# iDC-NEU/NeutronStarLite

Hardware: NVIDIA H100
Metric: gcn_aggregated_edges_per_sec (higher is better)
Workload: dtype f32

## Files before the change

### include/nts_b200.h

```cpp
#ifndef NTS_B200_H
#define NTS_B200_H

#include <stddef.h>
#include <stdint.h>

#ifdef __cplusplus
extern "C" {
#endif

typedef uint32_t nts_vid_t;

int nts_version(void);
const char *nts_last_error(void);
int nts_device_count(void);
int nts_set_device(int device);
int nts_device_sm_count(int *sm_count);
int nts_device_synchronize(void);
int nts_device_reset(void);

void *nts_malloc_device(size_t bytes);
int nts_free_device(void *ptr);
void *nts_malloc_pinned(size_t bytes);
int nts_free_pinned(void *ptr);
void *nts_pinned_device_pointer(void *host_ptr);
int nts_memcpy_h2d(void *dst_device, const void *src_host, size_t bytes, void *stream, int sync);
int nts_memcpy_d2h(void *dst_host, const void *src_device, size_t bytes, void *stream, int sync);
int nts_memcpy_d2d(void *dst_device, const void *src_device, size_t bytes, void *stream);
int nts_zero(void *device_ptr, size_t bytes, void *stream);

void *nts_stream_create(int non_blocking);
int nts_stream_destroy(void *stream);
int nts_stream_synchronize(void *stream);
void *nts_event_create(int with_timing);
int nts_event_destroy(void *event);
int nts_event_record(void *event, void *stream);
int nts_stream_wait_event(void *stream, void *event);
int nts_event_elapsed_ms(void *start, void *stop, float *ms);

int nts_segment_gather_sum(const float *input, float *output, const float *weight,
                           const nts_vid_t *indices, const nts_vid_t *offsets, nts_vid_t index_base,
                           nts_vid_t n_rows, uint64_t n_edges, nts_vid_t feature_size, void *stream);

int nts_gather_by_dst_from_src(const float *input, float *output, const float *weight_forward,
                               const nts_vid_t *row_indices, const nts_vid_t *column_offset,
                               nts_vid_t src_start, nts_vid_t src_end, nts_vid_t dst_start,
                               nts_vid_t dst_end, nts_vid_t edges, nts_vid_t batch_size,
                               nts_vid_t feature_size, int with_weight, void *stream);

int nts_gather_by_src_from_dst(const float *input, float *output, const float *weight_backward,
                               const nts_vid_t *row_offset, const nts_vid_t *column_indices,
                               nts_vid_t src_start, nts_vid_t src_end, nts_vid_t dst_start,
                               nts_vid_t dst_end, nts_vid_t edges, nts_vid_t batch_size,
                               nts_vid_t feature_size, int with_weight, void *stream);

int nts_segment_gather_sum_range(const float *input, float *output, const float *weight, const nts_vid_t *indices,
                                 const nts_vid_t *offsets, const nts_vid_t *slot_of, nts_vid_t index_base,
                                 nts_vid_t n_rows, uint64_t edge_begin, uint64_t edge_end, nts_vid_t feature_size,
                                 void *stream);

typedef struct nts_gather_plan nts_gather_plan;
int nts_gather_plan_pick_slabs(nts_vid_t gather_rows, uint64_t n_edges, nts_vid_t n_rows, nts_vid_t feature_size,
                               uint64_t l2_budget_bytes );
nts_gather_plan *nts_gather_plan_create(const nts_vid_t *offsets, const nts_vid_t *indices, const float *weight,
                                        const nts_vid_t *slot_of, nts_vid_t index_base, nts_vid_t n_rows,
                                        uint64_t n_edges, nts_vid_t gather_rows, int n_slabs, void *stream);
nts_gather_plan *nts_gather_plan_create_hybrid(const nts_vid_t *offsets, const nts_vid_t *indices,
                                               const float *weight, const nts_vid_t *slot_of, nts_vid_t index_base,
                                               nts_vid_t n_rows, uint64_t n_edges, nts_vid_t gather_rows, int n_slabs,
                                               int n_hub_cols, int n_hub_rows, void *stream);
nts_gather_plan *nts_gather_plan_create_tuned(const nts_vid_t *offsets, const nts_vid_t *indices, const float *weight,
                                              const nts_vid_t *slot_of, nts_vid_t index_base, nts_vid_t n_rows,
                                              uint64_t n_edges, nts_vid_t gather_rows, nts_vid_t feature_size,
                                              void *stream);
typedef struct nts_plan_part {
  const nts_vid_t *offsets, *indices;
  const float *weight;
  const nts_vid_t *slot_of;
  nts_vid_t index_base, index_add, n_rows, row_add;
  uint64_t n_edges;
} nts_plan_part;
nts_gather_plan *nts_gather_plan_create_parts(const nts_plan_part *parts, int n_parts, nts_vid_t n_rows,
                                              nts_vid_t gather_rows, int n_slabs, nts_vid_t feature_size, void *stream);
float nts_gather_plan_tuned_ms(const nts_gather_plan *plan);
int nts_gather_plan_destroy(nts_gather_plan *plan);
int nts_gather_plan_slabs(const nts_gather_plan *plan);
int nts_gather_plan_hubs(const nts_gather_plan *plan, int *cols, int *rows);
uint64_t nts_gather_plan_bytes(const nts_gather_plan *plan);
int nts_gather_plan_run(nts_gather_plan *plan, const float *input, float *output, nts_vid_t feature_size,
                        void *stream);
int nts_gather_plan_last_launch(const nts_gather_plan *plan, int *launches, int *grid, int *k, int *u, int *outv);
enum { NTS_DTYPE_F32 = 0, NTS_DTYPE_BF16 = 1 };
int nts_gather_plan_run_bf16(nts_gather_plan *plan, const void *input, int input_dtype, float *output,
                             nts_vid_t feature_size, void *stream);
nts_gather_plan *nts_gather_plan_create_tuned_bf16(const nts_vid_t *offsets, const nts_vid_t *indices,
                                                   const float *weight, const nts_vid_t *slot_of, nts_vid_t index_base,
                                                   nts_vid_t n_rows, uint64_t n_edges, nts_vid_t gather_rows,
                                                   nts_vid_t feature_size, void *stream);
int nts_gather_plan_set_tuning(int u, int min_blocks, int edges_per_warp);
int nts_gather_plan_set_variant(int variant);

int nts_segment_gather_sum_slots(const float *input, float *output, const float *weight,
                                 const nts_vid_t *indices, const nts_vid_t *offsets,
                                 const nts_vid_t *slot_of, nts_vid_t n_rows, uint64_t n_edges,
                                 nts_vid_t feature_size, void *stream);

int nts_segment_gather_sum_heads(const float *input, float *output, const float *weight,
                                 const nts_vid_t *indices, const nts_vid_t *offsets, const nts_vid_t *slot_of,
                                 nts_vid_t index_base, nts_vid_t n_rows, uint64_t n_edges,
                                 nts_vid_t feature_size, nts_vid_t heads, void *stream);

int nts_aggregate_set_variant(int variant, int edges_per_warp);
int nts_aggregate_last_launch(int *grid, int *block, int *smem_bytes, int *variant);
uint64_t nts_kernel_launch_count(void);

int nts_scatter_src_mirror_to_msg(float *message, const float *src_mirror_feature,
                                  const nts_vid_t *row_indices, const nts_vid_t *column_offset,
                                  const nts_vid_t *mirror_index, nts_vid_t batch_size,
                                  nts_vid_t feature_size, void *stream);
int nts_gather_msg_to_src_mirror(float *src_mirror_feature, const float *message,
                                 const nts_vid_t *row_indices, const nts_vid_t *column_offset,
                                 const nts_vid_t *mirror_index, nts_vid_t batch_size,
                                 nts_vid_t feature_size, void *stream);
int nts_scatter_dst_to_msg(float *message, const float *dst_feature, const nts_vid_t *row_indices,
                           const nts_vid_t *column_offset, nts_vid_t batch_size,
                           nts_vid_t feature_size, void *stream);
int nts_gather_msg_to_dst(float *dst_feature, const float *message, const nts_vid_t *row_indices,
                          const nts_vid_t *column_offset, nts_vid_t batch_size,
                          nts_vid_t feature_size, void *stream);
int nts_edge_softmax_forward(float *msg_output, const float *msg_input, float *msg_cached,
                             const nts_vid_t *row_indices, const nts_vid_t *column_offset,
                             nts_vid_t batch_size, nts_vid_t feature_size, void *stream);
int nts_edge_softmax_backward(float *msg_input_grad, const float *msg_output_grad,
                              const float *msg_cached, const nts_vid_t *row_indices,
                              const nts_vid_t *column_offset, nts_vid_t batch_size,
                              nts_vid_t feature_size, void *stream);
int nts_scatter_grad_back_to_message(const float *input, float *message_grad,
                                     const nts_vid_t *row_indices, const nts_vid_t *column_offset,
                                     nts_vid_t batch_size, nts_vid_t feature_size, void *stream);

int nts_aggregate_dst_fuse_weight_backward(float *mirror_grad, float *edge_weight_grad,
                                           const float *mirror, const float *edge_weight,
                                           const float *dst_grad, const nts_vid_t *row_indices,
                                           const nts_vid_t *column_offset,
                                           const nts_vid_t *mirror_index, nts_vid_t batch_size,
                                           nts_vid_t feature_size, void *stream);
int nts_aggregate_dst_fuse_weight_backward_heads(float *mirror_grad, float *edge_weight_grad,
                                                 const float *mirror, const float *edge_weight,
                                                 const float *dst_grad, const nts_vid_t *row_indices,
                                                 const nts_vid_t *column_offset,
                                                 const nts_vid_t *mirror_index, nts_vid_t batch_size,
                                                 nts_vid_t feature_size, nts_vid_t heads, void *stream);

int nts_gat_softmax_stats(float *seg_max, float *seg_sum, const float *src_score, const float *dst_score,
                          const nts_vid_t *row_indices, const nts_vid_t *column_offset,
                          const nts_vid_t *mirror_index, nts_vid_t batch_size, nts_vid_t heads,
                          float negative_slope, void *stream);
int nts_gat_fused_aggregate_forward(const float *mirror, float *output, const float *src_score,
                                    const float *dst_score, const float *seg_max, const float *seg_sum,
                                    const nts_vid_t *row_indices, const nts_vid_t *column_offset,
                                    const nts_vid_t *mirror_index, nts_vid_t batch_size, uint64_t n_edges,
                                    nts_vid_t feature_size, nts_vid_t heads, float negative_slope, void *stream);
int nts_gat_fused_aggregate_backward(float *mirror_grad, float *src_score_grad, float *dst_score_grad,
                                     const float *mirror, const float *src_score, const float *dst_score,
                                     const float *seg_max, const float *seg_sum, const float *out_dot_grad,
                                     const float *dst_grad, const nts_vid_t *row_indices,
                                     const nts_vid_t *column_offset, const nts_vid_t *mirror_index,
                                     nts_vid_t batch_size, nts_vid_t feature_size, nts_vid_t heads,
                                     float negative_slope, void *stream);
int nts_gat_fused_aggregate_backward_two_pass(float *mirror_grad, float *src_score_grad, float *dst_score_grad,
                                              float *dst_pack, const float *mirror, const float *src_score,
                                              const float *dst_score, const float *seg_max, const float *seg_sum,
                                              const float *out_dot_grad, const float *dst_grad,
                                              const nts_vid_t *row_indices, const nts_vid_t *column_offset,
                                              const nts_vid_t *mirror_index, const nts_vid_t *slot_row_offset,
                                              const nts_vid_t *slot_column_indices, nts_vid_t batch_size,
                                              nts_vid_t mirror_size, nts_vid_t feature_size, nts_vid_t heads,
                                              float negative_slope, void *stream);
int nts_gat_fused_aggregate_forward_bf16(const void *mirror, float *output, const float *src_score,
                                         const float *dst_score, const float *seg_max, const float *seg_sum,
                                         const nts_vid_t *row_indices, const nts_vid_t *column_offset,
                                         const nts_vid_t *mirror_index, nts_vid_t batch_size, uint64_t n_edges,
                                         nts_vid_t feature_size, nts_vid_t ld, nts_vid_t heads, float negative_slope,
                                         void *stream);
int nts_gat_fused_aggregate_backward_two_pass_bf16(float *mirror_grad, float *src_score_grad, float *dst_score_grad,
                                                   float *dst_pack, const void *mirror, const float *src_score,
                                                   const float *dst_score, const float *seg_max, const float *seg_sum,
                                                   const float *out_dot_grad, const void *dst_grad,
                                                   const nts_vid_t *row_indices, const nts_vid_t *column_offset,
                                                   const nts_vid_t *mirror_index, const nts_vid_t *slot_row_offset,
                                                   const nts_vid_t *slot_column_indices, nts_vid_t batch_size,
                                                   nts_vid_t mirror_size, nts_vid_t feature_size, nts_vid_t ld,
                                                   nts_vid_t heads, float negative_slope, void *stream);
int nts_rows_to_bf16(const void *src, int src_dtype, nts_vid_t lds, void *dst, nts_vid_t n_rows, nts_vid_t feature_size,
                     nts_vid_t ld, void *stream);

int nts_deserialize_records(float *mirror, const float *records, nts_vid_t n_records,
                            nts_vid_t feature_size, nts_vid_t partition_start,
                            nts_vid_t partition_end, void *stream);
int nts_aggregate_records(float *aggregate, const float *records, nts_vid_t n_records,
                          nts_vid_t feature_size, nts_vid_t partition_start,
                          nts_vid_t partition_end, void *stream);

int nts_gather_rows(float *dst, const float *src, const nts_vid_t *rows, nts_vid_t n_rows,
                    nts_vid_t feature_size, void *stream);
int nts_scatter_add_rows(float *dst, const float *src, const nts_vid_t *rows, nts_vid_t n_rows,
                         nts_vid_t feature_size, void *stream);
int nts_scatter_add_rows_atomic(float *dst, const float *src, const nts_vid_t *rows, nts_vid_t n_rows,
                                nts_vid_t feature_size, void *stream);

int nts_adam_update(float *W, float *M, float *V, const float *grad, uint64_t n, float weight_decay, float beta1,
                    float beta2, float alpha, float epsilon, void *stream);

#define NTS_IPC_HANDLE_BYTES 64
int nts_ipc_get_handle(void *device_ptr, unsigned char handle[NTS_IPC_HANDLE_BYTES]);
void *nts_ipc_open_handle(const unsigned char handle[NTS_IPC_HANDLE_BYTES]);
int nts_ipc_close_handle(void *peer_ptr);
int nts_signal_set(uint32_t *flag, uint32_t value, void *stream);
int nts_signal_wait_geq(const uint32_t *flag, uint32_t value, void *stream);

typedef struct nts_exchange nts_exchange;
typedef struct nts_exchange_chunk {
  const nts_vid_t *column_offset;
  const nts_vid_t *slots;
  const float *weight_forward;
  const nts_vid_t *row_offset_compact;
  const nts_vid_t *column_indices;
  const float *weight_backward;
  uint64_t edges;
} nts_exchange_chunk;
typedef struct nts_exchange_desc {
  int partitions, rank;
  nts_vid_t owned_vertices, dst_start;
  const nts_vid_t *local_column_offset, *local_row_indices, *local_row_offset, *local_column_indices;
  const float *local_weight_forward, *local_weight_backward;
  nts_vid_t local_edges;
  const nts_exchange_chunk *chunks;
  const nts_vid_t *need_count;
  const nts_vid_t *send_count;
  const nts_vid_t *send_rows_all;
  const nts_vid_t *fwd_push_offset;
  const nts_vid_t *bwd_push_offset;
  const nts_vid_t *local_need;
  nts_vid_t local_need_count;
} nts_exchange_desc;

nts_exchange *nts_exchange_create(const nts_exchange_desc *desc);
int nts_exchange_destroy(nts_exchange *ex);
uint64_t nts_exchange_required_floats(const nts_exchange *ex, nts_vid_t feature_size);
uint64_t nts_exchange_required_floats_bf16(const nts_exchange *ex, nts_vid_t feature_size);
uint64_t nts_exchange_capacity_floats(const nts_exchange *ex);
int nts_exchange_release_peers(nts_exchange *ex);
int nts_exchange_reserve(nts_exchange *ex, uint64_t floats_per_buffer, int n_buffers);
int nts_exchange_handles(nts_exchange *ex, unsigned char window_handle[64], unsigned char flags_handle[64]);
int nts_exchange_open_peers(nts_exchange *ex, const unsigned char *window_handles, const unsigned char *flag_handles);
int nts_exchange_forward(nts_exchange *ex, const float *x, float *y, nts_vid_t feature_size, void *stream);
int nts_exchange_backward(nts_exchange *ex, const float *g, float *dx, nts_vid_t feature_size, void *stream);
int nts_exchange_forward_bf16(nts_exchange *ex, const void *x, int x_dtype, float *y, nts_vid_t feature_size,
                              void *stream);
int nts_exchange_backward_bf16(nts_exchange *ex, const float *g, float *dx, nts_vid_t feature_size, void *stream);
int nts_exchange_set_trace(nts_exchange *ex, int enable);
int nts_exchange_last_timeline(nts_exchange *ex, float *ms, int capacity);
int nts_exchange_fetch_mirrors(nts_exchange *ex, const float *x, float *mirror, nts_vid_t feature_size, void *stream);
int nts_exchange_return_mirror_grads(nts_exchange *ex, const float *mirror_grad, float *dx, nts_vid_t feature_size,
                                     void *stream);

typedef struct nts_host_chunk {
  const nts_vid_t *column_offset, *row_indices, *row_offset, *column_indices;
  const float *edge_weight_forward, *edge_weight_backward;
  nts_vid_t src_start, src_end, dst_start, dst_end;
  uint64_t edges;
} nts_host_chunk;
typedef struct nts_exchange_plan nts_exchange_plan;
nts_exchange_plan *nts_exchange_plan_create(const nts_host_chunk *chunks, int partitions, int rank);
void nts_exchange_plan_destroy(nts_exchange_plan *plan);
const nts_vid_t *nts_exchange_plan_need(const nts_exchange_plan *plan, int i, nts_vid_t *count);
uint64_t nts_exchange_plan_packed_rows(const nts_exchange_plan *plan);
int nts_exchange_plan_pack_needs(const nts_exchange_plan *plan, nts_vid_t *need_counts, nts_vid_t *need_rows);
int nts_exchange_plan_set_peer_needs(nts_exchange_plan *plan, int j, const nts_vid_t *need_counts,
                                     const nts_vid_t *need_rows);
int nts_exchange_plan_finalize(nts_exchange_plan *plan);
typedef struct nts_exchange_plan_view {
  int partitions, rank;
  nts_vid_t owned_vertices, recv_total, send_total, backward_rows;
  uint64_t remote_edges;
  const nts_vid_t *need_count, *send_count, *peer_bwd_offset;
  const nts_vid_t *fwd_push_offset, *bwd_push_offset;
  const nts_vid_t *remote_column_offset, *remote_slots;
  const float *remote_weight;
  const nts_vid_t *backward_offsets, *backward_indices;
  const float *backward_weight;
  const nts_vid_t *send_rows_all;
} nts_exchange_plan_view;
int nts_exchange_plan_get_view(const nts_exchange_plan *plan, nts_exchange_plan_view *view);
int nts_exchange_plan_chunk(const nts_exchange_plan *plan, int i, const nts_vid_t **slots,
                            const nts_vid_t **row_offset_compact);
typedef struct nts_device_chunk {
  const nts_vid_t *column_offset, *row_indices, *row_offset, *column_indices;
  const float *edge_weight_forward, *edge_weight_backward;
} nts_device_chunk;
nts_exchange *nts_exchange_create_from_plan(nts_exchange_plan *plan, const nts_device_chunk *device_chunks);

int nts_host_degrees(const nts_vid_t *edges_src_dst, uint64_t n_edges, nts_vid_t n_vertices,
                     nts_vid_t *out_degree, nts_vid_t *in_degree);
int nts_host_partition_offsets(const nts_vid_t *edges_src_dst, uint64_t n_edges, nts_vid_t n_vertices,
                               int partitions, nts_vid_t *partition_offset);
int nts_host_chunk_edge_counts(const nts_vid_t *edges_src_dst, uint64_t n_edges,
                               const nts_vid_t *partition_offset, int partitions, int rank,
                               uint64_t *counts);
int nts_host_build_chunk(const nts_vid_t *edges_src_dst, uint64_t n_edges, nts_vid_t n_vertices,
                         const nts_vid_t *partition_offset, int partitions, int rank, int src_partition,
                         const nts_vid_t *out_degree, const nts_vid_t *in_degree,
                         nts_vid_t *column_offset, nts_vid_t *row_indices, float *edge_weight_forward,
                         nts_vid_t *row_offset, nts_vid_t *column_indices, float *edge_weight_backward,
                         unsigned char *source_active);
int nts_host_mirror_index(const nts_vid_t *edges_src_dst, uint64_t n_edges, nts_vid_t n_vertices,
                          const nts_vid_t *partition_offset, int rank, nts_vid_t *mirror_index,
                          nts_vid_t *owned);

int nts_host_read_feature_label_mask(const char *feature_path, const char *label_path, const char *mask_path,
                                     nts_vid_t feature_size, nts_vid_t v_begin, nts_vid_t v_end, float *features,
                                     int64_t *labels, int32_t *masks);
int nts_host_read_feature_binary(const char *path, nts_vid_t feature_size, nts_vid_t v_begin, nts_vid_t v_end,
                                 float *features);

#ifdef __cplusplus
}
#endif
#endif
```

### neutronstarlite_b200/_lib.py

```python
from __future__ import annotations

import ctypes as C
import os
import re

PKG = os.path.dirname(os.path.abspath(__file__))
ROOT = os.path.dirname(PKG)
LIB_PATH = os.path.join(PKG, "lib", "libnts_b200.so")
HEADER = os.path.join(ROOT, "include", "nts_b200.h")

_vp = C.c_void_p
_u32 = C.c_uint32
_u64 = C.c_uint64
_int = C.c_int
_sz = C.c_size_t

SIGNATURES = {
    "nts_version": (_int, []),
    "nts_last_error": (C.c_char_p, []),
    "nts_device_count": (_int, []),
    "nts_set_device": (_int, [_int]),
    "nts_device_sm_count": (_int, [C.POINTER(_int)]),
    "nts_device_synchronize": (_int, []),
    "nts_device_reset": (_int, []),
    "nts_malloc_device": (_vp, [_sz]),
    "nts_free_device": (_int, [_vp]),
    "nts_malloc_pinned": (_vp, [_sz]),
    "nts_free_pinned": (_int, [_vp]),
    "nts_pinned_device_pointer": (_vp, [_vp]),
    "nts_memcpy_h2d": (_int, [_vp, _vp, _sz, _vp, _int]),
    "nts_memcpy_d2h": (_int, [_vp, _vp, _sz, _vp, _int]),
    "nts_memcpy_d2d": (_int, [_vp, _vp, _sz, _vp]),
    "nts_zero": (_int, [_vp, _sz, _vp]),
    "nts_stream_create": (_vp, [_int]),
    "nts_stream_destroy": (_int, [_vp]),
    "nts_stream_synchronize": (_int, [_vp]),
    "nts_event_create": (_vp, [_int]),
    "nts_event_destroy": (_int, [_vp]),
    "nts_event_record": (_int, [_vp, _vp]),
    "nts_stream_wait_event": (_int, [_vp, _vp]),
    "nts_event_elapsed_ms": (_int, [_vp, _vp, C.POINTER(C.c_float)]),
    "nts_segment_gather_sum": (_int, [_vp, _vp, _vp, _vp, _vp, _u32, _u32, _u64, _u32, _vp]),
    "nts_gather_by_dst_from_src": (_int, [_vp, _vp, _vp, _vp, _vp, _u32, _u32, _u32, _u32, _u32, _u32, _u32, _int, _vp]),
    "nts_gather_by_src_from_dst": (_int, [_vp, _vp, _vp, _vp, _vp, _u32, _u32, _u32, _u32, _u32, _u32, _u32, _int, _vp]),
    "nts_segment_gather_sum_range": (_int, [_vp, _vp, _vp, _vp, _vp, _vp, _u32, _u32, _u64, _u64, _u32, _vp]),
    "nts_gather_plan_pick_slabs": (_int, [_u32, _u64, _u32, _u32, _u64]),
    "nts_gather_plan_create": (_vp, [_vp, _vp, _vp, _vp, _u32, _u32, _u64, _u32, _int, _vp]),
    "nts_gather_plan_create_hybrid": (_vp, [_vp, _vp, _vp, _vp, _u32, _u32, _u64, _u32, _int, _int, _int, _vp]),
    "nts_gather_plan_create_tuned": (_vp, [_vp, _vp, _vp, _vp, _u32, _u32, _u64, _u32, _u32, _vp]),
    "nts_gather_plan_create_parts": (_vp, [_vp, _int, _u32, _u32, _int, _u32, _vp]),
    "nts_gather_plan_tuned_ms": (C.c_float, [_vp]),
    "nts_gather_plan_destroy": (_int, [_vp]),
    "nts_gather_plan_slabs": (_int, [_vp]),
    "nts_gather_plan_hubs": (_int, [_vp, C.POINTER(_int), C.POINTER(_int)]),
    "nts_gather_plan_bytes": (_u64, [_vp]),
    "nts_gather_plan_run": (_int, [_vp, _vp, _vp, _u32, _vp]),
    "nts_gather_plan_run_bf16": (_int, [_vp, _vp, _int, _vp, _u32, _vp]),
    "nts_gather_plan_create_tuned_bf16": (_vp, [_vp, _vp, _vp, _vp, _u32, _u32, _u64, _u32, _u32, _vp]),
    "nts_gather_plan_last_launch": (_int, [_vp] + [C.POINTER(_int)] * 5),
    "nts_gather_plan_set_tuning": (_int, [_int, _int, _int]),
    "nts_gather_plan_set_variant": (_int, [_int]),
    "nts_segment_gather_sum_slots": (_int, [_vp, _vp, _vp, _vp, _vp, _vp, _u32, _u64, _u32, _vp]),
    "nts_segment_gather_sum_heads": (_int, [_vp, _vp, _vp, _vp, _vp, _vp, _u32, _u32, _u64, _u32, _u32, _vp]),
    "nts_aggregate_set_variant": (_int, [_int, _int]),
    "nts_aggregate_last_launch": (_int, [C.POINTER(_int)] * 4),
    "nts_kernel_launch_count": (_u64, []),
    "nts_scatter_src_mirror_to_msg": (_int, [_vp, _vp, _vp, _vp, _vp, _u32, _u32, _vp]),
    "nts_gather_msg_to_src_mirror": (_int, [_vp, _vp, _vp, _vp, _vp, _u32, _u32, _vp]),
    "nts_scatter_dst_to_msg": (_int, [_vp, _vp, _vp, _vp, _u32, _u32, _vp]),
    "nts_gather_msg_to_dst": (_int, [_vp, _vp, _vp, _vp, _u32, _u32, _vp]),
    "nts_edge_softmax_forward": (_int, [_vp, _vp, _vp, _vp, _vp, _u32, _u32, _vp]),
    "nts_edge_softmax_backward": (_int, [_vp, _vp, _vp, _vp, _vp, _u32, _u32, _vp]),
    "nts_scatter_grad_back_to_message": (_int, [_vp, _vp, _vp, _vp, _u32, _u32, _vp]),
    "nts_aggregate_dst_fuse_weight_backward": (_int, [_vp, _vp, _vp, _vp, _vp, _vp, _vp, _vp, _u32, _u32, _vp]),
    "nts_aggregate_dst_fuse_weight_backward_heads": (_int, [_vp] * 8 + [_u32, _u32, _u32, _vp]),
    "nts_gat_softmax_stats": (_int, [_vp] * 7 + [_u32, _u32, C.c_float, _vp]),
    "nts_gat_fused_aggregate_forward": (_int, [_vp] * 9 + [_u32, _u64, _u32, _u32, C.c_float, _vp]),
    "nts_gat_fused_aggregate_backward": (_int, [_vp] * 13 + [_u32, _u32, _u32, C.c_float, _vp]),
    "nts_gat_fused_aggregate_backward_two_pass": (_int, [_vp] * 16 + [_u32, _u32, _u32, _u32, C.c_float, _vp]),
    "nts_gat_fused_aggregate_forward_bf16": (_int, [_vp] * 9 + [_u32, _u64, _u32, _u32, _u32, C.c_float, _vp]),
    "nts_gat_fused_aggregate_backward_two_pass_bf16": (_int, [_vp] * 16 + [_u32] * 5 + [C.c_float, _vp]),
    "nts_rows_to_bf16": (_int, [_vp, _int, _u32, _vp, _u32, _u32, _u32, _vp]),
    "nts_deserialize_records": (_int, [_vp, _vp, _u32, _u32, _u32, _u32, _vp]),
    "nts_aggregate_records": (_int, [_vp, _vp, _u32, _u32, _u32, _u32, _vp]),
    "nts_gather_rows": (_int, [_vp, _vp, _vp, _u32, _u32, _vp]),
    "nts_scatter_add_rows": (_int, [_vp, _vp, _vp, _u32, _u32, _vp]),
    "nts_scatter_add_rows_atomic": (_int, [_vp, _vp, _vp, _u32, _u32, _vp]),
    "nts_ipc_get_handle": (_int, [_vp, C.c_char_p]),
    "nts_ipc_open_handle": (_vp, [C.c_char_p]),
    "nts_ipc_close_handle": (_int, [_vp]),
    "nts_adam_update": (_int, [_vp, _vp, _vp, _vp, _u64] + [C.c_float] * 5 + [_vp]),
    "nts_signal_set": (_int, [_vp, _u32, _vp]),
    "nts_signal_wait_geq": (_int, [_vp, _u32, _vp]),
    "nts_host_degrees": (_int, [_vp, _u64, _u32, _vp, _vp]),
    "nts_host_partition_offsets": (_int, [_vp, _u64, _u32, _int, _vp]),
    "nts_host_chunk_edge_counts": (_int, [_vp, _u64, _vp, _int, _int, _vp]),
    "nts_host_build_chunk": (_int, [_vp, _u64, _u32, _vp, _int, _int, _int, _vp, _vp, _vp, _vp, _vp, _vp, _vp, _vp, _vp]),
    "nts_host_mirror_index": (_int, [_vp, _u64, _u32, _vp, _int, _vp, _vp]),
    "nts_host_read_feature_label_mask": (_int, [C.c_char_p, C.c_char_p, C.c_char_p, _u32, _u32, _u32, _vp, _vp, _vp]),
    "nts_host_read_feature_binary": (_int, [C.c_char_p, _u32, _u32, _u32, _vp]),
}



class ExchangeChunk(C.Structure):
    _fields_ = [
        ("column_offset", _vp), ("slots", _vp), ("weight_forward", _vp), ("row_offset_compact", _vp),
        ("column_indices", _vp), ("weight_backward", _vp), ("edges", _u64),
    ]


class ExchangeDesc(C.Structure):
    _fields_ = [
        ("partitions", _int), ("rank", _int), ("owned_vertices", _u32), ("dst_start", _u32),
        ("local_column_offset", _vp), ("local_row_indices", _vp), ("local_row_offset", _vp),
        ("local_column_indices", _vp), ("local_weight_forward", _vp), ("local_weight_backward", _vp),
        ("local_edges", _u32),
        ("chunks", C.POINTER(ExchangeChunk)),
        ("need_count", C.POINTER(_u32)), ("send_count", C.POINTER(_u32)),
        ("send_rows_all", _vp), ("fwd_push_offset", C.POINTER(_u32)), ("bwd_push_offset", C.POINTER(_u32)),
        ("local_need", _vp), ("local_need_count", _u32),
    ]


class DeviceChunk(C.Structure):
    _fields_ = [
        ("column_offset", _vp), ("row_indices", _vp), ("row_offset", _vp), ("column_indices", _vp),
        ("edge_weight_forward", _vp), ("edge_weight_backward", _vp),
    ]


SIGNATURES.update({
    "nts_exchange_create": (_vp, [C.POINTER(ExchangeDesc)]),
    "nts_exchange_destroy": (_int, [_vp]),
    "nts_exchange_required_floats": (_u64, [_vp, _u32]),
    "nts_exchange_capacity_floats": (_u64, [_vp]),
    "nts_exchange_release_peers": (_int, [_vp]),
    "nts_exchange_reserve": (_int, [_vp, _u64, _int]),
    "nts_exchange_handles": (_int, [_vp, C.c_char_p, C.c_char_p]),
    "nts_exchange_open_peers": (_int, [_vp, C.c_char_p, C.c_char_p]),
    "nts_exchange_forward": (_int, [_vp, _vp, _vp, _u32, _vp]),
    "nts_exchange_backward": (_int, [_vp, _vp, _vp, _u32, _vp]),
    "nts_exchange_forward_bf16": (_int, [_vp, _vp, _int, _vp, _u32, _vp]),
    "nts_exchange_backward_bf16": (_int, [_vp, _vp, _vp, _u32, _vp]),
    "nts_exchange_required_floats_bf16": (_u64, [_vp, _u32]),
    "nts_exchange_set_trace": (_int, [_vp, _int]),
    "nts_exchange_last_timeline": (_int, [_vp, C.POINTER(C.c_float), _int]),
    "nts_exchange_fetch_mirrors": (_int, [_vp, _vp, _vp, _u32, _vp]),
    "nts_exchange_return_mirror_grads": (_int, [_vp, _vp, _vp, _u32, _vp]),
})



class HostChunk(C.Structure):
    _fields_ = [
        ("column_offset", _vp), ("row_indices", _vp), ("row_offset", _vp), ("column_indices", _vp),
        ("edge_weight_forward", _vp), ("edge_weight_backward", _vp),
        ("src_start", _u32), ("src_end", _u32), ("dst_start", _u32), ("dst_end", _u32), ("edges", _u64),
    ]


class ExchangePlanView(C.Structure):
    _fields_ = [
        ("partitions", _int), ("rank", _int),
        ("owned_vertices", _u32), ("recv_total", _u32), ("send_total", _u32), ("backward_rows", _u32),
        ("remote_edges", _u64),
        ("need_count", C.POINTER(_u32)), ("send_count", C.POINTER(_u32)), ("peer_bwd_offset", C.POINTER(_u32)),
        ("fwd_push_offset", C.POINTER(_u32)), ("bwd_push_offset", C.POINTER(_u32)),
        ("remote_column_offset", C.POINTER(_u32)), ("remote_slots", C.POINTER(_u32)),
        ("remote_weight", C.POINTER(C.c_float)),
        ("backward_offsets", C.POINTER(_u32)), ("backward_indices", C.POINTER(_u32)),
        ("backward_weight", C.POINTER(C.c_float)),
        ("send_rows_all", C.POINTER(_u32)),
    ]


SIGNATURES.update({
    "nts_exchange_plan_create": (_vp, [C.POINTER(HostChunk), _int, _int]),
    "nts_exchange_plan_destroy": (None, [_vp]),
    "nts_exchange_plan_need": (C.POINTER(_u32), [_vp, _int, C.POINTER(_u32)]),
    "nts_exchange_plan_packed_rows": (_u64, [_vp]),
    "nts_exchange_plan_pack_needs": (_int, [_vp, _vp, _vp]),
    "nts_exchange_plan_set_peer_needs": (_int, [_vp, _int, _vp, _vp]),
    "nts_exchange_plan_finalize": (_int, [_vp]),
    "nts_exchange_plan_get_view": (_int, [_vp, C.POINTER(ExchangePlanView)]),
    "nts_exchange_plan_chunk": (_int, [_vp, _int, C.POINTER(C.POINTER(_u32)), C.POINTER(C.POINTER(_u32))]),
    "nts_exchange_create_from_plan": (_vp, [_vp, C.POINTER(DeviceChunk)]),
})

_lib = None


class NtsError(RuntimeError):
    pass


def header_symbols():
    text = open(HEADER).read()
    text = re.sub(r"/\*.*?\*/", "", text, flags=re.S)
    return sorted(set(re.findall(r"\b(nts_[a-z0-9_]+)\s*\(", text)))


def load():
    global _lib
    if _lib is not None:
        return _lib
    if not os.path.exists(LIB_PATH):
        raise NtsError("libnts_b200.so not found at %s - run `python -m neutronstarlite_b200.build` "
                       "(there is no CPU fallback)" % LIB_PATH)
    lib = C.CDLL(LIB_PATH, mode=C.RTLD_GLOBAL)
    for name, (res, args) in SIGNATURES.items():
        fn = getattr(lib, name)
        fn.restype = res
        fn.argtypes = args
    _lib = lib
    return lib


def check(rc, what=""):
    if rc != 0:
        msg = load().nts_last_error().decode(errors="replace")
        raise NtsError("libnts_b200 %s failed (rc=%d): %s" % (what, rc, msg))


def call(name, *args):
    rc = getattr(load(), name)(*args)
    check(rc, name)
```

### neutronstarlite_b200/csrc/nts_common.cuh

```cuda
#pragma once
#include <cuda_bf16.h>
#include <cuda_runtime.h>
#include <stdint.h>
#include <stdio.h>
#include <stdlib.h>
#include <string.h>

#include "nts_b200.h"

namespace nts {

char *last_error_buffer();
bool abort_on_error();
void count_launch();

inline int fail(int code, const char *what, const char *file, int line) {
  snprintf(last_error_buffer(), 512, "%s (%s:%d)", what, file, line);
  if (abort_on_error()) {
    fprintf(stderr, "libnts_b200: %s\n", last_error_buffer());
    exit(1);
  }
  return code;
}

#define NTS_CUDA_OK(expr)                                                                         \
  do {                                                                                            \
    cudaError_t nts_e_ = (expr);                                                                  \
    if (nts_e_ != cudaSuccess)                                                                    \
      return ::nts::fail((int)nts_e_, cudaGetErrorString(nts_e_), __FILE__, __LINE__);            \
  } while (0)

#define NTS_ARG_CHECK(cond, msg)                                                                  \
  do {                                                                                            \
    if (!(cond))                                                                                  \
      return ::nts::fail(-1, msg, __FILE__, __LINE__);                                            \
  } while (0)

#define NTS_LAUNCH_CHECK()                                                                        \
  do {                                                                                            \
    ::nts::count_launch();                                                                        \
    NTS_CUDA_OK(cudaGetLastError());                                                              \
  } while (0)

inline cudaStream_t as_stream(void *s) { return reinterpret_cast<cudaStream_t>(s); }

inline bool aligned_to(const void *p, size_t a) { return (reinterpret_cast<uintptr_t>(p) & (a - 1)) == 0; }

int sm_count();

int run_plan_bf16(nts_gather_plan *pl, const void *input, int dtype, uint32_t lds, float *output, uint32_t F,
                  cudaStream_t st);
int to_bf16_rows(const void *src, int dtype, uint32_t lds, void *dst, uint32_t n_rows, uint32_t F, uint32_t ld,
                 cudaStream_t st);

int check_gat_bf16_layout(uint32_t F, uint32_t ld, uint32_t heads);

struct __align__(16) float8v {
  float4 lo, hi;
};

template <int VEC> struct Vec;
template <> struct Vec<1> { using type = float; };
template <> struct Vec<2> { using type = float2; };
template <> struct Vec<4> { using type = float4; };
template <> struct Vec<8> { using type = float8v; };

template <class T, int VEC> struct Ld { using type = typename Vec<VEC>::type; };
template <> struct Ld<__nv_bfloat16, 2> { using type = uint32_t; };
template <> struct Ld<__nv_bfloat16, 4> { using type = uint2; };
template <> struct Ld<__nv_bfloat16, 8> { using type = uint4; };
__device__ __forceinline__ float widen(float v) { return v; }
__device__ __forceinline__ float2 widen(float2 v) { return v; }
__device__ __forceinline__ float4 widen(float4 v) { return v; }
__device__ __forceinline__ float2 widen(uint32_t u) {
  return make_float2(__uint_as_float(u << 16), __uint_as_float(u & 0xffff0000u));
}
__device__ __forceinline__ float4 widen(uint2 u) {
  const float2 a = widen(u.x), b = widen(u.y);
  return make_float4(a.x, a.y, b.x, b.y);
}
__device__ __forceinline__ float8v widen(uint4 u) { return {widen(make_uint2(u.x, u.y)), widen(make_uint2(u.z, u.w))}; }

}

extern "C" nts_gather_plan *nts_plan_create_parts_typed(const nts_plan_part *parts, int n_parts, nts_vid_t n_rows,
                                                        nts_vid_t gather_rows, int n_slabs, nts_vid_t feature_size,
                                                        int bf16, void *stream);
```

### neutronstarlite_b200/csrc/nts_plan.cu

```cuda
#include <cub/cub.cuh>
#include <cuda_bf16.h>

#include <algorithm>
#include <type_traits>
#include <vector>

#include "nts_common.cuh"

struct nts_gather_plan {
  uint32_t n_rows = 0;
  uint64_t n_edges = 0;
  uint32_t gather_rows = 0;
  int slabs = 1;
  uint32_t slab_rows = 0;
  uint2 *pairs = nullptr;
  uint32_t *voff = nullptr;
  std::vector<uint64_t> slab_edge;
  float *workspace = nullptr;
  size_t workspace_floats = 0;
  __nv_bfloat16 *workspace_bf16 = nullptr;
  size_t workspace_bf16_elems = 0;
  int hub_cols = 0, hub_rows = 0;
  uint32_t *hub_col_ids = nullptr;
  uint32_t *hub_row_ids = nullptr;
  uint32_t lda_c = 0, lda_r = 0;
  float *dense = nullptr;
  size_t dense_floats = 0;
  int last_grid = 0, last_launches = 0, last_k = 0, last_u = 0, last_outv = 0;
  float tuned_ms = 0.f;
};

namespace nts {

static int g_plan_u = 0, g_plan_minb = 0, g_plan_q = 0, g_plan_variant = 0;

__device__ __forceinline__ uint32_t plan_find_row(const uint32_t *__restrict__ off, uint32_t n_rows, uint32_t e) {
  uint32_t lo = 0, hi = n_rows;
  while (hi - lo > 1) {
    uint32_t mid = lo + ((hi - lo) >> 1);
    if (__ldg(off + mid) <= e)
      lo = mid;
    else
      hi = mid;
  }
  return lo;
}

__global__ void plan_keys_kernel(const uint32_t *__restrict__ off, const uint32_t *__restrict__ idx,
                                 const uint32_t *__restrict__ slot_of, uint32_t base, uint32_t n_rows, uint32_t n_edges,
                                 uint32_t slab_rows, uint32_t slabs, uint32_t *__restrict__ key,
                                 uint32_t *__restrict__ val) {
  for (uint64_t e = (uint64_t)blockIdx.x * blockDim.x + threadIdx.x; e < n_edges; e += (uint64_t)gridDim.x * blockDim.x) {
    const uint32_t r = plan_find_row(off, n_rows, (uint32_t)e);
    const uint32_t id = __ldg(idx + e);
    const uint32_t g = slot_of ? __ldg(slot_of + id) : id - base;
    uint32_t s = g / slab_rows;
    if (s >= slabs)
      s = slabs - 1;
    key[e] = s * n_rows + r;
    val[e] = (uint32_t)e;
  }
}

__global__ void plan_pairs_kernel(const uint32_t *__restrict__ perm, const uint32_t *__restrict__ idx,
                                  const float *__restrict__ w, const uint32_t *__restrict__ slot_of, uint32_t base,
                                  uint32_t n_edges, uint2 *__restrict__ pairs) {
  for (uint64_t i = (uint64_t)blockIdx.x * blockDim.x + threadIdx.x; i < n_edges; i += (uint64_t)gridDim.x * blockDim.x) {
    const uint32_t e = perm ? __ldg(perm + i) : (uint32_t)i;
    const uint32_t id = __ldg(idx + e);
    const uint32_t g = slot_of ? __ldg(slot_of + id) : id - base;
    const float wt = w ? __ldg(w + e) : 1.f;
    pairs[i] = make_uint2(g, __float_as_uint(wt));
  }
}

__global__ void plan_part_keys_kernel(const uint32_t *__restrict__ off, const uint32_t *__restrict__ idx,
                                      const uint32_t *__restrict__ slot_of, const float *__restrict__ w, uint32_t base,
                                      uint32_t index_add, uint32_t n_rows_part, uint32_t row_add, uint32_t n_edges,
                                      uint32_t e_off, uint32_t n_rows_total, uint32_t slab_rows, uint32_t slabs,
                                      uint32_t *__restrict__ key, uint32_t *__restrict__ val,
                                      uint2 *__restrict__ unsorted) {
  for (uint64_t e = (uint64_t)blockIdx.x * blockDim.x + threadIdx.x; e < n_edges; e += (uint64_t)gridDim.x * blockDim.x) {
    const uint32_t r = plan_find_row(off, n_rows_part, (uint32_t)e) + row_add;
    const uint32_t id = __ldg(idx + e);
    const uint32_t g = (slot_of ? __ldg(slot_of + id) : id - base) + index_add;
    uint32_t s = g / slab_rows;
    if (s >= slabs)
      s = slabs - 1;
    key[e_off + e] = s * n_rows_total + r;
    val[e_off + e] = e_off + (uint32_t)e;
    unsorted[e_off + e] = make_uint2(g, __float_as_uint(w ? __ldg(w + e) : 1.f));
  }
}
__global__ void plan_permute_pairs_kernel(const uint32_t *__restrict__ perm, const uint2 *__restrict__ unsorted,
                                          uint32_t n_edges, uint2 *__restrict__ pairs) {
  for (uint64_t i = (uint64_t)blockIdx.x * blockDim.x + threadIdx.x; i < n_edges; i += (uint64_t)gridDim.x * blockDim.x)
    pairs[i] = unsorted[__ldg(perm + i)];
}

template <class KeyT>
__global__ void plan_offsets_kernel(const KeyT *__restrict__ sorted_key, uint32_t n_edges, uint32_t n_keys,
                                    uint32_t *__restrict__ voff) {
  for (uint64_t k = (uint64_t)blockIdx.x * blockDim.x + threadIdx.x; k <= n_keys; k += (uint64_t)gridDim.x * blockDim.x) {
    uint32_t lo = 0, hi = n_edges;
    while (lo < hi) {
      uint32_t mid = lo + ((hi - lo) >> 1);
      if (__ldg(sorted_key + mid) < (KeyT)k)
        lo = mid + 1;
      else
        hi = mid;
    }
    voff[k] = lo;
  }
}

constexpr uint32_t kNoHub = 0xffffffffu;

__global__ void plan_ref_count_kernel(const uint32_t *__restrict__ idx, const uint32_t *__restrict__ slot_of,
                                      uint32_t base, uint32_t n_edges, uint32_t *__restrict__ cnt) {
  for (uint64_t e = (uint64_t)blockIdx.x * blockDim.x + threadIdx.x; e < n_edges; e += (uint64_t)gridDim.x * blockDim.x) {
    const uint32_t id = __ldg(idx + e);
    atomicAdd(cnt + (slot_of ? __ldg(slot_of + id) : id - base), 1u);
  }
}

__global__ void plan_hybrid_keys_kernel(const uint32_t *__restrict__ off, const uint32_t *__restrict__ idx,
                                        const uint32_t *__restrict__ slot_of, uint32_t base, uint32_t n_rows,
                                        uint32_t n_edges, uint32_t slab_rows, uint32_t slabs,
                                        const uint32_t *__restrict__ col_slot, const uint32_t *__restrict__ row_slot,
                                        uint32_t lda_c, uint64_t dc_cells, uint32_t lda_r, uint64_t *__restrict__ key,
                                        uint32_t *__restrict__ val) {
  const uint64_t n_keys = (uint64_t)slabs * n_rows;
  for (uint64_t e = (uint64_t)blockIdx.x * blockDim.x + threadIdx.x; e < n_edges; e += (uint64_t)gridDim.x * blockDim.x) {
    const uint32_t r = plan_find_row(off, n_rows, (uint32_t)e);
    const uint32_t id = __ldg(idx + e);
    const uint32_t g = slot_of ? __ldg(slot_of + id) : id - base;
    const uint32_t cs = __ldg(col_slot + g), rs = __ldg(row_slot + r);
    uint64_t k;
    if (cs != kNoHub) {
      k = n_keys + (uint64_t)cs * lda_c + r;
    } else if (rs != kNoHub) {
      k = n_keys + dc_cells + (uint64_t)g * lda_r + rs;
    } else {
      uint32_t s = g / slab_rows;
      if (s >= slabs)
        s = slabs - 1;
      k = (uint64_t)s * n_rows + r;
    }
    key[e] = k;
    val[e] = (uint32_t)e;
  }
}

__global__ void plan_cell_sum_kernel(const uint64_t *__restrict__ cell_key, const uint32_t *__restrict__ run_start,
                                     const uint32_t *__restrict__ run_len, uint32_t n_runs,
                                     const uint32_t *__restrict__ perm, const float *__restrict__ w, uint64_t n_keys,
                                     float *__restrict__ dense) {
  const uint32_t lane = threadIdx.x & 31;
  for (uint64_t run = ((uint64_t)blockIdx.x * blockDim.x + threadIdx.x) >> 5; run < n_runs;
       run += ((uint64_t)gridDim.x * blockDim.x) >> 5) {
    const uint32_t b = __ldg(run_start + run), n = __ldg(run_len + run);
    float s = 0.f;
    for (uint32_t j = lane; j < n; j += 32)
      s += w ? __ldg(w + __ldg(perm + b + j)) : 1.f;
#pragma unroll
    for (int o = 16; o > 0; o >>= 1)
      s += __shfl_xor_sync(0xffffffffu, s, o);
    if (lane == 0)
      dense[__ldg(cell_key + run) - n_keys] = s;
  }
}

__global__ void pad_rows_kernel(const float *__restrict__ src, float *__restrict__ dst, uint32_t n_rows, uint32_t F,
                                uint32_t ld) {
  const uint64_t total = (uint64_t)n_rows * ld;
  for (uint64_t i = (uint64_t)blockIdx.x * blockDim.x + threadIdx.x; i < total; i += (uint64_t)gridDim.x * blockDim.x) {
    const uint64_t r = i / ld;
    const uint32_t c = (uint32_t)(i - r * ld);
    dst[i] = c < F ? __ldg(src + r * F + c) : 0.f;
  }
}

template <class S>
__global__ void bf16_rows_kernel(const S *__restrict__ src, uint32_t lds, uint4 *__restrict__ dst, uint32_t n_rows,
                                 uint32_t F, uint32_t ld) {
  const uint32_t ld8 = ld / 8;
  const uint64_t total = (uint64_t)n_rows * ld8;
  for (uint64_t i = (uint64_t)blockIdx.x * blockDim.x + threadIdx.x; i < total; i += (uint64_t)gridDim.x * blockDim.x) {
    const uint64_t r = i / ld8;
    const uint32_t c = (uint32_t)(i - r * ld8) * 8;
    const S *s = src + r * lds;
    uint32_t w[4];
#pragma unroll
    for (int j = 0; j < 4; j++) {
      const uint32_t c0 = c + 2 * j, c1 = c0 + 1;
      if constexpr (std::is_same<S, float>::value) {
        const __nv_bfloat162 h = __floats2bfloat162_rn(c0 < F ? __ldg(s + c0) : 0.f, c1 < F ? __ldg(s + c1) : 0.f);
        w[j] = *reinterpret_cast<const uint32_t *>(&h);
      } else {
        const uint16_t *u = reinterpret_cast<const uint16_t *>(s);
        w[j] = (c0 < F ? (uint32_t)__ldg(u + c0) : 0u) | ((c1 < F ? (uint32_t)__ldg(u + c1) : 0u) << 16);
      }
    }
    dst[i] = make_uint4(w[0], w[1], w[2], w[3]);
  }
}

__device__ __forceinline__ uint32_t p_smem_u32(const void *p) { return (uint32_t)__cvta_generic_to_shared(p); }
__device__ __forceinline__ void p_mbar_init(uint64_t *bar, uint32_t count) {
  asm volatile("mbarrier.init.shared::cta.b64 [%0], %1;" ::"r"(p_smem_u32(bar)), "r"(count));
}
__device__ __forceinline__ void p_mbar_expect_tx(uint64_t *bar, uint32_t bytes) {
  asm volatile("mbarrier.arrive.expect_tx.shared::cta.b64 _, [%0], %1;" ::"r"(p_smem_u32(bar)), "r"(bytes) : "memory");
}
__device__ __forceinline__ void p_mbar_wait(uint64_t *bar, uint32_t parity) {
  asm volatile("{\n\t"
               ".reg .pred p;\n\t"
               "WAIT_%=:\n\t"
               "mbarrier.try_wait.parity.shared::cta.b64 p, [%0], %1;\n\t"
               "@p bra DONE_%=;\n\t"
               "bra WAIT_%=;\n\t"
               "DONE_%=:\n\t"
               "}" ::"r"(p_smem_u32(bar)),
               "r"(parity)
               : "memory");
}
__device__ __forceinline__ void p_bulk_g2s(void *smem_dst, const void *gmem_src, uint32_t bytes, uint64_t *bar) {
  asm volatile("cp.async.bulk.shared::cluster.global.mbarrier::complete_tx::bytes [%0], [%1], %2, [%3];" ::"r"(
                   p_smem_u32(smem_dst)),
               "l"(gmem_src), "r"(bytes), "r"(p_smem_u32(bar))
               : "memory");
}

constexpr int kPlanWarps = 8;

template <int OUTV, bool ATOMIC>
__device__ __forceinline__ void flush_chunk(float *__restrict__ orow, uint32_t col, uint32_t F, float4 a) {
  if constexpr (OUTV == 4) {
    float4 *p = reinterpret_cast<float4 *>(orow + col);
    if constexpr (ATOMIC) {
      asm volatile("red.global.add.v4.f32 [%0], {%1, %2, %3, %4};" ::"l"(p), "f"(a.x), "f"(a.y), "f"(a.z), "f"(a.w)
                   : "memory");
    } else {
      float4 o = *p;
      o.x += a.x, o.y += a.y, o.z += a.z, o.w += a.w;
      *p = o;
    }
  } else if constexpr (OUTV == 2) {
    float2 *p = reinterpret_cast<float2 *>(orow + col);
    if constexpr (ATOMIC) {
      asm volatile("red.global.add.v2.f32 [%0], {%1, %2};" ::"l"(p), "f"(a.x), "f"(a.y) : "memory");
      if (col + 2 < F)
        asm volatile("red.global.add.v2.f32 [%0], {%1, %2};" ::"l"(p + 1), "f"(a.z), "f"(a.w) : "memory");
    } else {
      float2 o = p[0];
      o.x += a.x, o.y += a.y;
      p[0] = o;
      if (col + 2 < F) {
        float2 o1 = p[1];
        o1.x += a.z, o1.y += a.w;
        p[1] = o1;
      }
    }
  } else {
    const float v[4] = {a.x, a.y, a.z, a.w};
#pragma unroll
    for (int i = 0; i < 4; i++)
      if (col + i < F) {
        if constexpr (ATOMIC)
          atomicAdd(orow + col + i, v[i]);
        else
          orow[col + i] += v[i];
      }
  }
}

template <class T> struct GatherT;
template <> struct GatherT<float> {
  using chunk = float4;
  static constexpr int V = 4;
  __device__ static __forceinline__ void widen(const float4 &c, float (&v)[4]) {
    v[0] = c.x, v[1] = c.y, v[2] = c.z, v[3] = c.w;
  }
};
template <> struct GatherT<__nv_bfloat16> {
  using chunk = uint4;
  static constexpr int V = 8;
  __device__ static __forceinline__ void widen(const uint4 &c, float (&v)[8]) {
    const uint32_t u[4] = {c.x, c.y, c.z, c.w};
#pragma unroll
    for (int i = 0; i < 4; i++) {
      v[2 * i] = __uint_as_float(u[i] << 16);
      v[2 * i + 1] = __uint_as_float(u[i] & 0xffff0000u);
    }
  }
};

template <class T, int K, int U, int OUTV, int MINB, int G = 1>
__global__ void __launch_bounds__(kPlanWarps * 32, MINB)
    planned_gather_sum_kernel(const typename GatherT<T>::chunk *__restrict__ in, uint32_t ldc, float *__restrict__ out,
                              uint32_t F, const uint2 *__restrict__ pairs, const uint32_t *__restrict__ off,
                              uint32_t n_rows, uint32_t e_begin, uint32_t e_end, uint32_t Q, uint32_t tiles,
                              uint32_t tile_vecs) {
  static_assert(G == 1 || K == 1, "virtual warps are for rows narrower than a warp");
  using Chunk = typename GatherT<T>::chunk;
  constexpr int V = GatherT<T>::V;
  constexpr uint32_t GS = 32 / G;
  const uint32_t lane = threadIdx.x & (GS - 1);
  const uint32_t vwarp_in_block = threadIdx.x / GS;
  const uint64_t gwarp = (uint64_t)blockIdx.x * (kPlanWarps * G) + vwarp_in_block;
  const uint32_t tile = (uint32_t)(gwarp % tiles);
  const uint64_t q = gwarp / tiles;
  const uint64_t e0_64 = e_begin + q * (uint64_t)Q;

  extern __shared__ __align__(16) unsigned char smem_raw[];
  uint64_t *bar = reinterpret_cast<uint64_t *>(smem_raw);
  uint2 *s_pair = reinterpret_cast<uint2 *>(smem_raw + 16);
  uint32_t cta_e_base = 0, bulk_bytes = 0;
  {
    const uint64_t cta_w0 = (uint64_t)blockIdx.x * (kPlanWarps * G);
    const uint64_t first_q = cta_w0 / tiles;
    const uint64_t last_q = (cta_w0 + kPlanWarps * G - 1) / tiles;
    uint64_t ce0 = e_begin + first_q * (uint64_t)Q;
    uint64_t ce1 = e_begin + (last_q + 1) * (uint64_t)Q;
    if (ce1 > e_end)
      ce1 = e_end;
    if (ce0 < ce1) {
      cta_e_base = (uint32_t)(ce0 & ~1ull);
      const uint32_t n_el = (uint32_t)(ce1 - cta_e_base);
      bulk_bytes = (n_el * 8u) & ~15u;
      if (threadIdx.x == 0) {
        p_mbar_init(bar, 1);
        asm volatile("fence.mbarrier_init.release.cluster;" ::: "memory");
        if (n_el & 1u)
          s_pair[n_el - 1] = __ldg(pairs + cta_e_base + n_el - 1);
      }
      __syncthreads();
      if (threadIdx.x == 0 && bulk_bytes) {
        p_mbar_expect_tx(bar, bulk_bytes);
        p_bulk_g2s(s_pair, pairs + cta_e_base, bulk_bytes, bar);
      }
    }
  }
  if (e0_64 >= e_end)
    return;
  const uint32_t e0 = (uint32_t)e0_64;
  const uint32_t e1 = (e0_64 + Q < e_end) ? e0 + Q : e_end;

  const uint32_t c0 = tile * tile_vecs + lane;
  bool act[K];
#pragma unroll
  for (int k = 0; k < K; k++)
    act[k] = (k * GS + lane) < tile_vecs && (c0 + k * GS) < ldc;

  uint32_t row = plan_find_row(off, n_rows, e0);
  uint32_t row_end = __ldg(off + row + 1);
  bool row_started_inside = __ldg(off + row) >= e0;

  float acc[K][V];
#pragma unroll
  for (int k = 0; k < K; k++)
#pragma unroll
    for (int j = 0; j < V; j++)
      acc[k][j] = 0.f;

  auto flush = [&](bool whole) {
    float *orow = out + (size_t)row * F;
#pragma unroll
    for (int k = 0; k < K; k++) {
#pragma unroll
      for (int h = 0; h < V; h += 4) {
        const uint32_t col = (c0 + k * GS) * V + h;
        const float4 a = make_float4(acc[k][h], acc[k][h + 1], acc[k][h + 2], acc[k][h + 3]);
        if (act[k] && col < F) {
          if (whole)
            flush_chunk<OUTV, false>(orow, col, F, a);
          else
            flush_chunk<OUTV, true>(orow, col, F, a);
        }
      }
#pragma unroll
      for (int j = 0; j < V; j++)
        acc[k][j] = 0.f;
    }
  };
  auto advance = [&](uint32_t ee) {
    flush(row_started_inside);
    do {
      row++;
      row_end = __ldg(off + row + 1);
    } while (ee >= row_end);
    row_started_inside = true;
  };

  if (bulk_bytes)
    p_mbar_wait(bar, 0);

  const uint2 *sp = s_pair - cta_e_base;
  uint32_t e = e0;
  auto fma_chunk = [&](int k, float w, const Chunk &c) {
    float x[V];
    GatherT<T>::widen(c, x);
#pragma unroll
    for (int j = 0; j < V; j++)
      acc[k][j] = fmaf(w, x[j], acc[k][j]);
  };
  for (; e + U <= e1; e += U) {
    Chunk v[U][K];
    float wu[U];
#pragma unroll
    for (int u = 0; u < U; u++) {
      const uint2 pr = sp[e + u];
      wu[u] = __uint_as_float(pr.y);
      const Chunk *p = in + (size_t)pr.x * ldc + c0;
#pragma unroll
      for (int k = 0; k < K; k++)
        if (act[k])
          v[u][k] = __ldg(p + k * GS);
    }
#pragma unroll
    for (int u = 0; u < U; u++) {
      if (e + u >= row_end)
        advance(e + u);
#pragma unroll
      for (int k = 0; k < K; k++)
        if (act[k])
          fma_chunk(k, wu[u], v[u][k]);
    }
  }
  for (; e < e1; e++) {
    const uint2 pr = sp[e];
    const float wj = __uint_as_float(pr.y);
    const Chunk *p = in + (size_t)pr.x * ldc + c0;
    Chunk v1[K];
#pragma unroll
    for (int k = 0; k < K; k++)
      if (act[k])
        v1[k] = __ldg(p + k * GS);
    if (e >= row_end)
      advance(e);
#pragma unroll
    for (int k = 0; k < K; k++)
      if (act[k])
        fma_chunk(k, wj, v1[k]);
  }
  flush(row_started_inside && row_end <= e1);
}

struct PlanShape;
template <int K, int STAGES, int OUTV, int MINB>
__global__ void __launch_bounds__(kPlanWarps * 32, MINB)
    planned_gather_sum_tma_kernel(const float4 *__restrict__ in, uint32_t ld4, float *__restrict__ out, uint32_t F,
                                  const uint2 *__restrict__ pairs, const uint32_t *__restrict__ off, uint32_t n_rows,
                                  uint32_t e_begin, uint32_t e_end, uint32_t Q, uint32_t tiles, uint32_t tile_vecs,
                                  uint32_t pair_bytes) {
  const uint32_t lane = threadIdx.x & 31;
  const uint32_t warp_in_block = threadIdx.x >> 5;
  const uint64_t gwarp = (uint64_t)blockIdx.x * kPlanWarps + warp_in_block;
  const uint32_t tile = (uint32_t)(gwarp % tiles);
  const uint64_t q = gwarp / tiles;
  const uint64_t e0_64 = e_begin + q * (uint64_t)Q;

  extern __shared__ __align__(16) unsigned char smem_raw[];
  uint64_t *bar = reinterpret_cast<uint64_t *>(smem_raw);
  uint2 *s_pair = reinterpret_cast<uint2 *>(smem_raw + 16);
  const uint32_t ring_bytes = 8u * STAGES + 8u * (STAGES & 1) + STAGES * tile_vecs * 16u;
  unsigned char *ring = smem_raw + 16 + pair_bytes + (size_t)warp_in_block * ring_bytes;
  uint64_t *sbar = reinterpret_cast<uint64_t *>(ring);
  float4 *sbuf = reinterpret_cast<float4 *>(ring + 8u * STAGES + 8u * (STAGES & 1));
  uint32_t cta_e_base = 0, bulk_bytes = 0;
  {
    const uint64_t cta_w0 = (uint64_t)blockIdx.x * kPlanWarps;
    const uint64_t first_q = cta_w0 / tiles;
    const uint64_t last_q = (cta_w0 + kPlanWarps - 1) / tiles;
    uint64_t ce0 = e_begin + first_q * (uint64_t)Q;
    uint64_t ce1 = e_begin + (last_q + 1) * (uint64_t)Q;
    if (ce1 > e_end)
      ce1 = e_end;
    if (lane == 0)
      for (int s = 0; s < STAGES; s++)
        p_mbar_init(sbar + s, 1);
    if (ce0 < ce1) {
      cta_e_base = (uint32_t)(ce0 & ~1ull);
      const uint32_t n_el = (uint32_t)(ce1 - cta_e_base);
      bulk_bytes = (n_el * 8u) & ~15u;
      if (threadIdx.x == 0) {
        p_mbar_init(bar, 1);
        if (n_el & 1u)
          s_pair[n_el - 1] = __ldg(pairs + cta_e_base + n_el - 1);
      }
    }
    asm volatile("fence.mbarrier_init.release.cluster;" ::: "memory");
    __syncthreads();
    if (threadIdx.x == 0 && bulk_bytes) {
      p_mbar_expect_tx(bar, bulk_bytes);
      p_bulk_g2s(s_pair, pairs + cta_e_base, bulk_bytes, bar);
    }
  }
  if (e0_64 >= e_end)
    return;
  const uint32_t e0 = (uint32_t)e0_64;
  const uint32_t e1 = (e0_64 + Q < e_end) ? e0 + Q : e_end;
  const uint32_t c0 = tile * tile_vecs + lane;
  const uint32_t my_vecs = min(tile_vecs, ld4 - tile * tile_vecs);
  const uint32_t row_bytes = my_vecs * 16u;
  bool act[K];
#pragma unroll
  for (int k = 0; k < K; k++)
    act[k] = (k * 32 + lane) < my_vecs;

  uint32_t row = plan_find_row(off, n_rows, e0);
  uint32_t row_end = __ldg(off + row + 1);
  bool row_started_inside = __ldg(off + row) >= e0;
  float4 acc[K];
#pragma unroll
  for (int k = 0; k < K; k++)
    acc[k] = make_float4(0.f, 0.f, 0.f, 0.f);
  auto flush = [&](bool whole) {
    float *orow = out + (size_t)row * F;
#pragma unroll
    for (int k = 0; k < K; k++) {
      const uint32_t col = (c0 + k * 32) * 4;
      if (act[k] && col < F) {
        if (whole)
          flush_chunk<OUTV, false>(orow, col, F, acc[k]);
        else
          flush_chunk<OUTV, true>(orow, col, F, acc[k]);
      }
      acc[k] = make_float4(0.f, 0.f, 0.f, 0.f);
    }
  };
  auto advance = [&](uint32_t ee) {
    flush(row_started_inside);
    do {
      row++;
      row_end = __ldg(off + row + 1);
    } while (ee >= row_end);
    row_started_inside = true;
  };
  if (bulk_bytes)
    p_mbar_wait(bar, 0);
  const uint2 *sp = s_pair - cta_e_base;
  auto issue = [&](uint32_t e, uint32_t stage) {
    const uint32_t src_row = sp[e].x;
    p_mbar_expect_tx(sbar + stage, row_bytes);
    p_bulk_g2s(sbuf + (size_t)stage * tile_vecs, in + (size_t)src_row * ld4 + tile * tile_vecs, row_bytes, sbar + stage);
  };
  if (lane == 0)
    for (uint32_t s = 0; s < STAGES && e0 + s < e1; s++)
      issue(e0 + s, s);
  uint32_t stage = 0, parity = 0;
  for (uint32_t e = e0; e < e1; e++) {
    const float w = __uint_as_float(sp[e].y);
    p_mbar_wait(sbar + stage, parity);
    const float4 *b = sbuf + (size_t)stage * tile_vecs + lane;
    float4 v[K];
#pragma unroll
    for (int k = 0; k < K; k++)
      if (act[k])
        v[k] = b[k * 32];
    if (e >= row_end)
      advance(e);
#pragma unroll
    for (int k = 0; k < K; k++)
      if (act[k]) {
        acc[k].x = fmaf(w, v[k].x, acc[k].x);
        acc[k].y = fmaf(w, v[k].y, acc[k].y);
        acc[k].z = fmaf(w, v[k].z, acc[k].z);
        acc[k].w = fmaf(w, v[k].w, acc[k].w);
      }
    __syncwarp();
    if (lane == 0 && e + STAGES < e1)
      issue(e + STAGES, stage);
    if (++stage == STAGES) {
      stage = 0;
      parity ^= 1u;
    }
  }
  flush(row_started_inside && row_end <= e1);
}

template <int K, int STAGES, int OUTV, int MINB>
static int launch_planned_tma(nts_gather_plan *pl, const PlanShape &sh, const float4 *in, uint32_t ld4, float *out,
                              uint32_t F, uint32_t Q, cudaStream_t st);

struct PlanShape {
  int k, u, outv, minb, g;
  uint32_t tiles, tile_vecs;
};

template <class T, int K, int U, int OUTV, int MINB, int G = 1>
static int launch_planned(nts_gather_plan *pl, const PlanShape &sh, const T *in_rows, uint32_t ldc, float *out,
                          uint32_t F, uint32_t Q, cudaStream_t st) {
  auto kern = planned_gather_sum_kernel<T, K, U, OUTV, MINB, G>;
  const auto *in = reinterpret_cast<const typename GatherT<T>::chunk *>(in_rows);
  const size_t smem = 16 + ((size_t)kPlanWarps * G * Q + 4) * 8;
  NTS_CUDA_OK(cudaFuncSetAttribute(kern, cudaFuncAttributeMaxDynamicSharedMemorySize, (int)smem));
  pl->last_launches = 0;
  for (int s = 0; s < pl->slabs; s++) {
    const uint64_t eb = pl->slab_edge[s], ee = pl->slab_edge[s + 1];
    if (ee <= eb)
      continue;
    const uint64_t quanta = (ee - eb + Q - 1) / Q;
    const uint64_t blocks = (quanta * sh.tiles + kPlanWarps * G - 1) / (kPlanWarps * G);
    NTS_ARG_CHECK(blocks <= 0x7fffffffull, "aggregation grid too large");
    kern<<<(unsigned)blocks, kPlanWarps * 32, smem, st>>>(in, ldc, out, F, pl->pairs, pl->voff + (size_t)s * pl->n_rows,
                                                          pl->n_rows, (uint32_t)eb, (uint32_t)ee, Q, sh.tiles,
                                                          sh.tile_vecs);
    NTS_LAUNCH_CHECK();
    pl->last_grid = (int)blocks;
    pl->last_launches++;
  }
  return 0;
}

template <int K, int STAGES, int OUTV, int MINB>
static int launch_planned_tma(nts_gather_plan *pl, const PlanShape &sh, const float4 *in, uint32_t ld4, float *out,
                              uint32_t F, uint32_t Q, cudaStream_t st) {
  auto kern = planned_gather_sum_tma_kernel<K, STAGES, OUTV, MINB>;
  const uint32_t pair_bytes = (kPlanWarps * Q + 4) * 8;
  const uint32_t ring_bytes = 8u * STAGES + 8u * (STAGES & 1) + STAGES * sh.tile_vecs * 16u;
  const size_t smem = 16 + pair_bytes + (size_t)kPlanWarps * ring_bytes;
  NTS_ARG_CHECK(smem <= 227 * 1024, "row-staging ring does not fit shared memory");
  NTS_CUDA_OK(cudaFuncSetAttribute(kern, cudaFuncAttributeMaxDynamicSharedMemorySize, (int)smem));
  pl->last_launches = 0;
  for (int s = 0; s < pl->slabs; s++) {
    const uint64_t eb = pl->slab_edge[s], ee = pl->slab_edge[s + 1];
    if (ee <= eb)
      continue;
    const uint64_t quanta = (ee - eb + Q - 1) / Q;
    const uint64_t blocks = (quanta * sh.tiles + kPlanWarps - 1) / kPlanWarps;
    NTS_ARG_CHECK(blocks <= 0x7fffffffull, "aggregation grid too large");
    kern<<<(unsigned)blocks, kPlanWarps * 32, smem, st>>>(in, ld4, out, F, pl->pairs, pl->voff + (size_t)s * pl->n_rows,
                                                          pl->n_rows, (uint32_t)eb, (uint32_t)ee, Q, sh.tiles,
                                                          sh.tile_vecs, pair_bytes);
    NTS_LAUNCH_CHECK();
    pl->last_grid = (int)blocks;
    pl->last_launches++;
  }
  return 0;
}

#define NTS_PLAN_TMA_CASE(K_, S_, B_)                                                                               \
  if (sh.k == K_ && stages == S_ && sh.minb == B_) {                                                                \
    if (sh.outv == 4)                                                                                               \
      return launch_planned_tma<K_, S_, 4, B_>(pl, sh, in4, ld4, out, F, Q, st);                                    \
    if (sh.outv == 2)                                                                                               \
      return launch_planned_tma<K_, S_, 2, B_>(pl, sh, in4, ld4, out, F, Q, st);                                    \
    return launch_planned_tma<K_, S_, 1, B_>(pl, sh, in4, ld4, out, F, Q, st);                                      \
  }

#define NTS_PLAN_CASE_G(U_, B_, G_)                                                                                 \
  if (sh.k == 1 && sh.u == U_ && sh.minb == B_ && sh.g == G_) {                                                     \
    if (sh.outv == 4)                                                                                               \
      return launch_planned<T, 1, U_, 4, B_, G_>(pl, sh, in, ldc, out, F, Q, st);                                   \
    if (sh.outv == 2)                                                                                               \
      return launch_planned<T, 1, U_, 2, B_, G_>(pl, sh, in, ldc, out, F, Q, st);                                   \
    return launch_planned<T, 1, U_, 1, B_, G_>(pl, sh, in, ldc, out, F, Q, st);                                     \
  }

#define NTS_PLAN_CASE(K_, U_, B_)                                                                                   \
  if (sh.k == K_ && sh.u == U_ && sh.minb == B_) {                                                                  \
    if (sh.outv == 4)                                                                                               \
      return launch_planned<T, K_, U_, 4, B_>(pl, sh, in, ldc, out, F, Q, st);                                       \
    if (sh.outv == 2)                                                                                               \
      return launch_planned<T, K_, U_, 2, B_>(pl, sh, in, ldc, out, F, Q, st);                                       \
    return launch_planned<T, K_, U_, 1, B_>(pl, sh, in, ldc, out, F, Q, st);                                         \
  }

constexpr int kHubBM = 128, kHubBN = 128, kHubBK = 16, kHubThreads = 256;

__device__ __forceinline__ void p_cp_async16(void *smem_dst, const void *gmem_src, bool full) {
  asm volatile("cp.async.cg.shared.global [%0], [%1], 16, %2;" ::"r"(p_smem_u32(smem_dst)), "l"(gmem_src),
               "r"(full ? 16 : 0)
               : "memory");
}

template <class TB, int OUTV, bool SPLIT>
__global__ void __launch_bounds__(kHubThreads, 2)
    hub_block_gemm_kernel(const float *__restrict__ At, uint32_t lda, uint32_t M, uint32_t K, uint32_t k_split,
                          const TB *__restrict__ B, uint32_t ldb, const uint32_t *__restrict__ colmap,
                          float *__restrict__ out, uint32_t F, const uint32_t *__restrict__ rowmap, uint32_t m_tiles,
                          uint32_t n_tiles) {
  constexpr bool kBf16 = std::is_same<TB, __nv_bfloat16>::value;
  constexpr uint32_t kBV = 16 / sizeof(TB);
  __shared__ __align__(16) float As[2][kHubBK][kHubBM];
  __shared__ __align__(16) TB Bs[2][kHubBK][kHubBN];
  const uint32_t t = threadIdx.x;
  const uint32_t n_tile = blockIdx.x % n_tiles, rest = blockIdx.x / n_tiles;
  const uint32_t m0 = (rest % m_tiles) * kHubBM, n0 = n_tile * kHubBN;
  const uint32_t k_begin = (rest / m_tiles) * k_split;
  const uint32_t k_end = min(K, k_begin + k_split);
  if (k_begin >= k_end)
    return;
  const uint32_t n_kt = (k_end - k_begin + kHubBK - 1) / kHubBK;

  auto load = [&](uint32_t kt, int buf) {
#pragma unroll
    for (int i = 0; i < 2; i++) {
      const uint32_t c = t + i * kHubThreads, kk = c >> 5, c4 = (c & 31) * 4;
      const uint32_t k = k_begin + kt * kHubBK + kk;
      const bool a_ok = k < k_end && m0 + c4 < lda;
      p_cp_async16(&As[buf][kk][c4], a_ok ? At + (size_t)k * lda + m0 + c4 : At, a_ok);
    }
#pragma unroll
    for (int i = 0; i < (int)(kHubBK * kHubBN / kBV / kHubThreads); i++) {
      constexpr uint32_t kRowChunks = kHubBN / kBV;
      const uint32_t c = t + i * kHubThreads, kk = c / kRowChunks, cv = (c % kRowChunks) * kBV;
      const uint32_t k = k_begin + kt * kHubBK + kk;
      const bool b_ok = k < k_end && n0 + cv < ldb;
      const uint32_t brow = b_ok ? (colmap ? __ldg(colmap + k) : k) : 0;
      p_cp_async16(&Bs[buf][kk][cv], B + (size_t)brow * ldb + (b_ok ? n0 + cv : 0), b_ok);
    }
    asm volatile("cp.async.commit_group;" ::: "memory");
  };
  auto read_b4 = [&](int buf, int kk, uint32_t n) -> float4 {
    if constexpr (kBf16) {
      const uint2 u = *reinterpret_cast<const uint2 *>(&Bs[buf][kk][n]);
      return make_float4(__uint_as_float(u.x << 16), __uint_as_float(u.x & 0xffff0000u), __uint_as_float(u.y << 16),
                         __uint_as_float(u.y & 0xffff0000u));
    } else {
      return *reinterpret_cast<const float4 *>(&Bs[buf][kk][n]);
    }
  };

  const uint32_t tx = t & 15, ty = t >> 4;
  float acc[8][8];
#pragma unroll
  for (int i = 0; i < 8; i++)
#pragma unroll
    for (int j = 0; j < 8; j++)
      acc[i][j] = 0.f;

  load(0, 0);
  for (uint32_t kt = 0; kt < n_kt; kt++) {
    const int buf = kt & 1;
    if (kt + 1 < n_kt) {
      load(kt + 1, buf ^ 1);
      asm volatile("cp.async.wait_group 1;" ::: "memory");
    } else {
      asm volatile("cp.async.wait_group 0;" ::: "memory");
    }
    __syncthreads();
#pragma unroll
    for (int kk = 0; kk < kHubBK; kk++) {
      const float4 a0 = *reinterpret_cast<const float4 *>(&As[buf][kk][ty * 4]);
      const float4 a1 = *reinterpret_cast<const float4 *>(&As[buf][kk][64 + ty * 4]);
      const float4 b0 = read_b4(buf, kk, tx * 4);
      const float4 b1 = read_b4(buf, kk, 64 + tx * 4);
      const float a[8] = {a0.x, a0.y, a0.z, a0.w, a1.x, a1.y, a1.z, a1.w};
      const float b[8] = {b0.x, b0.y, b0.z, b0.w, b1.x, b1.y, b1.z, b1.w};
#pragma unroll
      for (int i = 0; i < 8; i++)
#pragma unroll
        for (int j = 0; j < 8; j++)
          acc[i][j] = fmaf(a[i], b[j], acc[i][j]);
    }
    __syncthreads();
  }

#pragma unroll
  for (int i = 0; i < 8; i++) {
    const uint32_t m = m0 + (i >> 2) * 64 + ty * 4 + (i & 3);
    if (m >= M)
      continue;
    float *orow = out + (size_t)(rowmap ? __ldg(rowmap + m) : m) * F;
#pragma unroll
    for (int j = 0; j < 2; j++) {
      const uint32_t col = n0 + j * 64 + tx * 4;
      if (col < F)
        flush_chunk<OUTV, SPLIT>(orow, col, F,
                                 make_float4(acc[i][j * 4], acc[i][j * 4 + 1], acc[i][j * 4 + 2], acc[i][j * 4 + 3]));
    }
  }
}

template <class TB, int OUTV>
static int launch_hub_blocks(nts_gather_plan *pl, const TB *in, uint32_t ldb, float *out, uint32_t F,
                             cudaStream_t st) {
  const uint32_t n_tiles = (F + kHubBN - 1) / kHubBN;
  if (pl->hub_cols) {
    const uint32_t m_tiles = (pl->n_rows + kHubBM - 1) / kHubBM;
    const uint64_t blocks = (uint64_t)m_tiles * n_tiles;
    NTS_ARG_CHECK(blocks <= 0x7fffffffull, "hub column block grid too large");
    hub_block_gemm_kernel<TB, OUTV, false><<<(unsigned)blocks, kHubThreads, 0, st>>>(
        pl->dense, pl->lda_c, pl->n_rows, (uint32_t)pl->hub_cols, (uint32_t)pl->hub_cols, in, ldb, pl->hub_col_ids, out,
        F, nullptr, m_tiles, n_tiles);
    NTS_LAUNCH_CHECK();
  }
  if (pl->hub_rows) {
    const uint32_t m_tiles = (pl->hub_rows + kHubBM - 1) / kHubBM;
    const uint32_t K = pl->gather_rows;
    const uint64_t want = (uint64_t)sm_count() * 2 * 4;
    uint64_t splits = (want + (uint64_t)m_tiles * n_tiles - 1) / ((uint64_t)m_tiles * n_tiles);
    uint32_t k_split = (uint32_t)((K + splits - 1) / splits);
    k_split = std::max<uint32_t>((k_split + kHubBK - 1) / kHubBK * kHubBK, 16 * kHubBK);
    splits = (K + k_split - 1) / k_split;
    hub_block_gemm_kernel<TB, OUTV, true><<<(unsigned)(splits * m_tiles * n_tiles), kHubThreads, 0, st>>>(
        pl->dense + (size_t)pl->hub_cols * pl->lda_c, pl->lda_r, (uint32_t)pl->hub_rows, K, k_split, in, ldb, nullptr,
        out, F, pl->hub_row_ids, m_tiles, n_tiles);
    NTS_LAUNCH_CHECK();
  }
  return 0;
}

template <class T>
static int run_gather(nts_gather_plan *pl, const T *in, uint32_t ld, float *output, uint32_t F, cudaStream_t st) {
  constexpr bool kBf16 = std::is_same<T, __nv_bfloat16>::value;
  PlanShape sh;
  const uint32_t ldc = ld / GatherT<T>::V;
  const uint32_t chunks = (ldc + 31) / 32;
  const uint32_t kmax = 5;
  sh.tiles = (chunks + kmax - 1) / kmax;
  sh.tile_vecs = (ldc + sh.tiles - 1) / sh.tiles;
  sh.k = (int)((sh.tile_vecs + 31) / 32);
  sh.tiles = (ldc + sh.tile_vecs - 1) / sh.tile_vecs;
  sh.outv = (F % 4 == 0 && aligned_to(output, 16)) ? 4 : ((F % 2 == 0 && aligned_to(output, 8)) ? 2 : 1);
  if (pl->hub_cols || pl->hub_rows) {
    const int rc = sh.outv == 4   ? launch_hub_blocks<T, 4>(pl, in, ld, output, F, st)
                   : sh.outv == 2 ? launch_hub_blocks<T, 2>(pl, in, ld, output, F, st)
                                  : launch_hub_blocks<T, 1>(pl, in, ld, output, F, st);
    if (rc)
      return rc;
  }
  sh.g = ldc <= 8 ? 4 : (ldc <= 16 ? 2 : 1);
  if (g_plan_variant == 1 || getenv("NTS_PLAN_NO_SUBWARP"))
    sh.g = 1;
  sh.minb = sh.k >= 3 ? 2 : (sh.k == 2 ? 3 : 4);
  sh.u = sh.k == 4 ? 2 : 4;
  if constexpr (kBf16) {
    sh.minb = sh.k >= 4 ? 2 : (sh.k >= 2 ? 3 : 4);
    sh.u = sh.k == 1 ? 4 : 2;
  }
  {
    static int env_read = 0;
    if (!env_read) {
      env_read = 1;
      if (const char *t = getenv("NTS_PLAN_TUNE"))
        sscanf(t, "%d,%d,%d", &g_plan_u, &g_plan_minb, &g_plan_q);
    }
    if (g_plan_u > 0)
      sh.u = g_plan_u;
    if (g_plan_minb > 0)
      sh.minb = g_plan_minb;
  }
  uint32_t Q = g_plan_q > 0 ? (uint32_t)g_plan_q : 512u / sh.g;
  if (g_plan_q <= 0) {
    const uint64_t per_slab = pl->slab_edge[pl->slabs] / (uint64_t)pl->slabs + 1;
    const uint64_t want_warps = (uint64_t)sm_count() * 64 * sh.g;
    while (Q > 32 && ((per_slab + Q - 1) / Q) * sh.tiles < want_warps)
      Q >>= 1;
  }
  Q = (Q + 31u) & ~31u;
  if (Q * sh.g > 1024)
    Q = (1024 / sh.g) & ~31u;
  pl->last_k = sh.k, pl->last_u = sh.u, pl->last_outv = sh.outv;
  float *out = output;
  if constexpr (kBf16) {
    NTS_PLAN_CASE_G(4, 4, 2)
    NTS_PLAN_CASE_G(4, 4, 4)
    NTS_PLAN_CASE_G(8, 2, 2)
    NTS_PLAN_CASE_G(8, 2, 4)
    if (sh.g != 1)
      return fail(-1, "no BF16 virtual-warp instantiation for this (U, occupancy) point", __FILE__, __LINE__);
    NTS_PLAN_CASE(1, 4, 4)
    NTS_PLAN_CASE(1, 8, 2)
    NTS_PLAN_CASE(2, 2, 3)
    NTS_PLAN_CASE(2, 4, 2)
    NTS_PLAN_CASE(3, 4, 2)
    NTS_PLAN_CASE(3, 2, 3)
    NTS_PLAN_CASE(3, 6, 1)
    NTS_PLAN_CASE(4, 2, 2)
    NTS_PLAN_CASE(4, 4, 2)
    NTS_PLAN_CASE(5, 2, 2)
    return fail(-1, "no BF16 planned-aggregation instantiation for this (chunks, U, occupancy) point", __FILE__,
                __LINE__);
  } else {
  const float4 *in4 = reinterpret_cast<const float4 *>(in);
  const uint32_t ld4 = ldc;
  if (g_plan_variant == 1) {
    const int stages = sh.u >= 8 ? 8 : (sh.u >= 4 ? 4 : 2);
    sh.minb = g_plan_minb > 0 ? g_plan_minb : (sh.k >= 4 ? 2 : 4);
    NTS_PLAN_TMA_CASE(1, 8, 4)
    NTS_PLAN_TMA_CASE(1, 4, 4)
    NTS_PLAN_TMA_CASE(1, 8, 3)
    NTS_PLAN_TMA_CASE(2, 4, 3)
    NTS_PLAN_TMA_CASE(2, 4, 2)
    NTS_PLAN_TMA_CASE(3, 4, 2)
    NTS_PLAN_TMA_CASE(4, 4, 2)
    NTS_PLAN_TMA_CASE(4, 2, 2)
    NTS_PLAN_TMA_CASE(5, 4, 2)
    NTS_PLAN_TMA_CASE(5, 2, 2)
    NTS_PLAN_TMA_CASE(5, 4, 1)
    NTS_PLAN_TMA_CASE(5, 8, 1)
    return fail(-1, "no TMA row-staging instantiation for this (chunks, stages, occupancy) point", __FILE__, __LINE__);
  }
  NTS_PLAN_CASE_G(4, 4, 2)
  NTS_PLAN_CASE_G(4, 4, 4)
  NTS_PLAN_CASE_G(8, 3, 2)
  NTS_PLAN_CASE_G(8, 3, 4)
  if (sh.g != 1)
    return fail(-1, "no virtual-warp instantiation for this (U, occupancy) point", __FILE__, __LINE__);
  NTS_PLAN_CASE(1, 8, 4)
  NTS_PLAN_CASE(1, 4, 4)
  NTS_PLAN_CASE(1, 8, 3)
  NTS_PLAN_CASE(1, 16, 2)
  NTS_PLAN_CASE(2, 4, 3)
  NTS_PLAN_CASE(2, 8, 2)
  NTS_PLAN_CASE(3, 4, 3)
  NTS_PLAN_CASE(3, 4, 2)
  NTS_PLAN_CASE(4, 2, 2)
  NTS_PLAN_CASE(4, 4, 2)
  NTS_PLAN_CASE(5, 2, 2)
  NTS_PLAN_CASE(5, 1, 3)
  NTS_PLAN_CASE(5, 2, 3)
  NTS_PLAN_CASE(5, 4, 1)
  NTS_PLAN_CASE(5, 4, 2)
  return fail(-1, "no planned-aggregation instantiation for this (chunks, U, occupancy) point", __FILE__, __LINE__);
  }
}

template <class E> static int ensure_workspace(E *&ws, size_t &have, size_t elems) {
  if (elems <= have)
    return 0;
  if (ws)
    NTS_CUDA_OK(cudaFree(ws));
  ws = nullptr;
  have = 0;
  NTS_CUDA_OK(cudaMalloc(reinterpret_cast<void **>(&ws), elems * sizeof(E)));
  have = elems;
  return 0;
}

static int run_plan(nts_gather_plan *pl, const float *input, float *output, uint32_t F, cudaStream_t st) {
  if (pl->n_rows == 0 || pl->n_edges == 0 || F == 0)
    return 0;
  NTS_ARG_CHECK(input && output, "null feature pointer");
  const uint32_t ld = (F + 3u) & ~3u;
  const float *in = input;
  if (ld != F || !aligned_to(input, 16)) {
    if (const int rc = ensure_workspace(pl->workspace, pl->workspace_floats, (size_t)pl->gather_rows * ld))
      return rc;
    const uint64_t total = (uint64_t)pl->gather_rows * ld;
    const unsigned blocks = (unsigned)std::min<uint64_t>((total + 255) / 256, (uint64_t)sm_count() * 32);
    pad_rows_kernel<<<blocks, 256, 0, st>>>(input, pl->workspace, pl->gather_rows, F, ld);
    NTS_LAUNCH_CHECK();
    in = pl->workspace;
  }
  return run_gather<float>(pl, in, ld, output, F, st);
}

int to_bf16_rows(const void *src, int dtype, uint32_t lds, void *dst, uint32_t n_rows, uint32_t F, uint32_t ld,
                 cudaStream_t st) {
  NTS_ARG_CHECK(dtype == NTS_DTYPE_F32 || dtype == NTS_DTYPE_BF16, "input dtype must be NTS_DTYPE_F32 or NTS_DTYPE_BF16");
  NTS_ARG_CHECK(ld % 8 == 0 && ld >= F && lds >= F && aligned_to(dst, 16), "bad BF16 row layout");
  if (!n_rows || !F)
    return 0;
  const uint64_t total = (uint64_t)n_rows * (ld / 8);
  const unsigned blocks = (unsigned)std::min<uint64_t>((total + 255) / 256, (uint64_t)sm_count() * 32);
  uint4 *d = static_cast<uint4 *>(dst);
  if (dtype == NTS_DTYPE_F32)
    bf16_rows_kernel<float><<<blocks, 256, 0, st>>>(static_cast<const float *>(src), lds, d, n_rows, F, ld);
  else
    bf16_rows_kernel<__nv_bfloat16><<<blocks, 256, 0, st>>>(static_cast<const __nv_bfloat16 *>(src), lds, d, n_rows,
                                                            F, ld);
  NTS_LAUNCH_CHECK();
  return 0;
}

int run_plan_bf16(nts_gather_plan *pl, const void *input, int dtype, uint32_t lds, float *output, uint32_t F,
                  cudaStream_t st) {
  NTS_ARG_CHECK(dtype == NTS_DTYPE_F32 || dtype == NTS_DTYPE_BF16, "input dtype must be NTS_DTYPE_F32 or NTS_DTYPE_BF16");
  NTS_ARG_CHECK(g_plan_variant == 0, "the TMA row-staging variant (nts_gather_plan_set_variant(1)) gathers FP32 rows only");
  if (pl->n_rows == 0 || pl->n_edges == 0 || F == 0)
    return 0;
  NTS_ARG_CHECK(input && output, "null feature pointer");
  NTS_ARG_CHECK(lds >= F, "row stride below the feature width");
  if (dtype == NTS_DTYPE_BF16 && lds % 8 == 0 && aligned_to(input, 16))
    return run_gather<__nv_bfloat16>(pl, static_cast<const __nv_bfloat16 *>(input), lds, output, F, st);
  const uint32_t ld = (F + 7u) & ~7u;
  if (const int rc = ensure_workspace(pl->workspace_bf16, pl->workspace_bf16_elems, (size_t)pl->gather_rows * ld))
    return rc;
  if (const int rc = to_bf16_rows(input, dtype, lds, pl->workspace_bf16, pl->gather_rows, F, ld, st))
    return rc;
  return run_gather<__nv_bfloat16>(pl, pl->workspace_bf16, ld, output, F, st);
}

}

using namespace nts;

extern "C" {

static int pick_slabs_for_rows(nts_vid_t gather_rows, uint64_t n_edges, nts_vid_t n_rows, uint64_t row_bytes,
                               uint64_t l2_budget_bytes) {
  if (!l2_budget_bytes)
    l2_budget_bytes = 16ull << 20;
  const uint64_t bytes = (uint64_t)gather_rows * row_bytes;
  uint64_t s = (bytes + l2_budget_bytes - 1) / l2_budget_bytes;
  const uint64_t by_degree = n_rows ? n_edges / ((uint64_t)n_rows * 16ull) : 1;
  if (s > by_degree)
    s = by_degree;
  if (s > 64)
    s = 64;
  return s < 1 ? 1 : (int)s;
}

int nts_gather_plan_pick_slabs(nts_vid_t gather_rows, uint64_t n_edges, nts_vid_t n_rows, nts_vid_t feature_size,
                               uint64_t l2_budget_bytes) {
  return pick_slabs_for_rows(gather_rows, n_edges, n_rows, ((feature_size + 3ull) & ~3ull) * 4ull, l2_budget_bytes);
}

static bool hub_counts(const nts_vid_t *offsets, const nts_vid_t *indices, const nts_vid_t *slot_of, nts_vid_t base,
                       uint32_t n_rows, uint32_t E, uint32_t gather_rows, std::vector<uint32_t> &col_cnt,
                       std::vector<uint32_t> &seg, cudaStream_t st) {
  uint32_t *cnt = nullptr;
  std::vector<uint32_t> off(n_rows + 1);
  col_cnt.assign(gather_rows, 0);
  const unsigned blocks = (unsigned)std::min<uint64_t>(((uint64_t)E + 255) / 256, (uint64_t)sm_count() * 32);
  bool ok = cudaMalloc(reinterpret_cast<void **>(&cnt), (size_t)gather_rows * 4) == cudaSuccess &&
            cudaMemsetAsync(cnt, 0, (size_t)gather_rows * 4, st) == cudaSuccess;
  if (ok && E) {
    plan_ref_count_kernel<<<blocks, 256, 0, st>>>(indices, slot_of, base, E, cnt);
    count_launch();
  }
  ok = ok && cudaMemcpyAsync(col_cnt.data(), cnt, (size_t)gather_rows * 4, cudaMemcpyDeviceToHost, st) == cudaSuccess &&
       cudaMemcpyAsync(off.data(), offsets, ((size_t)n_rows + 1) * 4, cudaMemcpyDeviceToHost, st) == cudaSuccess &&
       cudaStreamSynchronize(st) == cudaSuccess;
  cudaFree(cnt);
  seg.resize(n_rows);
  for (uint32_t r = 0; r < n_rows; r++)
    seg[r] = off[r + 1] - off[r];
  return ok;
}

static std::vector<uint32_t> top_ids(const std::vector<uint32_t> &cnt, size_t h) {
  std::vector<uint32_t> ids(cnt.size());
  for (size_t i = 0; i < ids.size(); i++)
    ids[i] = (uint32_t)i;
  h = std::min(h, ids.size());
  std::partial_sort(ids.begin(), ids.begin() + h, ids.end(),
                    [&](uint32_t a, uint32_t b) { return cnt[a] != cnt[b] ? cnt[a] > cnt[b] : a < b; });
  ids.resize(h);
  return ids;
}

static bool build_hybrid(nts_gather_plan *pl, const nts_vid_t *offsets, const nts_vid_t *indices, const float *weight,
                         const nts_vid_t *slot_of, nts_vid_t index_base, int n_hub_cols, int n_hub_rows,
                         cudaStream_t st) {
  const uint32_t E = (uint32_t)pl->n_edges, n_rows = pl->n_rows, G = pl->gather_rows;
  std::vector<uint32_t> col_cnt, seg;
  if (!hub_counts(offsets, indices, slot_of, index_base, n_rows, E, G, col_cnt, seg, st))
    return false;
  const std::vector<uint32_t> cols = top_ids(col_cnt, (size_t)n_hub_cols), rows = top_ids(seg, (size_t)n_hub_rows);
  pl->hub_cols = (int)cols.size();
  pl->hub_rows = (int)rows.size();
  pl->lda_c = (n_rows + 3u) & ~3u;
  pl->lda_r = ((uint32_t)pl->hub_rows + 3u) & ~3u;
  const uint64_t dc_cells = (uint64_t)pl->hub_cols * pl->lda_c;
  pl->dense_floats = dc_cells + (pl->hub_rows ? (uint64_t)G * pl->lda_r : 0);
  std::vector<uint32_t> col_slot(G, kNoHub), row_slot(n_rows, kNoHub);
  for (size_t i = 0; i < cols.size(); i++)
    col_slot[cols[i]] = (uint32_t)i;
  for (size_t i = 0; i < rows.size(); i++)
    row_slot[rows[i]] = (uint32_t)i;

  const uint64_t n_keys = (uint64_t)pl->slabs * n_rows;
  int bits = 1;
  while (bits < 64 && (1ull << bits) < n_keys + pl->dense_floats)
    bits++;
  uint64_t *key_in = nullptr, *key_out = nullptr;
  uint32_t *val_in = nullptr, *val_out = nullptr, *d_col_slot = nullptr, *d_row_slot = nullptr, *d_runs = nullptr;
  void *tmp = nullptr;
  size_t tmp_bytes = 0;
  bool ok =
      cudaMalloc(reinterpret_cast<void **>(&pl->pairs), (size_t)E * sizeof(uint2)) == cudaSuccess &&
      cudaMalloc(reinterpret_cast<void **>(&pl->voff), ((size_t)n_keys + 1) * 4) == cudaSuccess &&
      cudaMalloc(reinterpret_cast<void **>(&pl->dense), pl->dense_floats * 4) == cudaSuccess &&
      cudaMalloc(reinterpret_cast<void **>(&pl->hub_col_ids), cols.size() * 4 + 4) == cudaSuccess &&
      cudaMalloc(reinterpret_cast<void **>(&pl->hub_row_ids), rows.size() * 4 + 4) == cudaSuccess &&
      cudaMalloc(reinterpret_cast<void **>(&d_col_slot), (size_t)G * 4 + 4) == cudaSuccess &&
      cudaMalloc(reinterpret_cast<void **>(&d_row_slot), (size_t)n_rows * 4 + 4) == cudaSuccess &&
      cudaMalloc(reinterpret_cast<void **>(&key_in), (size_t)E * 8) == cudaSuccess &&
      cudaMalloc(reinterpret_cast<void **>(&key_out), (size_t)E * 8) == cudaSuccess &&
      cudaMalloc(reinterpret_cast<void **>(&val_in), (size_t)E * 4) == cudaSuccess &&
      cudaMalloc(reinterpret_cast<void **>(&val_out), (size_t)E * 4) == cudaSuccess &&
      cudaMalloc(reinterpret_cast<void **>(&d_runs), 4) == cudaSuccess &&
      cub::DeviceRadixSort::SortPairs(nullptr, tmp_bytes, key_in, key_out, val_in, val_out, (int64_t)E, 0, bits, st) ==
          cudaSuccess &&
      cudaMalloc(&tmp, tmp_bytes ? tmp_bytes : 16) == cudaSuccess &&
      cudaMemcpyAsync(pl->hub_col_ids, cols.data(), cols.size() * 4, cudaMemcpyHostToDevice, st) == cudaSuccess &&
      cudaMemcpyAsync(pl->hub_row_ids, rows.data(), rows.size() * 4, cudaMemcpyHostToDevice, st) == cudaSuccess &&
      cudaMemcpyAsync(d_col_slot, col_slot.data(), (size_t)G * 4, cudaMemcpyHostToDevice, st) == cudaSuccess &&
      cudaMemcpyAsync(d_row_slot, row_slot.data(), (size_t)n_rows * 4, cudaMemcpyHostToDevice, st) == cudaSuccess &&
      cudaMemsetAsync(pl->dense, 0, pl->dense_floats * 4, st) == cudaSuccess;
  const unsigned blocks = (unsigned)std::min<uint64_t>(((uint64_t)E + 255) / 256, (uint64_t)sm_count() * 32);
  if (ok) {
    plan_hybrid_keys_kernel<<<blocks, 256, 0, st>>>(offsets, indices, slot_of, index_base, n_rows, E, pl->slab_rows,
                                                    (uint32_t)pl->slabs, d_col_slot, d_row_slot, pl->lda_c, dc_cells,
                                                    pl->lda_r, key_in, val_in);
    count_launch();
    ok = cub::DeviceRadixSort::SortPairs(tmp, tmp_bytes, key_in, key_out, val_in, val_out, (int64_t)E, 0, bits, st) ==
         cudaSuccess;
  }
  if (ok) {
    const unsigned kb = (unsigned)std::min<uint64_t>((n_keys + 256) / 256, (uint64_t)sm_count() * 32);
    plan_offsets_kernel<uint64_t><<<kb, 256, 0, st>>>(key_out, E, (uint32_t)n_keys, pl->voff);
    count_launch();
    std::vector<uint32_t> h(pl->slabs + 1);
    ok = cudaStreamSynchronize(st) == cudaSuccess;
    for (int s = 0; s <= pl->slabs && ok; s++)
      ok = cudaMemcpy(&h[s], pl->voff + (size_t)s * n_rows, 4, cudaMemcpyDeviceToHost) == cudaSuccess;
    for (int s = 0; s <= pl->slabs; s++)
      pl->slab_edge[s] = h[s];
  }
  const uint32_t n_res = (uint32_t)pl->slab_edge[pl->slabs], n_dense = E - n_res;
  if (ok && n_res) {
    plan_pairs_kernel<<<blocks, 256, 0, st>>>(val_out, indices, weight, slot_of, index_base, n_res, pl->pairs);
    count_launch();
  }
  if (ok && n_dense) {
    uint32_t n_runs = 0;
    size_t b1 = 0, b2 = 0;
    ok = cub::DeviceRunLengthEncode::Encode(nullptr, b1, key_out + n_res, key_in, val_in, d_runs, (int64_t)n_dense,
                                            st) == cudaSuccess &&
         cub::DeviceScan::ExclusiveSum(nullptr, b2, val_in, d_col_slot, (int64_t)n_dense, st) == cudaSuccess;
    if (ok && std::max(b1, b2) > tmp_bytes) {
      cudaFree(tmp);
      tmp_bytes = std::max(b1, b2);
      ok = cudaMalloc(&tmp, tmp_bytes) == cudaSuccess;
    }
    uint32_t *run_start = nullptr;
    ok = ok && cudaMalloc(reinterpret_cast<void **>(&run_start), (size_t)n_dense * 4) == cudaSuccess &&
         cub::DeviceRunLengthEncode::Encode(tmp, b1, key_out + n_res, key_in, val_in, d_runs, (int64_t)n_dense, st) ==
             cudaSuccess &&
         cudaMemcpyAsync(&n_runs, d_runs, 4, cudaMemcpyDeviceToHost, st) == cudaSuccess &&
         cudaStreamSynchronize(st) == cudaSuccess &&
         cub::DeviceScan::ExclusiveSum(tmp, b2, val_in, run_start, (int64_t)n_runs, st) == cudaSuccess;
    if (ok) {
      const unsigned rb = (unsigned)std::min<uint64_t>(((uint64_t)n_runs * 32 + 255) / 256, (uint64_t)sm_count() * 32);
      plan_cell_sum_kernel<<<rb, 256, 0, st>>>(key_in, run_start, val_in, n_runs, val_out + n_res, weight, n_keys,
                                               pl->dense);
      count_launch();
      ok = cudaStreamSynchronize(st) == cudaSuccess;
    }
    cudaFree(run_start);
  }
  cudaFree(key_in), cudaFree(key_out), cudaFree(val_in), cudaFree(val_out), cudaFree(tmp);
  cudaFree(d_col_slot), cudaFree(d_row_slot), cudaFree(d_runs);
  return ok;
}

nts_gather_plan *nts_gather_plan_create(const nts_vid_t *offsets, const nts_vid_t *indices, const float *weight,
                                        const nts_vid_t *slot_of, nts_vid_t index_base, nts_vid_t n_rows,
                                        uint64_t n_edges, nts_vid_t gather_rows, int n_slabs, void *stream) {
  return nts_gather_plan_create_hybrid(offsets, indices, weight, slot_of, index_base, n_rows, n_edges, gather_rows,
                                       n_slabs, 0, 0, stream);
}

nts_gather_plan *nts_gather_plan_create_hybrid(const nts_vid_t *offsets, const nts_vid_t *indices,
                                               const float *weight, const nts_vid_t *slot_of, nts_vid_t index_base,
                                               nts_vid_t n_rows, uint64_t n_edges, nts_vid_t gather_rows, int n_slabs,
                                               int n_hub_cols, int n_hub_rows, void *stream) {
  auto bad = [](const char *m) -> nts_gather_plan * {
    fail(-1, m, __FILE__, __LINE__);
    return nullptr;
  };
  if (n_edges >= 0xffffffffull)
    return bad("chunk edge count must fit uint32 offsets");
  if (n_rows && n_edges && !(offsets && indices))
    return bad("null graph array");
  if (n_hub_cols < 0 || n_hub_rows < 0)
    return bad("negative hub count");
  if (n_slabs < 1)
    n_slabs = 1;
  if (gather_rows == 0)
    n_slabs = 1;
  if ((uint64_t)n_slabs * n_rows >= 0xffffffffull)
    return bad("slabs * rows must fit 32-bit segment keys");
  cudaStream_t st = as_stream(stream);
  nts_gather_plan *pl = new nts_gather_plan();
  pl->n_rows = n_rows;
  pl->n_edges = n_edges;
  pl->gather_rows = gather_rows;
  pl->slabs = n_slabs;
  pl->slab_rows = gather_rows ? (gather_rows + n_slabs - 1) / n_slabs : 1;
  pl->slab_edge.assign(n_slabs + 1, 0);
  if (n_rows == 0 || n_edges == 0)
    return pl;
  const uint32_t E = (uint32_t)n_edges;
  const uint32_t n_keys = (uint32_t)n_slabs * n_rows;
  uint32_t *key_in = nullptr, *key_out = nullptr, *val_in = nullptr, *val_out = nullptr;
  void *tmp = nullptr;
  const bool hubs = gather_rows > 0 && (n_hub_cols > 0 || n_hub_rows > 0);
  bool ok = hubs || (cudaMalloc(reinterpret_cast<void **>(&pl->pairs), (size_t)E * sizeof(uint2)) == cudaSuccess &&
                     cudaMalloc(reinterpret_cast<void **>(&pl->voff), ((size_t)n_keys + 1) * sizeof(uint32_t)) ==
                         cudaSuccess);
  const unsigned blocks = (unsigned)std::min<uint64_t>(((uint64_t)E + 255) / 256, (uint64_t)sm_count() * 32);
  if (hubs) {
    ok = build_hybrid(pl, offsets, indices, weight, slot_of, index_base, n_hub_cols, n_hub_rows, st);
  } else if (ok && n_slabs == 1) {
    plan_pairs_kernel<<<blocks, 256, 0, st>>>(nullptr, indices, weight, slot_of, index_base, E, pl->pairs);
    count_launch();
    ok = cudaMemcpyAsync(pl->voff, offsets, ((size_t)n_rows + 1) * sizeof(uint32_t), cudaMemcpyDeviceToDevice, st) ==
         cudaSuccess;
    pl->slab_edge[0] = 0;
    pl->slab_edge[1] = n_edges;
  } else if (ok) {
    size_t tmp_bytes = 0;
    int bits = 1;
    while (bits < 32 && (1ull << bits) < (uint64_t)n_keys)
      bits++;
    ok = cudaMalloc(reinterpret_cast<void **>(&key_in), (size_t)E * 4) == cudaSuccess &&
         cudaMalloc(reinterpret_cast<void **>(&key_out), (size_t)E * 4) == cudaSuccess &&
         cudaMalloc(reinterpret_cast<void **>(&val_in), (size_t)E * 4) == cudaSuccess &&
         cudaMalloc(reinterpret_cast<void **>(&val_out), (size_t)E * 4) == cudaSuccess &&
         cub::DeviceRadixSort::SortPairs(nullptr, tmp_bytes, key_in, key_out, val_in, val_out, (int64_t)E, 0, bits, st) ==
             cudaSuccess &&
         cudaMalloc(&tmp, tmp_bytes ? tmp_bytes : 16) == cudaSuccess;
    if (ok) {
      plan_keys_kernel<<<blocks, 256, 0, st>>>(offsets, indices, slot_of, index_base, n_rows, E, pl->slab_rows,
                                               (uint32_t)n_slabs, key_in, val_in);
      count_launch();
      ok = cub::DeviceRadixSort::SortPairs(tmp, tmp_bytes, key_in, key_out, val_in, val_out, (int64_t)E, 0, bits, st) ==
           cudaSuccess;
    }
    if (ok) {
      plan_pairs_kernel<<<blocks, 256, 0, st>>>(val_out, indices, weight, slot_of, index_base, E, pl->pairs);
      count_launch();
      const unsigned kb = (unsigned)std::min<uint64_t>(((uint64_t)n_keys + 256) / 256, (uint64_t)sm_count() * 32);
      plan_offsets_kernel<uint32_t><<<kb, 256, 0, st>>>(key_out, E, n_keys, pl->voff);
      count_launch();
      std::vector<uint32_t> h(n_slabs + 1);
      ok = cudaStreamSynchronize(st) == cudaSuccess;
      for (int s = 0; s <= n_slabs && ok; s++)
        ok = cudaMemcpy(&h[s], pl->voff + (size_t)s * n_rows, 4, cudaMemcpyDeviceToHost) == cudaSuccess;
      for (int s = 0; s <= n_slabs; s++)
        pl->slab_edge[s] = h[s];
    }
  }
  if (ok)
    ok = cudaStreamSynchronize(st) == cudaSuccess && cudaGetLastError() == cudaSuccess;
  cudaFree(key_in), cudaFree(key_out), cudaFree(val_in), cudaFree(val_out), cudaFree(tmp);
  if (!ok) {
    nts_gather_plan_destroy(pl);
    fail(-1, "nts_gather_plan_create: device allocation or preprocessing failed", __FILE__, __LINE__);
    return nullptr;
  }
  return pl;
}

static nts_gather_plan *build_plan_parts(const nts_plan_part *parts, int n_parts, nts_vid_t n_rows, nts_vid_t gather_rows,
                                         int n_slabs, cudaStream_t st) {
  auto bad = [](const char *m) -> nts_gather_plan * {
    fail(-1, m, __FILE__, __LINE__);
    return nullptr;
  };
  uint64_t total = 0;
  for (int k = 0; k < n_parts; k++) {
    if (parts[k].n_edges && !(parts[k].offsets && parts[k].indices))
      return bad("null graph array in a plan part");
    if ((uint64_t)parts[k].row_add + parts[k].n_rows > n_rows)
      return bad("plan part rows exceed the output rows");
    total += parts[k].n_edges;
  }
  if (total >= 0xffffffffull)
    return bad("merged edge count must fit uint32 offsets");
  if (n_slabs < 1 || gather_rows == 0)
    n_slabs = 1;
  if ((uint64_t)n_slabs * n_rows >= 0xffffffffull)
    return bad("slabs * rows must fit 32-bit segment keys");
  nts_gather_plan *pl = new nts_gather_plan();
  pl->n_rows = n_rows;
  pl->n_edges = total;
  pl->gather_rows = gather_rows;
  pl->slabs = n_slabs;
  pl->slab_rows = gather_rows ? (gather_rows + n_slabs - 1) / n_slabs : 1;
  pl->slab_edge.assign(n_slabs + 1, 0);
  if (n_rows == 0 || total == 0)
    return pl;
  const uint32_t E = (uint32_t)total, n_keys = (uint32_t)n_slabs * n_rows;
  uint32_t *key_in = nullptr, *key_out = nullptr, *val_in = nullptr, *val_out = nullptr;
  uint2 *unsorted = nullptr;
  void *tmp = nullptr;
  size_t tmp_bytes = 0;
  int bits = 1;
  while (bits < 32 && (1ull << bits) < (uint64_t)n_keys)
    bits++;
  bool ok = cudaMalloc(reinterpret_cast<void **>(&pl->pairs), (size_t)E * sizeof(uint2)) == cudaSuccess &&
            cudaMalloc(reinterpret_cast<void **>(&pl->voff), ((size_t)n_keys + 1) * sizeof(uint32_t)) == cudaSuccess &&
            cudaMalloc(reinterpret_cast<void **>(&unsorted), (size_t)E * sizeof(uint2)) == cudaSuccess &&
            cudaMalloc(reinterpret_cast<void **>(&key_in), (size_t)E * 4) == cudaSuccess &&
            cudaMalloc(reinterpret_cast<void **>(&key_out), (size_t)E * 4) == cudaSuccess &&
            cudaMalloc(reinterpret_cast<void **>(&val_in), (size_t)E * 4) == cudaSuccess &&
            cudaMalloc(reinterpret_cast<void **>(&val_out), (size_t)E * 4) == cudaSuccess &&
            cub::DeviceRadixSort::SortPairs(nullptr, tmp_bytes, key_in, key_out, val_in, val_out, (int64_t)E, 0, bits, st) ==
                cudaSuccess &&
            cudaMalloc(&tmp, tmp_bytes ? tmp_bytes : 16) == cudaSuccess;
  uint32_t e_off = 0;
  for (int k = 0; k < n_parts && ok; k++) {
    const nts_plan_part &pt = parts[k];
    if (!pt.n_edges)
      continue;
    const unsigned blocks = (unsigned)std::min<uint64_t>((pt.n_edges + 255) / 256, (uint64_t)sm_count() * 32);
    plan_part_keys_kernel<<<blocks, 256, 0, st>>>(pt.offsets, pt.indices, pt.slot_of, pt.weight, pt.index_base,
                                                  pt.index_add, pt.n_rows, pt.row_add, (uint32_t)pt.n_edges, e_off, n_rows,
                                                  pl->slab_rows, (uint32_t)n_slabs, key_in, val_in, unsorted);
    count_launch();
    e_off += (uint32_t)pt.n_edges;
  }
  if (ok)
    ok = cub::DeviceRadixSort::SortPairs(tmp, tmp_bytes, key_in, key_out, val_in, val_out, (int64_t)E, 0, bits, st) ==
         cudaSuccess;
  if (ok) {
    const unsigned blocks = (unsigned)std::min<uint64_t>(((uint64_t)E + 255) / 256, (uint64_t)sm_count() * 32);
    plan_permute_pairs_kernel<<<blocks, 256, 0, st>>>(val_out, unsorted, E, pl->pairs);
    count_launch();
    const unsigned kb = (unsigned)std::min<uint64_t>(((uint64_t)n_keys + 256) / 256, (uint64_t)sm_count() * 32);
    plan_offsets_kernel<uint32_t><<<kb, 256, 0, st>>>(key_out, E, n_keys, pl->voff);
    count_launch();
    std::vector<uint32_t> h(n_slabs + 1);
    ok = cudaStreamSynchronize(st) == cudaSuccess;
    for (int s = 0; s <= n_slabs && ok; s++)
      ok = cudaMemcpy(&h[s], pl->voff + (size_t)s * n_rows, 4, cudaMemcpyDeviceToHost) == cudaSuccess;
    for (int s = 0; s <= n_slabs; s++)
      pl->slab_edge[s] = h[s];
  }
  if (ok)
    ok = cudaStreamSynchronize(st) == cudaSuccess && cudaGetLastError() == cudaSuccess;
  cudaFree(key_in), cudaFree(key_out), cudaFree(val_in), cudaFree(val_out), cudaFree(tmp), cudaFree(unsorted);
  if (!ok) {
    fail(-1, "nts_gather_plan_create_parts: device allocation or preprocessing failed", __FILE__, __LINE__);
    cudaFree(pl->pairs), cudaFree(pl->voff);
    delete pl;
    return nullptr;
  }
  return pl;
}

nts_gather_plan *nts_plan_create_parts_typed(const nts_plan_part *parts, int n_parts, nts_vid_t n_rows,
                                             nts_vid_t gather_rows, int n_slabs, nts_vid_t feature_size, int bf16,
                                             void *stream) {
  if (!parts || n_parts < 1) {
    fail(-1, "no plan parts", __FILE__, __LINE__);
    return nullptr;
  }
  cudaStream_t st = as_stream(stream);
  if (n_slabs >= 1)
    return build_plan_parts(parts, n_parts, n_rows, gather_rows, n_slabs, st);
  uint64_t total = 0;
  for (int k = 0; k < n_parts; k++)
    total += parts[k].n_edges;
  const uint64_t row_bytes = bf16 ? ((feature_size + 7ull) & ~7ull) * 2ull : ((feature_size + 3ull) & ~3ull) * 4ull;
  const int s_max = pick_slabs_for_rows(gather_rows, total, n_rows, row_bytes, 16ull << 20);
  nts_gather_plan *best = build_plan_parts(parts, n_parts, n_rows, gather_rows, 1, st);
  if (!best || s_max <= 1 || total == 0 || feature_size == 0)
    return best;
  float *x = nullptr, *y = nullptr;
  cudaEvent_t e0 = nullptr, e1 = nullptr;
  const size_t xb = (size_t)gather_rows * feature_size * (bf16 ? 2 : sizeof(float)),
               yb = (size_t)n_rows * feature_size * sizeof(float);
  bool ok = cudaMalloc(reinterpret_cast<void **>(&x), xb) == cudaSuccess &&
            cudaMalloc(reinterpret_cast<void **>(&y), yb) == cudaSuccess &&
            cudaMemsetAsync(x, 0, xb, st) == cudaSuccess && cudaMemsetAsync(y, 0, yb, st) == cudaSuccess &&
            cudaEventCreate(&e0) == cudaSuccess && cudaEventCreate(&e1) == cudaSuccess;
  auto time_plan = [&](nts_gather_plan *pl, float *ms) -> bool {
    *ms = 1e30f;
    for (int it = 0; it < 3; it++) {
      float t = 0.f;
      if (cudaEventRecord(e0, st) != cudaSuccess ||
          (bf16 ? run_plan_bf16(pl, x, NTS_DTYPE_BF16, feature_size, y, feature_size, st)
                : run_plan(pl, x, y, feature_size, st)) != 0 ||
          cudaEventRecord(e1, st) != cudaSuccess || cudaEventSynchronize(e1) != cudaSuccess ||
          cudaEventElapsedTime(&t, e0, e1) != cudaSuccess)
        return false;
      if (it > 0 && t < *ms)
        *ms = t;
    }
    return true;
  };
  float best_ms = 0.f;
  ok = ok && time_plan(best, &best_ms);
  for (int s = 2; ok; s *= 2) {
    const int cand = s > s_max ? s_max : s;
    nts_gather_plan *pl = build_plan_parts(parts, n_parts, n_rows, gather_rows, cand, st);
    float ms = 0.f;
    if (!pl || !time_plan(pl, &ms)) {
      nts_gather_plan_destroy(pl);
      break;
    }
    if (ms < best_ms) {
      nts_gather_plan_destroy(best);
      best = pl;
      best_ms = ms;
    } else {
      nts_gather_plan_destroy(pl);
      if (ms > 1.1f * best_ms)
        break;
    }
    if (cand == s_max)
      break;
  }
  cudaFree(x), cudaFree(y);
  if (e0)
    cudaEventDestroy(e0);
  if (e1)
    cudaEventDestroy(e1);
  best->tuned_ms = best_ms;
  return best;
}

nts_gather_plan *nts_gather_plan_create_parts(const nts_plan_part *parts, int n_parts, nts_vid_t n_rows,
                                              nts_vid_t gather_rows, int n_slabs, nts_vid_t feature_size, void *stream) {
  return nts_plan_create_parts_typed(parts, n_parts, n_rows, gather_rows, n_slabs, feature_size, 0, stream);
}

float nts_gather_plan_tuned_ms(const nts_gather_plan *pl) { return pl ? pl->tuned_ms : 0.f; }

static constexpr double kHubFloor = 0.05;
static constexpr int kHubMax = 512;

static nts_gather_plan *create_tuned(const nts_vid_t *offsets, const nts_vid_t *indices, const float *weight,
                                     const nts_vid_t *slot_of, nts_vid_t index_base, nts_vid_t n_rows, uint64_t n_edges,
                                     nts_vid_t gather_rows, nts_vid_t feature_size, bool bf16, void *stream) {
  cudaStream_t st = as_stream(stream);
  const uint64_t row_bytes = bf16 ? ((feature_size + 7ull) & ~7ull) * 2ull : ((feature_size + 3ull) & ~3ull) * 4ull;
  const int s_max = pick_slabs_for_rows(gather_rows, n_edges, n_rows, row_bytes, 16ull << 20);
  const char *hub_env = getenv("NTS_PLAN_HUBS");
  const bool try_hubs = !(hub_env && strcmp(hub_env, "0") == 0) && n_rows > 0 && gather_rows > 0;
  nts_gather_plan *best = nts_gather_plan_create(offsets, indices, weight, slot_of, index_base, n_rows, n_edges,
                                                 gather_rows, 1, stream);
  if (!best || (s_max <= 1 && !try_hubs) || n_edges == 0 || feature_size == 0)
    return best;
  float *x = nullptr, *y = nullptr;
  cudaEvent_t e0 = nullptr, e1 = nullptr;
  const size_t xb = (size_t)gather_rows * feature_size * (bf16 ? 2 : sizeof(float)),
               yb = (size_t)n_rows * feature_size * sizeof(float);
  bool ok = cudaMalloc(reinterpret_cast<void **>(&x), xb) == cudaSuccess &&
            cudaMalloc(reinterpret_cast<void **>(&y), yb) == cudaSuccess &&
            cudaMemsetAsync(x, 0, xb, st) == cudaSuccess && cudaMemsetAsync(y, 0, yb, st) == cudaSuccess &&
            cudaEventCreate(&e0) == cudaSuccess && cudaEventCreate(&e1) == cudaSuccess;
  auto run_one = [&](nts_gather_plan *pl) {
    return bf16 ? run_plan_bf16(pl, x, NTS_DTYPE_BF16, feature_size, y, feature_size, st)
                : run_plan(pl, x, y, feature_size, st);
  };
  auto time_plan = [&](nts_gather_plan *pl, float *ms) -> bool {
    *ms = 1e30f;
    for (int it = 0; it < 3; it++) {
      float t = 0.f;
      if (cudaEventRecord(e0, st) != cudaSuccess || run_one(pl) != 0 ||
          cudaEventRecord(e1, st) != cudaSuccess || cudaEventSynchronize(e1) != cudaSuccess ||
          cudaEventElapsedTime(&t, e0, e1) != cudaSuccess)
        return false;
      if (it > 0 && t < *ms)
        *ms = t;
    }
    return true;
  };
  float best_ms = 0.f;
  ok = ok && time_plan(best, &best_ms);
  auto consider = [&](int s, int hc, int hr, float *ms) -> int {
    nts_gather_plan *pl = nts_gather_plan_create_hybrid(offsets, indices, weight, slot_of, index_base, n_rows, n_edges,
                                                        gather_rows, s, hc, hr, stream);
    if (!pl || !time_plan(pl, ms)) {
      nts_gather_plan_destroy(pl);
      return -1;
    }
    if (*ms < best_ms) {
      nts_gather_plan_destroy(best);
      best = pl;
      best_ms = *ms;
      return 1;
    }
    nts_gather_plan_destroy(pl);
    return 0;
  };
  for (int s = 2; ok && s_max > 1; s *= 2) {
    const int cand = s > s_max ? s_max : s;
    float ms = 0.f;
    const int r = consider(cand, 0, 0, &ms);
    if (r < 0 || (r == 0 && ms > 1.1f * best_ms))
      break;
    if (cand == s_max)
      break;
  }
  if (ok && try_hubs) {
    std::vector<uint32_t> col_cnt, seg;
    ok = hub_counts(offsets, indices, slot_of, index_base, n_rows, (uint32_t)n_edges, gather_rows, col_cnt, seg, st);
    int n_c = 0, n_r = 0;
    for (uint32_t c : col_cnt)
      n_c += c > kHubFloor * n_rows;
    for (uint32_t s : seg)
      n_r += s > kHubFloor * gather_rows;
    const int plain_slabs = best->slabs;
    float ms = 0.f;
    for (int c = 32; ok && c <= std::min(n_c, kHubMax); c *= 2)
      if (consider(best->slabs, c, 0, &ms) != 1)
        break;
    for (int r = 32; ok && r <= std::min(n_r, kHubMax); r *= 2)
      if (consider(best->slabs, best->hub_cols, r, &ms) != 1)
        break;
    if (best->hub_cols || best->hub_rows) {
      const int hc = best->hub_cols, hr = best->hub_rows;
      for (int s : {plain_slabs / 2, std::min(plain_slabs * 2, s_max)})
        if (s >= 1 && s != plain_slabs && s != best->slabs)
          consider(s, hc, hr, &ms);
    }
  }
  cudaFree(x), cudaFree(y);
  if (e0)
    cudaEventDestroy(e0);
  if (e1)
    cudaEventDestroy(e1);
  best->tuned_ms = best_ms;
  return best;
}

nts_gather_plan *nts_gather_plan_create_tuned(const nts_vid_t *offsets, const nts_vid_t *indices, const float *weight,
                                              const nts_vid_t *slot_of, nts_vid_t index_base, nts_vid_t n_rows,
                                              uint64_t n_edges, nts_vid_t gather_rows, nts_vid_t feature_size,
                                              void *stream) {
  return create_tuned(offsets, indices, weight, slot_of, index_base, n_rows, n_edges, gather_rows, feature_size, false,
                      stream);
}

nts_gather_plan *nts_gather_plan_create_tuned_bf16(const nts_vid_t *offsets, const nts_vid_t *indices,
                                                   const float *weight, const nts_vid_t *slot_of, nts_vid_t index_base,
                                                   nts_vid_t n_rows, uint64_t n_edges, nts_vid_t gather_rows,
                                                   nts_vid_t feature_size, void *stream) {
  return create_tuned(offsets, indices, weight, slot_of, index_base, n_rows, n_edges, gather_rows, feature_size, true,
                      stream);
}

int nts_gather_plan_destroy(nts_gather_plan *pl) {
  if (!pl)
    return 0;
  cudaFree(pl->pairs);
  cudaFree(pl->voff);
  cudaFree(pl->workspace);
  cudaFree(pl->workspace_bf16);
  cudaFree(pl->dense);
  cudaFree(pl->hub_col_ids);
  cudaFree(pl->hub_row_ids);
  delete pl;
  return 0;
}

int nts_gather_plan_slabs(const nts_gather_plan *pl) { return pl ? pl->slabs : 0; }

int nts_gather_plan_hubs(const nts_gather_plan *pl, int *cols, int *rows) {
  NTS_ARG_CHECK(pl != nullptr, "null plan");
  if (cols)
    *cols = pl->hub_cols;
  if (rows)
    *rows = pl->hub_rows;
  return 0;
}

uint64_t nts_gather_plan_bytes(const nts_gather_plan *pl) {
  if (!pl)
    return 0;
  return pl->n_edges * 8ull + ((uint64_t)pl->slabs * pl->n_rows + 1) * 4ull + pl->workspace_floats * 4ull +
         pl->workspace_bf16_elems * 2ull + pl->dense_floats * 4ull + ((uint64_t)pl->hub_cols + pl->hub_rows) * 4ull;
}

int nts_gather_plan_last_launch(const nts_gather_plan *pl, int *launches, int *grid, int *k, int *u, int *outv) {
  NTS_ARG_CHECK(pl != nullptr, "null plan");
  if (launches)
    *launches = pl->last_launches;
  if (grid)
    *grid = pl->last_grid;
  if (k)
    *k = pl->last_k;
  if (u)
    *u = pl->last_u;
  if (outv)
    *outv = pl->last_outv;
  return 0;
}

int nts_gather_plan_run(nts_gather_plan *pl, const float *input, float *output, nts_vid_t feature_size, void *stream) {
  NTS_ARG_CHECK(pl != nullptr, "null plan");
  return run_plan(pl, input, output, feature_size, as_stream(stream));
}

int nts_gather_plan_run_bf16(nts_gather_plan *pl, const void *input, int input_dtype, float *output,
                             nts_vid_t feature_size, void *stream) {
  NTS_ARG_CHECK(pl != nullptr, "null plan");
  return run_plan_bf16(pl, input, input_dtype, feature_size, output, feature_size, as_stream(stream));
}

int nts_rows_to_bf16(const void *src, int src_dtype, nts_vid_t lds, void *dst, nts_vid_t n_rows, nts_vid_t feature_size,
                     nts_vid_t ld, void *stream) {
  NTS_ARG_CHECK((src && dst) || n_rows == 0 || feature_size == 0, "null pointer passed to nts_rows_to_bf16");
  return to_bf16_rows(src, src_dtype, lds, dst, n_rows, feature_size, ld, as_stream(stream));
}

int nts_gather_plan_set_variant(int variant) {
  NTS_ARG_CHECK(variant == 0 || variant == 1, "variant must be 0 (register staging) or 1 (TMA row staging)");
  g_plan_variant = variant;
  return 0;
}

int nts_gather_plan_set_tuning(int u, int min_blocks, int edges_per_warp) {
  NTS_ARG_CHECK(u >= 0 && min_blocks >= 0 && edges_per_warp >= 0 && edges_per_warp <= 4096, "bad tuning point");
  g_plan_u = u;
  g_plan_minb = min_blocks;
  g_plan_q = edges_per_warp;
  return 0;
}

}
```

### neutronstarlite_b200/exchange.py

```python
from __future__ import annotations

import numpy as np
import torch
import torch.distributed as dist

from . import _lib
from . import ops


def _ptr(t):
    return 0 if t is None else t.data_ptr()


class ExchangePlan:

    def __init__(self, pg, group=None, merged=True):
        self.pg = pg
        self.P = pg.partitions
        self.p = pg.partition_id
        self.group = group
        P, p = self.P, self.p
        chunks = pg.graph_chunks
        dev = chunks[0].column_offset_gpu.device if chunks[0].column_offset_gpu is not None else torch.device("cpu")
        self.device = dev
        self.need = [None] * P
        self.csc_slots = [None] * P
        self.csr_offsets_compact = [None] * P
        for i in range(P):
            c = chunks[i]
            ro = self._arr(c, "row_offset").to(torch.int64)
            deg = ro[1:] - ro[:-1]
            active = torch.nonzero(deg > 0).view(-1)
            self.need[i] = active.to(torch.int32)
            if i != p:
                slot_of = torch.zeros(c.batch_size_backward, dtype=torch.int32, device=dev)
                slot_of[active] = torch.arange(active.numel(), dtype=torch.int32, device=dev)
                ri = self._arr(c, "row_indices").to(torch.int64) - c.src_range[0]
                self.csc_slots[i] = slot_of[ri] if ri.numel() else torch.zeros(0, dtype=torch.int32, device=dev)
                self.csr_offsets_compact[i] = torch.cat([ro[active], ro[-1:]]).to(torch.int32)
        self.need_count = [int(n.numel()) for n in self.need]
        self.send_rows = [None] * P
        counts_in = torch.tensor([self.need_count[i] if i != p else 0 for i in range(P)], dtype=torch.int64)
        counts_out = torch.zeros(P, dtype=torch.int64)
        if P > 1:
            cdev = dev if dist.get_backend(group) == "nccl" else torch.device("cpu")
            ci, co = counts_in.to(cdev), counts_out.to(cdev)
            dist.all_to_all_single(co, ci, group=group)
            counts_out = co.cpu()
            send = torch.cat([self.need[i] if i != p else self.need[i][:0] for i in range(P)]).to(cdev)
            recv = torch.zeros(int(counts_out.sum()), dtype=torch.int32, device=cdev)
            dist.all_to_all_single(recv, send, output_split_sizes=counts_out.tolist(),
                                   input_split_sizes=counts_in.tolist(), group=group)
            pos = 0
            for j in range(P):
                n = int(counts_out[j])
                self.send_rows[j] = recv[pos:pos + n].to(dev)
                pos += n
        self.send_count = [0 if r is None else int(r.numel()) for r in self.send_rows]
        if P == 1:
            self.send_rows = [None]
        self.recv_total = sum(self.need_count[i] for i in range(P) if i != p)
        self.send_total = sum(self.send_count[j] for j in range(P) if j != p)
        rows = [self.send_rows[j] for j in range(P) if j != p and self.send_rows[j] is not None]
        self.send_rows_all = torch.cat(rows).contiguous() if rows else torch.zeros(0, dtype=torch.int32, device=dev)
        self.remote_edges = sum(int(chunks[i].edge_size) for i in range(P) if i != p)
        self.remote_col_offset = self.remote_slots = self.remote_w = None
        self.bwd_offsets = self.bwd_indices = self.bwd_w = None
        self.recv_offs = np.concatenate([[0], np.cumsum([self.need_count[i] if i != p else 0 for i in range(P)])])
        if merged:
            self._merge_remote()

    def _merge_remote(self):
        P, p, dev = self.P, self.p, self.device
        chunks = self.pg.graph_chunks
        self.recv_offs = np.concatenate([[0], np.cumsum([self.need_count[i] if i != p else 0 for i in range(P)])])
        self.remote_edges = 0
        self.remote_col_offset = self.remote_slots = self.remote_w = None
        self.bwd_offsets = self.bwd_indices = self.bwd_w = None
        self.send_rows_all = None
        if P == 1:
            return
        Vp = self.pg.owned_vertices
        dsts, slots, ws, b_off, b_idx, b_w = [], [], [], [], [], []
        edge_base = 0
        for i in range(P):
            if i == p:
                continue
            c = chunks[i]
            if c.edge_size:
                co = self._arr(c, "column_offset").to(torch.int64)
                dsts.append(torch.repeat_interleave(torch.arange(Vp, device=dev), co[1:] - co[:-1]))
                slots.append(self.csc_slots[i].to(torch.int64) + int(self.recv_offs[i]))
                ws.append(self._farr(c, "edge_weight_forward"))
                b_idx.append(self._arr(c, "column_indices"))
                b_w.append(self._farr(c, "edge_weight_backward"))
            b_off.append(self.csr_offsets_compact[i][:-1].to(torch.int64) + edge_base)
            edge_base += c.edge_size
        self.remote_edges = edge_base
        if edge_base:
            dst = torch.cat(dsts)
            order = torch.argsort(dst, stable=True)
            self.remote_slots = torch.cat(slots)[order].to(torch.int32)
            self.remote_w = torch.cat(ws)[order].contiguous()
            col = torch.zeros(Vp + 1, dtype=torch.int64, device=dev)
            col[1:] = torch.cumsum(torch.bincount(dst, minlength=Vp), 0)
            self.remote_col_offset = col.to(torch.int32)
            self.bwd_indices = torch.cat(b_idx).contiguous()
            self.bwd_w = torch.cat(b_w).contiguous()
        self.bwd_offsets = torch.cat(b_off + [torch.tensor([edge_base], dtype=torch.int64, device=dev)]).to(torch.int32)
        rows = [self.send_rows[j] for j in range(P) if j != p and self.send_rows[j] is not None]
        self.send_rows_all = torch.cat(rows).contiguous() if rows else torch.zeros(0, dtype=torch.int32, device=dev)

    @staticmethod
    def _farr(c, name):
        g = getattr(c, name + "_gpu")
        if g is not None:
            return g
        return torch.from_numpy(getattr(c, name))

    @staticmethod
    def _arr(c, name):
        g = getattr(c, name + "_gpu")
        if g is not None:
            return g
        return torch.from_numpy(getattr(c, name).view(np.int32))

    def push_offsets(self):
        P, p = self.P, self.p
        if P == 1:
            return [0], [0]
        mine = [self.need_count[i] if i != p else 0 for i in range(P)]
        allc = [None] * P
        dist.all_gather_object(allc, mine, group=self.group)
        fwd = [int(sum(allc[j][i] for i in range(p) if i != j)) if j != p else 0 for j in range(P)]
        bwd = [int(sum(allc[j][i] for j in range(p) if j != i)) if i != p else 0 for i in range(P)]
        return fwd, bwd

    def ring(self):
        return [(self.p + s) % self.P for s in range(1, self.P)]


class GpuExchange:

    def __init__(self, pg, transport="nccl", group=None, n_buffers=None):
        if not torch.cuda.is_available():
            raise _lib.NtsError("GpuExchange needs a CUDA device (libnts_b200 has no CPU fallback)")
        self.pg = pg
        self.P, self.p = pg.partitions, pg.partition_id
        self.group = group
        self.plan = ExchangePlan(pg, group, merged=(transport != "p2p"))
        self.transport = transport
        self.device = self.plan.device
        self.comm_stream = torch.cuda.Stream(device=self.device)
        self._staging = {}
        self._p2p = None
        if transport == "p2p" and self.P > 1:
            import os
            nb = n_buffers if n_buffers else int(os.environ.get("NTS_EXCHANGE_BUFFERS", "2"))
            self._p2p = _PeerWindows(self, n_buffers=nb)
        elif transport not in ("nccl", "p2p"):
            raise ValueError("transport must be 'nccl' or 'p2p'")

    def close(self):
        if self._p2p is not None:
            self._p2p.close()
            self._p2p = None

    def _buf(self, key, rows, F, dtype=torch.float32):
        t = self._staging.get((key, F))
        if t is None or t.shape[0] < rows:
            t = torch.empty((max(rows, 1), F), dtype=dtype, device=self.device)
            self._staging[(key, F)] = t
        return t[:rows]

    def _merged_plan(self, direction, F):
        plans = self.__dict__.setdefault("_bf16_merged", {})
        pl = plans.get((direction, F))
        if pl is None:
            plan, Vp = self.plan, self.pg.owned_vertices
            if direction == "fwd":
                pl = ops.GatherPlan(plan.remote_col_offset, plan.remote_slots, plan.remote_w, 0, Vp,
                                    plan.remote_edges, plan.recv_total, 0, tune_for=F, gather_dtype=torch.bfloat16)
            else:
                pl = ops.GatherPlan(plan.bwd_offsets, plan.bwd_indices, plan.bwd_w,
                                    self.pg.graph_chunks[self.p].dst_range[0], plan.recv_total, plan.remote_edges,
                                    Vp, 0, tune_for=F, gather_dtype=torch.bfloat16)
            plans[(direction, F)] = pl
        return pl

    def forward(self, x, gather_dtype=None):
        pg, plan, P, p = self.pg, self.plan, self.P, self.p
        bf16 = ops._check_gather_dtype(gather_dtype) is not None
        F = x.shape[1]
        y = torch.zeros((pg.owned_vertices, F), dtype=torch.float32, device=x.device)
        cur = torch.cuda.current_stream()
        if P == 1:
            return ops.gather_by_dst_from_src(pg.graph_chunks[0], y, x, gather_dtype=gather_dtype)
        if self._p2p is not None:
            return self._forward_p2p(x, y, bf16)
        if bf16:
            return self._forward_nccl_bf16(x, y)
        send = self._buf("fsend", plan.send_total, F)
        recv = self._buf("frecv", plan.recv_total, F)
        if plan.send_total:
            _lib.call("nts_gather_rows", _ptr(send), _ptr(x), _ptr(plan.send_rows_all), plan.send_total, F,
                      cur.cuda_stream)
        self.comm_stream.wait_stream(cur)
        with torch.cuda.stream(self.comm_stream):
            in_split = [plan.send_count[j] if j != p else 0 for j in range(P)]
            out_split = [plan.need_count[i] if i != p else 0 for i in range(P)]
            dist.all_to_all_single(recv, send, output_split_sizes=out_split, input_split_sizes=in_split,
                                   group=self.group)
        ops.gather_by_dst_from_src(pg.graph_chunks[p], y, x)
        cur.wait_stream(self.comm_stream)
        recv.record_stream(cur)
        self._aggregate_remote(y, recv)
        return y

    def _forward_nccl_bf16(self, x, y):
        pg, plan, P, p = self.pg, self.plan, self.P, self.p
        F = x.shape[1]
        cur = torch.cuda.current_stream()
        xb = x if x.dtype == torch.bfloat16 else x.to(torch.bfloat16)
        send = self._buf("fsend16", plan.send_total, F, torch.bfloat16)
        recv = self._buf("frecv16", plan.recv_total, F, torch.bfloat16)
        if plan.send_total:
            torch.index_select(xb, 0, plan.send_rows_all, out=send)
        self.comm_stream.wait_stream(cur)
        with torch.cuda.stream(self.comm_stream):
            in_split = [plan.send_count[j] if j != p else 0 for j in range(P)]
            out_split = [plan.need_count[i] if i != p else 0 for i in range(P)]
            dist.all_to_all_single(recv, send, output_split_sizes=out_split, input_split_sizes=in_split,
                                   group=self.group)
        ops.gather_by_dst_from_src(pg.graph_chunks[p], y, xb, gather_dtype=torch.bfloat16)
        cur.wait_stream(self.comm_stream)
        recv.record_stream(cur)
        if plan.remote_edges:
            self._merged_plan("fwd", F).run(recv, y, torch.bfloat16)
        return y

    def _backward_nccl_bf16(self, g, dx):
        pg, plan, P, p = self.pg, self.plan, self.P, self.p
        F = g.shape[1]
        cur = torch.cuda.current_stream()
        gb = g.to(torch.bfloat16)
        send = self._buf("bsend", plan.recv_total, F)
        recv = self._buf("brecv", plan.send_total, F)
        send.zero_()
        if plan.remote_edges:
            self._merged_plan("bwd", F).run(gb, send, torch.bfloat16)
        self.comm_stream.wait_stream(cur)
        with torch.cuda.stream(self.comm_stream):
            in_split = [plan.need_count[i] if i != p else 0 for i in range(P)]
            out_split = [plan.send_count[j] if j != p else 0 for j in range(P)]
            dist.all_to_all_single(recv, send, output_split_sizes=out_split, input_split_sizes=in_split,
                                   group=self.group)
        ops.gather_by_src_from_dst(pg.graph_chunks[p], dx, gb, gather_dtype=torch.bfloat16)
        cur.wait_stream(self.comm_stream)
        recv.record_stream(cur)
        if plan.send_total:
            _lib.call("nts_scatter_add_rows_atomic", _ptr(dx), _ptr(recv), _ptr(plan.send_rows_all), plan.send_total, F,
                      cur.cuda_stream)
        return dx

    def _aggregate_remote(self, y, staged):
        plan = self.plan
        if not plan.remote_edges:
            return
        ev = ops._timer.bracket("fwd", staged.shape[1], plan.remote_edges, self.pg.owned_vertices) if ops._timer else None
        if ev:
            ev[0].record()
        _lib.call("nts_segment_gather_sum", _ptr(staged), _ptr(y), _ptr(plan.remote_w), _ptr(plan.remote_slots),
                  _ptr(plan.remote_col_offset), 0, self.pg.owned_vertices, plan.remote_edges, staged.shape[1],
                  torch.cuda.current_stream().cuda_stream)
        if ev:
            ev[1].record()

    def _partial_remote(self, out_rows, g):
        plan = self.plan
        if not plan.remote_edges:
            return
        ev = ops._timer.bracket("bwd", g.shape[1], plan.remote_edges, out_rows.shape[0]) if ops._timer else None
        if ev:
            ev[0].record()
        _lib.call("nts_segment_gather_sum", _ptr(g), _ptr(out_rows), _ptr(plan.bwd_w), _ptr(plan.bwd_indices),
                  _ptr(plan.bwd_offsets), self.pg.graph_chunks[self.p].dst_range[0], out_rows.shape[0],
                  plan.remote_edges, g.shape[1], torch.cuda.current_stream().cuda_stream)
        if ev:
            ev[1].record()

    def fetch_mirrors(self, x):
        plan, P, p = self.plan, self.P, self.p
        F = x.shape[1]
        cur = torch.cuda.current_stream()
        M = sum(plan.need_count)
        mirror = torch.zeros((M, F), dtype=torch.float32, device=x.device)
        if self._p2p is not None:
            self._p2p.reserve(F)
            _lib.call("nts_exchange_fetch_mirrors", self._p2p.handle, _ptr(x), _ptr(mirror), F, cur.cuda_stream)
            return mirror
        if P == 1:
            if M:
                _lib.call("nts_gather_rows", _ptr(mirror), _ptr(x), _ptr(plan.need[0]), M, F, cur.cuda_stream)
            return mirror
        rows_out = [plan.send_rows[j] if j != p else plan.need[p] for j in range(P)]
        n_out = [int(r.numel()) for r in rows_out]
        send = self._buf("msend", sum(n_out), F)
        pos = 0
        for j in range(P):
            if n_out[j]:
                _lib.call("nts_gather_rows", _ptr(send[pos:pos + n_out[j]]), _ptr(x), _ptr(rows_out[j]), n_out[j], F,
                          cur.cuda_stream)
            pos += n_out[j]
        dist.all_to_all_single(mirror, send, output_split_sizes=list(plan.need_count), input_split_sizes=n_out,
                               group=self.group)
        return mirror

    def return_mirror_grads(self, gm):
        pg, plan, P, p = self.pg, self.plan, self.P, self.p
        F = gm.shape[1]
        cur = torch.cuda.current_stream()
        dx = torch.zeros((pg.owned_vertices, F), dtype=torch.float32, device=gm.device)
        if self._p2p is not None:
            self._p2p.reserve(F)
            _lib.call("nts_exchange_return_mirror_grads", self._p2p.handle, _ptr(gm.contiguous()), _ptr(dx), F,
                      cur.cuda_stream)
            return dx
        if P == 1:
            if gm.shape[0]:
                _lib.call("nts_scatter_add_rows", _ptr(dx), _ptr(gm), _ptr(plan.need[0]), gm.shape[0], F,
                          cur.cuda_stream)
            return dx
        rows_in = [plan.send_rows[j] if j != p else plan.need[p] for j in range(P)]
        n_in = [int(r.numel()) for r in rows_in]
        recv = self._buf("mrecv", sum(n_in), F)
        dist.all_to_all_single(recv, gm.contiguous(), output_split_sizes=n_in,
                               input_split_sizes=list(plan.need_count), group=self.group)
        pos = 0
        for j in range(P):
            if n_in[j]:
                _lib.call("nts_scatter_add_rows", _ptr(dx), _ptr(recv[pos:pos + n_in[j]]), _ptr(rows_in[j]), n_in[j],
                          F, cur.cuda_stream)
            pos += n_in[j]
        return dx

    def backward(self, g, gather_dtype=None):
        pg, plan, P, p = self.pg, self.plan, self.P, self.p
        bf16 = ops._check_gather_dtype(gather_dtype) is not None
        F = g.shape[1]
        dx = torch.zeros((pg.owned_vertices, F), dtype=torch.float32, device=g.device)
        cur = torch.cuda.current_stream()
        if P == 1:
            return ops.gather_by_src_from_dst(pg.graph_chunks[0], dx, g, gather_dtype=gather_dtype)
        if self._p2p is not None:
            return self._backward_p2p(g, dx, bf16)
        if bf16:
            return self._backward_nccl_bf16(g, dx)
        send = self._buf("bsend", plan.recv_total, F)
        recv = self._buf("brecv", plan.send_total, F)
        send.zero_()
        self._partial_remote(send, g)
        self.comm_stream.wait_stream(cur)
        with torch.cuda.stream(self.comm_stream):
            in_split = [plan.need_count[i] if i != p else 0 for i in range(P)]
            out_split = [plan.send_count[j] if j != p else 0 for j in range(P)]
            dist.all_to_all_single(recv, send, output_split_sizes=out_split, input_split_sizes=in_split,
                                   group=self.group)
        ops.gather_by_src_from_dst(pg.graph_chunks[p], dx, g)
        cur.wait_stream(self.comm_stream)
        recv.record_stream(cur)
        if plan.send_total:
            _lib.call("nts_scatter_add_rows_atomic", _ptr(dx), _ptr(recv), _ptr(plan.send_rows_all), plan.send_total, F,
                      cur.cuda_stream)
        return dx

    def _forward_p2p(self, x, y, bf16=False):
        self._p2p.reserve(x.shape[1], bf16)
        ev = ops._timer.bracket("fwd", x.shape[1], self.pg.owned_edges, self.pg.owned_vertices) if ops._timer else None
        if ev:
            ev[0].record()
        if bf16:
            _lib.call("nts_exchange_forward_bf16", self._p2p.handle, _ptr(x), ops._DTYPE_CODE[x.dtype], _ptr(y),
                      x.shape[1], torch.cuda.current_stream().cuda_stream)
        else:
            _lib.call("nts_exchange_forward", self._p2p.handle, _ptr(x), _ptr(y), x.shape[1],
                      torch.cuda.current_stream().cuda_stream)
        if ev:
            ev[1].record()
        return y

    def _backward_p2p(self, g, dx, bf16=False):
        self._p2p.reserve(g.shape[1], bf16)
        ev = ops._timer.bracket("bwd", g.shape[1], self.pg.owned_edges, self.pg.owned_vertices) if ops._timer else None
        if ev:
            ev[0].record()
        _lib.call("nts_exchange_backward_bf16" if bf16 else "nts_exchange_backward", self._p2p.handle, _ptr(g),
                  _ptr(dx), g.shape[1], torch.cuda.current_stream().cuda_stream)
        if ev:
            ev[1].record()
        return dx


class _PeerWindows:

    def __init__(self, ex, n_buffers=2):
        import ctypes as C
        self.ex = ex
        P, p = ex.P, ex.p
        pg, plan = ex.pg, ex.plan
        L = _lib.load()
        self.n_buffers = int(n_buffers)
        fwd_off, bwd_off = plan.push_offsets()
        c = pg.graph_chunks[p]
        u32 = C.c_uint32 * P
        chunks = (_lib.ExchangeChunk * P)()
        for i in range(P):
            if i == p:
                continue
            ci = pg.graph_chunks[i]
            h = chunks[i]
            h.column_offset, h.slots = _ptr(ci.column_offset_gpu), _ptr(plan.csc_slots[i])
            h.weight_forward, h.weight_backward = _ptr(ci.edge_weight_forward_gpu), _ptr(ci.edge_weight_backward_gpu)
            h.row_offset_compact, h.column_indices = _ptr(plan.csr_offsets_compact[i]), _ptr(ci.column_indices_gpu)
            h.edges = int(ci.edge_size)
        self._keep = {
            "need_count": u32(*[plan.need_count[i] if i != p else 0 for i in range(P)]),
            "send_count": u32(*[plan.send_count[j] if j != p else 0 for j in range(P)]),
            "fwd_off": u32(*fwd_off), "bwd_off": u32(*bwd_off), "chunks": chunks,
        }
        d = _lib.ExchangeDesc()
        d.partitions, d.rank = P, p
        d.owned_vertices, d.dst_start = pg.owned_vertices, c.dst_range[0]
        d.local_column_offset, d.local_row_indices = _ptr(c.column_offset_gpu), _ptr(c.row_indices_gpu)
        d.local_row_offset, d.local_column_indices = _ptr(c.row_offset_gpu), _ptr(c.column_indices_gpu)
        d.local_weight_forward, d.local_weight_backward = _ptr(c.edge_weight_forward_gpu), _ptr(c.edge_weight_backward_gpu)
        d.local_edges = c.edge_size
        d.chunks = chunks
        d.need_count = self._keep["need_count"]
        d.send_count = self._keep["send_count"]
        d.send_rows_all = _ptr(plan.send_rows_all)
        d.fwd_push_offset = self._keep["fwd_off"]
        d.bwd_push_offset = self._keep["bwd_off"]
        d.local_need, d.local_need_count = _ptr(plan.need[p]), plan.need_count[p]
        self.handle = L.nts_exchange_create(C.byref(d))
        if not self.handle:
            raise _lib.NtsError("nts_exchange_create failed: " + L.nts_last_error().decode())

    def _cpu_collective(self):
        return dist.get_backend(self.ex.group) != "nccl"

    def reserve(self, F, bf16=False):
        import ctypes as C
        L = _lib.load()
        ex = self.ex
        required = L.nts_exchange_required_floats_bf16 if bf16 else L.nts_exchange_required_floats
        seen = "_max_F16" if bf16 else "_max_F"
        if required(self.handle, F) <= L.nts_exchange_capacity_floats(self.handle) and F <= getattr(self, seen, 0):
            return
        cdev = torch.device("cpu") if self._cpu_collective() else ex.device
        need = torch.tensor([required(self.handle, F)], dtype=torch.int64, device=cdev)
        dist.all_reduce(need, op=dist.ReduceOp.MAX, group=ex.group)
        setattr(self, seen, max(F, getattr(self, seen, 0)))
        if int(need.item()) <= L.nts_exchange_capacity_floats(self.handle):
            return
        _lib.call("nts_exchange_release_peers", self.handle)
        dist.barrier(group=ex.group)
        _lib.call("nts_exchange_reserve", self.handle, int(need.item()), self.n_buffers)
        wh, fh = C.create_string_buffer(64), C.create_string_buffer(64)
        _lib.call("nts_exchange_handles", self.handle, wh, fh)
        handles = [None] * ex.P
        dist.all_gather_object(handles, (bytes(wh.raw), bytes(fh.raw)), group=ex.group)
        _lib.call("nts_exchange_open_peers", self.handle, b"".join(h[0] for h in handles),
                  b"".join(h[1] for h in handles))
        dist.barrier(group=ex.group)

    def close(self):
        if getattr(self, "handle", None):
            _lib.load().nts_exchange_destroy(self.handle)
            self.handle = None

    def __del__(self):
        try:
            self.close()
        except Exception:
            pass


def default_exchange(pg):
    ex = pg.__dict__.get("_default_exchange")
    if ex is None:
        ex = GpuExchange(pg, transport="nccl")
        pg.__dict__["_default_exchange"] = ex
    return ex
```

### neutronstarlite_b200/ops.py

```python
from __future__ import annotations

import ctypes as C
import time as _time

import torch

from . import _lib


def _stream():
    return torch.cuda.current_stream().cuda_stream


def _check_input(t, name="input"):
    if not t.is_cuda:
        raise _lib.NtsError("%s must be a CUDA tensor (libnts_b200 has no CPU fallback)" % name)
    if t.dtype != torch.float32 or t.dim() != 2:
        raise _lib.NtsError("%s must be a 2-D float32 tensor" % name)
    if not t.is_contiguous():
        raise _lib.NtsError("%s must be contiguous" % name)
    return t


def _check_gather_dtype(gather_dtype):
    if gather_dtype is not None and gather_dtype != torch.bfloat16:
        raise _lib.NtsError("gather_dtype must be None or torch.bfloat16, not %s" % (gather_dtype,))
    return gather_dtype


def _check_gathered(t, name, gather_dtype):
    if gather_dtype is None or (t.is_cuda and t.dtype == torch.float32):
        return _check_input(t, name)
    if not t.is_cuda:
        raise _lib.NtsError("%s must be a CUDA tensor (libnts_b200 has no CPU fallback)" % name)
    if t.dtype != torch.bfloat16 or t.dim() != 2:
        raise _lib.NtsError("%s must be a 2-D float32 or bfloat16 tensor" % name)
    if not t.is_contiguous():
        raise _lib.NtsError("%s must be contiguous" % name)
    return t


_DTYPE_CODE = {torch.float32: 0, torch.bfloat16: 1}


def _ptr(t):
    return 0 if t is None else t.data_ptr()


class KernelTimer:

    def __init__(self):
        self.records = []

    def bracket(self, tag, F, edges, rows):
        start = torch.cuda.Event(enable_timing=True)
        stop = torch.cuda.Event(enable_timing=True)
        self.records.append((tag, int(F), int(edges), int(rows), start, stop))
        return start, stop

    def summary(self):
        torch.cuda.synchronize()
        out = {}
        for tag, F, edges, rows, a, b in self.records:
            d = out.setdefault((tag, F), {"calls": 0, "ms": 0.0, "edges": 0, "rows": 0})
            d["calls"] += 1
            d["ms"] += a.elapsed_time(b)
            d["edges"] += edges
            d["rows"] += rows
        return out


_timer = None


def set_kernel_timer(timer):
    global _timer
    _timer = timer


class _timed:

    def __init__(self, tag, F, edges, rows):
        self.ev = _timer.bracket(tag, F, edges, rows) if _timer else None

    def __enter__(self):
        if self.ev:
            self.ev[0].record()

    def __exit__(self, *exc):
        if self.ev:
            self.ev[1].record()
        return False


def segment_gather_sum(out, x, weight, indices, offsets, index_base, n_rows, n_edges):
    _lib.call("nts_segment_gather_sum", _ptr(x), _ptr(out), _ptr(weight), _ptr(indices), _ptr(offsets),
              int(index_base), int(n_rows), int(n_edges), int(x.shape[1]), _stream())
    return out


class GatherPlan:

    def __init__(self, offsets, indices, weight, index_base, n_rows, n_edges, gather_rows, slabs, slot_of=None,
                 tune_for=0, hubs=(0, 0), gather_dtype=None):
        L = _lib.load()
        _check_gather_dtype(gather_dtype)
        t0 = _time.perf_counter()
        if slabs > 0:
            self.handle = L.nts_gather_plan_create_hybrid(_ptr(offsets), _ptr(indices), _ptr(weight), _ptr(slot_of),
                                                          int(index_base), int(n_rows), int(n_edges),
                                                          int(gather_rows), int(slabs), int(hubs[0]), int(hubs[1]),
                                                          _stream())
        else:
            create = L.nts_gather_plan_create_tuned_bf16 if gather_dtype is not None else L.nts_gather_plan_create_tuned
            self.handle = create(_ptr(offsets), _ptr(indices), _ptr(weight), _ptr(slot_of), int(index_base),
                                 int(n_rows), int(n_edges), int(gather_rows), int(tune_for), _stream())
        self.build_s = _time.perf_counter() - t0
        if not self.handle:
            raise _lib.NtsError("nts_gather_plan_create failed: " + L.nts_last_error().decode(errors="replace"))
        self.slabs = int(L.nts_gather_plan_slabs(self.handle))
        hc, hr = C.c_int(0), C.c_int(0)
        _lib.call("nts_gather_plan_hubs", self.handle, C.byref(hc), C.byref(hr))
        self.hub_cols, self.hub_rows = hc.value, hr.value
        self.n_rows, self.n_edges = int(n_rows), int(n_edges)

    def key(self):
        return (self.slabs,) + ((self.hub_cols, self.hub_rows) if self.hub_cols or self.hub_rows else ())

    def run(self, x, out, gather_dtype=None):
        if _check_gather_dtype(gather_dtype) is not None:
            if x.dtype not in _DTYPE_CODE:
                raise _lib.NtsError("BF16 gathers take a float32 or bfloat16 input, not %s" % x.dtype)
            _lib.call("nts_gather_plan_run_bf16", self.handle, _ptr(x), _DTYPE_CODE[x.dtype], _ptr(out),
                      int(x.shape[1]), _stream())
            return out
        if x.dtype == torch.bfloat16:
            raise _lib.NtsError("a bfloat16 input needs gather_dtype=torch.bfloat16")
        _lib.call("nts_gather_plan_run", self.handle, _ptr(x), _ptr(out), int(x.shape[1]), _stream())
        return out

    def bytes(self):
        return int(_lib.load().nts_gather_plan_bytes(self.handle))

    def __del__(self):
        try:
            if getattr(self, "handle", None):
                _lib.load().nts_gather_plan_destroy(self.handle)
                self.handle = None
        except Exception:
            pass


import os as _os

PLAN_MIN_EDGES = 1 << 20
_plan_mode = {"0": "off", "1": "on"}.get(_os.environ.get("NTS_PLAN", ""), "auto")
_plan_slabs = int(_os.environ.get("NTS_PLAN_SLABS", "0"))


def set_plan_mode(mode, slabs=0):
    global _plan_mode, _plan_slabs
    if mode not in ("auto", "on", "off"):
        raise ValueError("plan mode must be auto, on or off")
    _plan_mode, _plan_slabs = mode, int(slabs)


def _chunk_plan(chunk, direction, F, gather_dtype=None):
    if gather_dtype is None and (_plan_mode == "off" or (_plan_mode == "auto" and chunk.edge_size < PLAN_MIN_EDGES)):
        return None
    if direction == "fwd":
        n_rows, gather_rows = chunk.batch_size_forward, chunk.batch_size_backward
    else:
        n_rows, gather_rows = chunk.batch_size_backward, chunk.batch_size_forward
    plans = chunk.__dict__.setdefault("_gather_plans", {})
    tuned = chunk.__dict__.setdefault("_gather_plan_for", {})
    key = (direction, _plan_slabs) if _plan_slabs else (direction, "F", int(F))
    if gather_dtype is not None and not _plan_slabs:
        key += ("bf16",)
    plan = plans.get(key) if _plan_slabs else tuned.get(key)
    if plan is None:
        if direction == "fwd":
            plan = GatherPlan(chunk.column_offset_gpu, chunk.row_indices_gpu, chunk.edge_weight_forward_gpu,
                              chunk.src_range[0], n_rows, chunk.edge_size, gather_rows, _plan_slabs, tune_for=int(F),
                              gather_dtype=gather_dtype)
        else:
            plan = GatherPlan(chunk.row_offset_gpu, chunk.column_indices_gpu, chunk.edge_weight_backward_gpu,
                              chunk.dst_range[0], n_rows, chunk.edge_size, gather_rows, _plan_slabs, tune_for=int(F),
                              gather_dtype=gather_dtype)
        share = (direction,) + plan.key()
        if share in plans:
            plan = plans[share]
        plans[share] = plan
        if not _plan_slabs:
            tuned[key] = plan
    return plan


def _bf16_plan(chunk, direction, F, with_weight, gather_dtype):
    if _check_gather_dtype(gather_dtype) is None:
        return _chunk_plan(chunk, direction, F) if with_weight else None
    if not with_weight:
        raise _lib.NtsError("BF16 gathers always apply the edge weights (with_weight=True)")
    return _chunk_plan(chunk, direction, F, gather_dtype)


def gather_by_dst_from_src(chunk, out, x, with_weight=True, gather_dtype=None):
    plan = _bf16_plan(chunk, "fwd", x.shape[1], with_weight, gather_dtype)
    ev = _timer.bracket("fwd", x.shape[1], chunk.edge_size, chunk.batch_size_forward) if _timer else None
    if ev:
        ev[0].record()
    if plan is not None:
        plan.run(x, out, gather_dtype)
    else:
        _lib.call("nts_gather_by_dst_from_src", _ptr(x), _ptr(out), _ptr(chunk.edge_weight_forward_gpu),
                  _ptr(chunk.row_indices_gpu), _ptr(chunk.column_offset_gpu), chunk.src_range[0], chunk.src_range[1],
                  chunk.dst_range[0], chunk.dst_range[1], chunk.edge_size, chunk.batch_size_forward,
                  int(x.shape[1]), 1 if with_weight else 0, _stream())
    if ev:
        ev[1].record()
    return out


def gather_by_src_from_dst(chunk, out, grad, with_weight=True, gather_dtype=None):
    plan = _bf16_plan(chunk, "bwd", grad.shape[1], with_weight, gather_dtype)
    ev = _timer.bracket("bwd", grad.shape[1], chunk.edge_size, chunk.batch_size_backward) if _timer else None
    if ev:
        ev[0].record()
    if plan is not None:
        plan.run(grad, out, gather_dtype)
    else:
        _lib.call("nts_gather_by_src_from_dst", _ptr(grad), _ptr(out), _ptr(chunk.edge_weight_backward_gpu),
                  _ptr(chunk.row_offset_gpu), _ptr(chunk.column_indices_gpu), chunk.src_range[0], chunk.src_range[1],
                  chunk.dst_range[0], chunk.dst_range[1], chunk.edge_size, chunk.batch_size_backward,
                  int(grad.shape[1]), 1 if with_weight else 0, _stream())
    if ev:
        ev[1].record()
    return out


class ntsGraphOp:

    def __init__(self, partitioned_graph, active=None):
        self.partitioned_graph_ = partitioned_graph
        self.active_ = active

    def forward(self, f_input, f_input1=None):
        raise NotImplementedError

    def backward(self, output_grad):
        raise NotImplementedError

    def get_additional_grad(self):
        raise NotImplementedError("get_additional_grad is not implemented")


class ForwardSingleGPUfuseOp(ntsGraphOp):

    def __init__(self, partitioned_graph, active=None, gather_dtype=None):
        super().__init__(partitioned_graph, active)
        self.gather_dtype = _check_gather_dtype(gather_dtype)

    def forward(self, f_input, f_input1=None):
        x = _check_gathered(f_input, "input", self.gather_dtype)
        c = self.partitioned_graph_.graph_chunks[0]
        y = torch.zeros((c.batch_size_forward, x.shape[1]), dtype=torch.float32, device=x.device)
        return gather_by_dst_from_src(c, y, x, gather_dtype=self.gather_dtype)

    def backward(self, f_output_grad):
        g = _check_input(f_output_grad, "output_grad")
        c = self.partitioned_graph_.graph_chunks[0]
        dx = torch.zeros((c.batch_size_backward, g.shape[1]), dtype=torch.float32, device=g.device)
        return gather_by_src_from_dst(c, dx, g, gather_dtype=self.gather_dtype)


class ForwardGPUfuseOp(ntsGraphOp):

    def __init__(self, partitioned_graph, active=None, exchange=None, gather_dtype=None):
        super().__init__(partitioned_graph, active)
        self.gather_dtype = _check_gather_dtype(gather_dtype)
        if exchange is None:
            from .exchange import default_exchange
            exchange = default_exchange(partitioned_graph)
        self.exchange = exchange

    def forward(self, f_input, f_input1=None):
        x = _check_gathered(f_input, "input", self.gather_dtype)
        if self.gather_dtype is None:
            return self.exchange.forward(x)
        return self.exchange.forward(x, gather_dtype=self.gather_dtype)

    def backward(self, f_output_grad):
        g = _check_input(f_output_grad, "output_grad")
        if self.gather_dtype is None:
            return self.exchange.backward(g)
        return self.exchange.backward(g, gather_dtype=self.gather_dtype)


class _EdgeOp(ntsGraphOp):
    def _topo(self):
        pg = self.partitioned_graph_
        if pg.column_offset_gpu is None or pg.row_indices_gpu is None:
            raise _lib.NtsError("whole-partition CSC missing: call PartitionedGraph.generate_all(dist=True, device=...)")
        return pg


class DistGPUGetDepNbrOp(ntsGraphOp):

    def __init__(self, partitioned_graph, active=None, exchange=None):
        super().__init__(partitioned_graph, active)
        if exchange is None:
            from .exchange import default_exchange
            exchange = default_exchange(partitioned_graph)
        self.exchange = exchange

    def forward(self, f_input, f_input1=None):
        return self.exchange.fetch_mirrors(_check_input(f_input))

    def backward(self, f_output_grad):
        return self.exchange.return_mirror_grads(_check_input(f_output_grad, "output_grad"))


class DistGPUScatterSrc(_EdgeOp):

    def forward(self, f_input, f_input1=None):
        pg = self._topo()
        x = _check_input(f_input)
        msg = torch.zeros((pg.owned_edges, x.shape[1]), dtype=torch.float32, device=x.device)
        _lib.call("nts_scatter_src_mirror_to_msg", _ptr(msg), _ptr(x), _ptr(pg.row_indices_gpu),
                  _ptr(pg.column_offset_gpu), _ptr(pg.mirror_index_gpu), pg.owned_vertices, x.shape[1], _stream())
        return msg

    def backward(self, f_output_grad):
        pg = self._topo()
        g = _check_input(f_output_grad, "output_grad")
        out = torch.zeros((pg.owned_mirrors, g.shape[1]), dtype=torch.float32, device=g.device)
        _lib.call("nts_gather_msg_to_src_mirror", _ptr(out), _ptr(g), _ptr(pg.row_indices_gpu),
                  _ptr(pg.column_offset_gpu), _ptr(pg.mirror_index_gpu), pg.owned_vertices, g.shape[1], _stream())
        return out


class DistGPUScatterDst(_EdgeOp):

    def forward(self, f_input, f_input1=None):
        pg = self._topo()
        x = _check_input(f_input)
        msg = torch.zeros((pg.owned_edges, x.shape[1]), dtype=torch.float32, device=x.device)
        _lib.call("nts_scatter_dst_to_msg", _ptr(msg), _ptr(x), _ptr(pg.row_indices_gpu),
                  _ptr(pg.column_offset_gpu), pg.owned_vertices, x.shape[1], _stream())
        return msg

    def backward(self, f_output_grad):
        pg = self._topo()
        g = _check_input(f_output_grad, "output_grad")
        out = torch.zeros((pg.owned_vertices, g.shape[1]), dtype=torch.float32, device=g.device)
        _lib.call("nts_gather_msg_to_dst", _ptr(out), _ptr(g), _ptr(pg.row_indices_gpu),
                  _ptr(pg.column_offset_gpu), pg.owned_vertices, g.shape[1], _stream())
        return out


class DistGPUAggregateDst(_EdgeOp):

    def forward(self, f_input, f_input1=None):
        pg = self._topo()
        m = _check_input(f_input)
        out = torch.zeros((pg.owned_vertices, m.shape[1]), dtype=torch.float32, device=m.device)
        _lib.call("nts_gather_msg_to_dst", _ptr(out), _ptr(m), _ptr(pg.row_indices_gpu),
                  _ptr(pg.column_offset_gpu), pg.owned_vertices, m.shape[1], _stream())
        return out

    def backward(self, f_output_grad):
        pg = self._topo()
        g = _check_input(f_output_grad, "output_grad")
        msg = torch.zeros((pg.owned_edges, g.shape[1]), dtype=torch.float32, device=g.device)
        _lib.call("nts_scatter_dst_to_msg", _ptr(msg), _ptr(g), _ptr(pg.row_indices_gpu),
                  _ptr(pg.column_offset_gpu), pg.owned_vertices, g.shape[1], _stream())
        return msg


class DistGPUEdgeSoftMax(_EdgeOp):

    def __init__(self, partitioned_graph, active=None):
        super().__init__(partitioned_graph, active)
        self.IntermediateResult = None

    def forward(self, f_input, f_input1=None):
        pg = self._topo()
        m = _check_input(f_input)
        out = torch.zeros_like(m)
        self.IntermediateResult = torch.zeros_like(m)
        _lib.call("nts_edge_softmax_forward", _ptr(out), _ptr(m), _ptr(self.IntermediateResult),
                  _ptr(pg.row_indices_gpu), _ptr(pg.column_offset_gpu), pg.owned_vertices, m.shape[1], _stream())
        return out

    def backward(self, f_output_grad):
        pg = self._topo()
        g = _check_input(f_output_grad, "output_grad")
        out = torch.zeros_like(g)
        _lib.call("nts_edge_softmax_backward", _ptr(out), _ptr(g), _ptr(self.IntermediateResult),
                  _ptr(pg.row_indices_gpu), _ptr(pg.column_offset_gpu), pg.owned_vertices, g.shape[1], _stream())
        return out


class DistGPUAggregateDstFuseWeight(_EdgeOp):

    def __init__(self, partitioned_graph, active=None):
        super().__init__(partitioned_graph, active)
        self._mirror = None
        self._a = None
        self.e_weight_grad = None

    def forward(self, f_input, e_weight=None):
        pg = self._topo()
        x = _check_input(f_input)
        a = _check_input(e_weight, "edge weight")
        self._mirror, self._a = x, a
        heads = int(a.shape[1])
        out = torch.zeros((pg.owned_vertices, x.shape[1]), dtype=torch.float32, device=x.device)
        _lib.call("nts_segment_gather_sum_heads", _ptr(x), _ptr(out), _ptr(a), _ptr(pg.row_indices_gpu),
                  _ptr(pg.column_offset_gpu), _ptr(pg.mirror_index_gpu), 0, pg.owned_vertices, pg.owned_edges,
                  x.shape[1], heads, _stream())
        return out

    def backward(self, f_output_grad):
        pg = self._topo()
        g = _check_input(f_output_grad, "output_grad")
        dm = torch.zeros((pg.owned_mirrors, g.shape[1]), dtype=torch.float32, device=g.device)
        self.e_weight_grad = torch.zeros_like(self._a)
        _lib.call("nts_aggregate_dst_fuse_weight_backward_heads", _ptr(dm), _ptr(self.e_weight_grad),
                  _ptr(self._mirror), _ptr(self._a), _ptr(g), _ptr(pg.row_indices_gpu), _ptr(pg.column_offset_gpu),
                  _ptr(pg.mirror_index_gpu), pg.owned_vertices, g.shape[1], int(self._a.shape[1]), _stream())
        return dm

    def get_additional_grad(self):
        return self.e_weight_grad


class DistGPUFusedGATOp(_EdgeOp):

    def __init__(self, partitioned_graph, active=None, negative_slope=0.2, two_pass_backward=True, gather_dtype=None):
        super().__init__(partitioned_graph, active)
        self.slope = float(negative_slope)
        self.two_pass_backward = bool(two_pass_backward)
        self.gather_dtype = _check_gather_dtype(gather_dtype)
        if self.gather_dtype is not None and not self.two_pass_backward:
            raise _lib.NtsError("BF16 gathers of the fused GAT layer need two_pass_backward=True")
        self._saved = None

    @staticmethod
    def slot_indices(pg):
        cached = getattr(pg, "_slot_indices_gpu", None)
        if cached is None:
            cached = pg.mirror_index_gpu[pg.row_indices_gpu.long()].to(torch.int32).contiguous()
            pg._slot_indices_gpu = cached
        return cached

    @staticmethod
    def slot_csr(pg):
        cached = getattr(pg, "_slot_csr_gpu", None)
        if cached is not None:
            return cached
        col = pg.column_offset_gpu.long()
        V, M = pg.owned_vertices, pg.owned_mirrors
        slot = DistGPUFusedGATOp.slot_indices(pg).long()
        dst = torch.repeat_interleave(torch.arange(V, device=col.device), col[1:V + 1] - col[:V])
        order = torch.sort(slot, stable=True).indices
        csr_dst = dst[order].to(torch.int32).contiguous()
        off = torch.zeros(M + 1, dtype=torch.int64, device=col.device)
        off[1:] = torch.cumsum(torch.bincount(slot, minlength=M), 0)
        pg._slot_csr_gpu = (off.to(torch.int32).contiguous(), csr_dst)
        return pg._slot_csr_gpu

    def forward(self, mirror, src_score, dst_score):
        pg = self._topo()
        x = _check_input(mirror, "mirror")
        s = _check_input(src_score, "src_score")
        d = _check_input(dst_score, "dst_score")
        H = int(s.shape[1])
        seg_max = torch.empty((pg.owned_vertices, H), dtype=torch.float32, device=x.device)
        seg_sum = torch.empty_like(seg_max)
        slots = self.slot_indices(pg)
        with _timed("gat_stats", x.shape[1], pg.owned_edges, pg.owned_vertices):
            _lib.call("nts_gat_softmax_stats", _ptr(seg_max), _ptr(seg_sum), _ptr(s), _ptr(d), _ptr(slots),
                      _ptr(pg.column_offset_gpu), 0, pg.owned_vertices, H, self.slope, _stream())
        F = int(x.shape[1])
        if self.gather_dtype is not None:
            return self._forward_bf16(pg, x, s, d, seg_max, seg_sum, slots, H, F)
        xk, Fk = x, F
        if H == 1 and F % 4 != 0:
            Fk = (F + 3) // 4 * 4
            xk = torch.nn.functional.pad(x, (0, Fk - F))
        out = torch.zeros((pg.owned_vertices, Fk), dtype=torch.float32, device=x.device)
        with _timed("gat_fwd", F, pg.owned_edges, pg.owned_vertices):
            _lib.call("nts_gat_fused_aggregate_forward", _ptr(xk), _ptr(out), _ptr(s), _ptr(d), _ptr(seg_max),
                      _ptr(seg_sum), _ptr(slots), _ptr(pg.column_offset_gpu), 0,
                      pg.owned_vertices, pg.owned_edges, Fk, H, self.slope, _stream())
        if Fk != F:
            out = out[:, :F].contiguous()
        self._saved = (x, s, d, seg_max, seg_sum, out)
        return out

    @staticmethod
    def _to_bf16_rows(t, ld):
        n, F = t.shape
        r = torch.empty((n, ld), dtype=torch.bfloat16, device=t.device)
        with _timed("gat_bf16_round", F, 0, n):
            _lib.call("nts_rows_to_bf16", _ptr(t), _DTYPE_CODE[torch.float32], F, _ptr(r), n, F, ld, _stream())
        return r

    def _forward_bf16(self, pg, x, s, d, seg_max, seg_sum, slots, H, F):
        ld = (F + 7) // 8 * 8
        mt = self._to_bf16_rows(x, ld)
        out = torch.zeros((pg.owned_vertices, ld), dtype=torch.float32, device=x.device)
        with _timed("gat_fwd", F, pg.owned_edges, pg.owned_vertices):
            _lib.call("nts_gat_fused_aggregate_forward_bf16", _ptr(mt), _ptr(out), _ptr(s), _ptr(d), _ptr(seg_max),
                      _ptr(seg_sum), _ptr(slots), _ptr(pg.column_offset_gpu), 0, pg.owned_vertices, pg.owned_edges,
                      F, ld, H, self.slope, _stream())
        if ld != F:
            out = out[:, :F].contiguous()
        self._saved = (mt, s, d, seg_max, seg_sum, out)
        return out

    def _backward_bf16(self, pg, g):
        mt, s, d, seg_max, seg_sum, out = self._saved
        H = int(s.shape[1])
        M, ld = mt.shape
        F = int(out.shape[1])
        gt = self._to_bf16_rows(g, ld)
        out_dot_g = (out.detach() * gt[:, :F].float()).view(-1, H, F // H).sum(-1).contiguous()
        dm = torch.zeros((M, ld), dtype=torch.float32, device=g.device)
        ds = torch.zeros_like(s)
        dd = torch.zeros_like(d)
        slot_off, slot_dst = self.slot_csr(pg)
        pack = torch.empty((pg.owned_vertices, H, 4), dtype=torch.float32, device=g.device)
        with _timed("gat_bwd", F, 2 * pg.owned_edges, pg.owned_vertices):
            _lib.call("nts_gat_fused_aggregate_backward_two_pass_bf16", _ptr(dm), _ptr(ds), _ptr(dd), _ptr(pack),
                      _ptr(mt), _ptr(s), _ptr(d), _ptr(seg_max), _ptr(seg_sum), _ptr(out_dot_g), _ptr(gt),
                      _ptr(self.slot_indices(pg)), _ptr(pg.column_offset_gpu), 0, _ptr(slot_off), _ptr(slot_dst),
                      pg.owned_vertices, M, F, ld, H, self.slope, _stream())
        if ld != F:
            dm = dm[:, :F].contiguous()
        return dm, ds, dd

    def backward(self, f_output_grad):
        pg = self._topo()
        g = _check_input(f_output_grad, "output_grad")
        if self.gather_dtype is not None:
            return self._backward_bf16(pg, g)
        x, s, d, seg_max, seg_sum, out = self._saved
        H = int(s.shape[1])
        D = x.shape[1] // H
        out_dot_g = (out.detach() * g).view(-1, H, D).sum(-1).contiguous()
        dm = torch.zeros_like(x)
        ds = torch.zeros_like(s)
        dd = torch.zeros_like(d)
        if self.two_pass_backward:
            slot_off, slot_dst = self.slot_csr(pg)
            pack = torch.empty((pg.owned_vertices, H, 4), dtype=torch.float32, device=x.device)
            with _timed("gat_bwd", x.shape[1], 2 * pg.owned_edges, pg.owned_vertices):
                _lib.call("nts_gat_fused_aggregate_backward_two_pass", _ptr(dm), _ptr(ds), _ptr(dd), _ptr(pack),
                          _ptr(x), _ptr(s), _ptr(d), _ptr(seg_max), _ptr(seg_sum), _ptr(out_dot_g), _ptr(g),
                          _ptr(self.slot_indices(pg)), _ptr(pg.column_offset_gpu), 0,
                          _ptr(slot_off), _ptr(slot_dst), pg.owned_vertices, x.shape[0], x.shape[1], H, self.slope,
                          _stream())
            return dm, ds, dd
        _lib.call("nts_gat_fused_aggregate_backward", _ptr(dm), _ptr(ds), _ptr(dd), _ptr(x), _ptr(s), _ptr(d),
                  _ptr(seg_max), _ptr(seg_sum), _ptr(out_dot_g), _ptr(g), _ptr(pg.row_indices_gpu),
                  _ptr(pg.column_offset_gpu), _ptr(pg.mirror_index_gpu), pg.owned_vertices, x.shape[1], H,
                  self.slope, _stream())
        return dm, ds, dd
```

### neutronstarlite_b200/toolkits.py

```python
from __future__ import annotations

import math

import numpy as np
import torch
import torch.distributed as dist

from .context import NtsContext
from . import _lib, ops


class Parameter:
    def __init__(self, w, h, alpha, beta1, beta2, epsilon, weight_decay, device=None, generator=None):
        scale = math.sqrt(6.0 / (w + h))
        W = (2 * scale) * torch.rand((w, h), dtype=torch.float32, generator=generator) - scale
        self.W = W.to(device).requires_grad_(True)
        self.M = torch.zeros((w, h), dtype=torch.float32, device=device)
        self.V = torch.zeros((w, h), dtype=torch.float32, device=device)
        self.W_gradient = None
        f32 = np.float32
        self.alpha = f32(alpha)
        self.beta1, self.beta2, self.epsilon = f32(beta1), f32(beta2), f32(epsilon)
        self.alpha_t, self.beta1_t, self.beta2_t = f32(alpha), f32(beta1), f32(beta2)
        self.weight_decay = f32(weight_decay)
        self.curr_epoch = 0
        self.decay_rate, self.decay_epoch = 1, -1

    def init_parameter(self):
        if dist.is_initialized() and dist.get_world_size() > 1:
            dist.broadcast(self.W.data, src=0)

    def set_decay(self, decay_rate, decay_epoch):
        self.decay_rate, self.decay_epoch = int(decay_rate), int(decay_epoch)

    def all_reduce_to_gradient(self, grad):
        self.W_gradient = grad.detach().clone().contiguous()
        if dist.is_initialized() and dist.get_world_size() > 1:
            dist.all_reduce(self.W_gradient, op=dist.ReduceOp.SUM)

    def next(self):
        if self.decay_epoch != -1 and self.curr_epoch != 0 and self.curr_epoch % self.decay_epoch == 0:
            self.alpha_t *= self.decay_rate
        one = np.float32(1)
        self.alpha_t = np.float32(self.alpha_t)
        self.alpha = np.float32(self.alpha_t * np.sqrt(one - self.beta2) / (one - self.beta1))
        self.beta1 = np.float32(self.beta1 * self.beta1_t)
        self.beta2 = np.float32(self.beta2 * self.beta2_t)
        self.curr_epoch += 1

    def forward(self, x):
        return x.mm(self.W)

    def learn_with_decay_Adam(self):
        with torch.no_grad():
            if self.W.is_cuda:
                from . import _lib
                _lib.call("nts_adam_update", self.W.data_ptr(), self.M.data_ptr(), self.V.data_ptr(),
                          self.W_gradient.data_ptr(), self.W.numel(), float(self.weight_decay), float(self.beta1),
                          float(self.beta2), float(self.alpha), float(self.epsilon),
                          torch.cuda.current_stream().cuda_stream)
                return
            one = np.float32(1)
            W_g = self.W * float(self.weight_decay) + self.W_gradient
            self.M = float(self.beta1) * self.M + float(one - self.beta1) * W_g
            self.V = float(self.beta2) * self.V + float(one - self.beta2) * W_g * W_g
            self.W -= float(self.alpha) * self.M / (torch.sqrt(self.V) + float(self.epsilon))

    def zero_grad(self):
        self.W.grad = None


class GCNImpl:

    _input_is_gathered = True

    def __init__(self, partitioned_graph, layers, features, labels, mask, learn_rate=0.01, weight_decay=0.0001,
                 decay_rate=0.97, decay_epoch=100, drop_rate=0.5, op_class=None, op_kwargs=None, seed=0,
                 gather_dtype=None):
        self.pg = partitioned_graph
        self.layers = list(layers)
        self.device = features.device
        self.drop_rate = drop_rate
        self.ctx = NtsContext()
        gen = torch.Generator().manual_seed(seed)
        self.P = []
        for i in range(len(self.layers) - 1):
            p = Parameter(self.layers[i], self.layers[i + 1], learn_rate, 0.9, 0.999, 1e-9, weight_decay,
                          device=self.device, generator=gen)
            p.init_parameter()
            p.set_decay(decay_rate, decay_epoch)
            self.P.append(p)
        self.L_GT = labels.to(self.device)
        self.MASK = mask.to(self.device)
        self.train_rows = (self.MASK == 0).nonzero().view(-1)
        self.X = [None] * len(self.layers)
        self.gather_dtype = ops._check_gather_dtype(gather_dtype)
        if self.gather_dtype is not None and self._input_is_gathered:
            features = features.detach().to(self.gather_dtype)
        self.X[0] = features.requires_grad_(True)
        if op_class is None:
            op_class = ops.ForwardSingleGPUfuseOp if partitioned_graph.partitions == 1 else ops.ForwardGPUfuseOp
        self.op_class = op_class
        self.op_kwargs = dict(op_kwargs or {})
        if self.gather_dtype is not None:
            self.op_kwargs["gather_dtype"] = self.gather_dtype
        self.loss = None
        self.epoch = 0

    def vertexForward(self, a, x, layer):
        if layer < len(self.layers) - 2:
            return torch.relu(self.P[layer].forward(a))
        return self.P[layer].forward(a).log_softmax(1)

    def Forward(self):
        for i in range(len(self.layers) - 1):
            x_i = self.X[i]
            if i != 0 and self.drop_rate > 0:
                dropped = torch.nn.functional.dropout(x_i, self.drop_rate, training=True)
                self.ctx.appendNNOp(x_i, dropped)
                x_i = dropped
            x_i = x_i.contiguous()
            y_i = self.ctx.runGraphOp(self.op_class, self.pg, None, x_i, **self.op_kwargs)
            self.X[i + 1] = self.ctx.runVertexForward(lambda n, v, _l=i: self.vertexForward(n, v, _l), y_i, x_i)

    def Loss(self):
        a = self.X[-1]
        self.loss = torch.nn.functional.nll_loss(a.index_select(0, self.train_rows),
                                                 self.L_GT.index_select(0, self.train_rows))
        self.ctx.appendNNOp(a, self.loss)

    def Update(self):
        for p in self.P:
            p.all_reduce_to_gradient(p.W.grad)
            p.learn_with_decay_Adam()
            p.next()

    def Test(self, s):
        sel = self.MASK == s
        correct = (self.X[-1].argmax(1) == self.L_GT)[sel].sum()
        total = sel.sum()
        pair = torch.stack([correct, total]).to(torch.int64)
        if dist.is_initialized() and dist.get_world_size() > 1:
            dist.all_reduce(pair)
        return pair

    def run_epoch(self, test=False):
        if self.epoch != 0:
            for p in self.P:
                p.zero_grad()
        self.Forward()
        acc = [self.Test(s) for s in (0, 1, 2)] if test else None
        self.Loss()
        self.ctx.self_backward(True)
        self.Update()
        self.epoch += 1
        return self.loss, acc


class GCNEagerImpl(GCNImpl):

    _input_is_gathered = False

    def __init__(self, *args, **kwargs):
        super().__init__(*args, **kwargs)
        self.X[0] = self.X[0].detach()

    def vertexForward(self, a, x, layer):
        if layer == 0:
            return self.P[layer].forward(a)
        if self.drop_rate > 0:
            a = torch.nn.functional.dropout(a, self.drop_rate, training=True)
        return self.P[layer].forward(torch.relu(a))

    def Forward(self):
        for i in range(len(self.layers) - 1):
            y_i = self.ctx.runVertexForward(lambda n, v, _l=i: self.vertexForward(n, v, _l), self.X[i], self.X[i])
            self.X[i + 1] = self.ctx.runGraphOp(self.op_class, self.pg, None, y_i.contiguous(), **self.op_kwargs)

    def Loss(self):
        a = self.X[-1].log_softmax(1)
        self.loss = torch.nn.functional.nll_loss(a.index_select(0, self.train_rows),
                                                 self.L_GT.index_select(0, self.train_rows))
        self.ctx.appendNNOp(self.X[-1], self.loss)


class GATImpl:

    def __init__(self, partitioned_graph, layers, features, labels, mask, heads=8, learn_rate=0.01,
                 weight_decay=0.0001, exchange=None, seed=0, sum_fanout_grads=True, fused_kernel=False,
                 two_pass_backward=True, gather_dtype=None):
        self.pg = partitioned_graph
        self.fused_kernel = fused_kernel
        self.two_pass_backward = two_pass_backward
        self.gather_dtype = ops._check_gather_dtype(gather_dtype)
        if self.gather_dtype is not None and not (fused_kernel and two_pass_backward):
            raise _lib.NtsError("GATImpl gather_dtype needs fused_kernel=True and two_pass_backward=True")
        self.layers = list(layers)
        self.device = features.device
        self.heads = [heads] * (len(self.layers) - 2) + [1]
        self.ctx = NtsContext(sum_fanout_grads=sum_fanout_grads)
        gen = torch.Generator().manual_seed(seed)
        self.P, self.al, self.ar = [], [], []
        for i in range(len(self.layers) - 1):
            H = self.heads[i]
            D = self.layers[i + 1] // H
            assert H * D == self.layers[i + 1], "layer width must be a multiple of heads"
            mk = lambda a, b: Parameter(a, b, learn_rate, 0.9, 0.999, 1e-9, weight_decay, device=self.device,
                                        generator=gen)
            for lst, shape in ((self.P, (self.layers[i], H * D)), (self.al, (H, D)), (self.ar, (H, D))):
                prm = mk(*shape)
                prm.init_parameter()
                lst.append(prm)
        if exchange is None:
            from .exchange import GpuExchange
            exchange = GpuExchange(partitioned_graph)
        self.exchange = exchange
        self.L_GT = labels.to(self.device)
        self.MASK = mask.to(self.device)
        self.train_rows = (self.MASK == 0).nonzero().view(-1)
        self.X = [None] * len(self.layers)
        self.X[0] = features.requires_grad_(True)
        self.loss = None
        self.epoch = 0

    def params(self):
        return self.P + self.al + self.ar

    def Forward(self):
        ctx, pg = self.ctx, self.pg
        for i in range(len(self.layers) - 1):
            H = self.heads[i]
            D = self.layers[i + 1] // H
            last = i == len(self.layers) - 2
            X_trans = ctx.runVertexForward(lambda x, _i=i: self.P[_i].forward(x), self.X[i])
            mirror = ctx.runGraphOp(ops.DistGPUGetDepNbrOp, pg, None, X_trans.contiguous(), exchange=self.exchange)
            src_att = ctx.runVertexForward(
                lambda m, _i=i: (m.view(-1, H, D) * self.al[_i].W).sum(-1).contiguous(), mirror)
            dst_att = ctx.runVertexForward(
                lambda x, _i=i: (x.view(-1, H, D) * self.ar[_i].W).sum(-1).contiguous(), X_trans)
            if self.fused_kernel:
                nbr = ctx.runGraphOpN(ops.DistGPUFusedGATOp, pg, None, [mirror, src_att, dst_att],
                                      two_pass_backward=self.two_pass_backward, gather_dtype=self.gather_dtype)
            else:
                e_src = ctx.runGraphOp(ops.DistGPUScatterSrc, pg, None, src_att)
                e_dst = ctx.runGraphOp(ops.DistGPUScatterDst, pg, None, dst_att)
                e_msg = e_src + e_dst
                m = ctx.runEdgeForward(lambda t: torch.nn.functional.leaky_relu(t, 0.2), e_msg)
                a = ctx.runGraphOp(ops.DistGPUEdgeSoftMax, pg, None, m)
                nbr = ctx.runGraphOp(ops.DistGPUAggregateDstFuseWeight, pg, None, mirror, a)
            if last:
                self.X[i + 1] = ctx.runVertexForward(lambda t: t.log_softmax(1), nbr)
            else:
                self.X[i + 1] = ctx.runVertexForward(lambda t: torch.relu(t), nbr)

    def Loss(self):
        a = self.X[-1]
        self.loss = torch.nn.functional.nll_loss(a.index_select(0, self.train_rows),
                                                 self.L_GT.index_select(0, self.train_rows))
        self.ctx.appendNNOp(a, self.loss)

    def Update(self):
        for p in self.params():
            if p.W.grad is None:
                continue
            p.all_reduce_to_gradient(p.W.grad)
            p.learn_with_decay_Adam()
            p.next()

    def run_epoch(self):
        if self.epoch != 0:
            for p in self.params():
                p.zero_grad()
        self.Forward()
        self.Loss()
        self.ctx.self_backward(True)
        self.Update()
        self.epoch += 1
        return self.loss
```

Measured before the change: 14.53 billion.

## Add overwrite gather mode, multi-stage hub GEMM pipeline, and row-padded inputs

Adds a plan run entry point with an overwrite flag so single-GPU gathers write output directly instead of zeroing and then read-modify-writing it. The hub block GEMM moves from double buffering to a 4-stage cp.async pipeline in dynamic shared memory, with a selectable 64 or 128 row tile and separate store, RMW and atomic-reduce epilogues. Input features with widths that are not a multiple of 4 are row-padded so gathers can use a leading dimension and skip contiguous copies. The cost is more code paths and more shared memory per block, which can lower occupancy.

New measurement: 15.26 billion (median of 6 runs). 1.05x the previous value.

```diff
diff --git a/include/nts_b200.h b/include/nts_b200.h
--- a/include/nts_b200.h
+++ b/include/nts_b200.h
@@ -92,6 +92,9 @@
 enum { NTS_DTYPE_F32 = 0, NTS_DTYPE_BF16 = 1 };
 int nts_gather_plan_run_bf16(nts_gather_plan *plan, const void *input, int input_dtype, float *output,
                              nts_vid_t feature_size, void *stream);
+enum { NTS_PLAN_OVERWRITE = 1, NTS_PLAN_GATHER_BF16 = 2 };
+int nts_gather_plan_run_ex(nts_gather_plan *plan, const void *input, int input_dtype, nts_vid_t input_ld,
+                           float *output, nts_vid_t feature_size, int flags, void *stream);
 nts_gather_plan *nts_gather_plan_create_tuned_bf16(const nts_vid_t *offsets, const nts_vid_t *indices,
                                                    const float *weight, const nts_vid_t *slot_of, nts_vid_t index_base,
                                                    nts_vid_t n_rows, uint64_t n_edges, nts_vid_t gather_rows,
diff --git a/neutronstarlite_b200/_lib.py b/neutronstarlite_b200/_lib.py
--- a/neutronstarlite_b200/_lib.py
+++ b/neutronstarlite_b200/_lib.py
@@ -56,6 +56,7 @@
     "nts_gather_plan_bytes": (_u64, [_vp]),
     "nts_gather_plan_run": (_int, [_vp, _vp, _vp, _u32, _vp]),
     "nts_gather_plan_run_bf16": (_int, [_vp, _vp, _int, _vp, _u32, _vp]),
+    "nts_gather_plan_run_ex": (_int, [_vp, _vp, _int, _u32, _vp, _u32, _int, _vp]),
     "nts_gather_plan_create_tuned_bf16": (_vp, [_vp, _vp, _vp, _vp, _u32, _u32, _u64, _u32, _u32, _vp]),
     "nts_gather_plan_last_launch": (_int, [_vp] + [C.POINTER(_int)] * 5),
     "nts_gather_plan_set_tuning": (_int, [_int, _int, _int]),
diff --git a/neutronstarlite_b200/csrc/nts_common.cuh b/neutronstarlite_b200/csrc/nts_common.cuh
--- a/neutronstarlite_b200/csrc/nts_common.cuh
+++ b/neutronstarlite_b200/csrc/nts_common.cuh
@@ -49,7 +49,7 @@
 int sm_count();
 
 int run_plan_bf16(nts_gather_plan *pl, const void *input, int dtype, uint32_t lds, float *output, uint32_t F,
-                  cudaStream_t st);
+                  cudaStream_t st, bool overwrite = false);
 int to_bf16_rows(const void *src, int dtype, uint32_t lds, void *dst, uint32_t n_rows, uint32_t F, uint32_t ld,
                  cudaStream_t st);
 
diff --git a/neutronstarlite_b200/csrc/nts_plan.cu b/neutronstarlite_b200/csrc/nts_plan.cu
--- a/neutronstarlite_b200/csrc/nts_plan.cu
+++ b/neutronstarlite_b200/csrc/nts_plan.cu
@@ -171,13 +171,13 @@
   }
 }
 
-__global__ void pad_rows_kernel(const float *__restrict__ src, float *__restrict__ dst, uint32_t n_rows, uint32_t F,
-                                uint32_t ld) {
+__global__ void pad_rows_kernel(const float *__restrict__ src, uint32_t lds, float *__restrict__ dst, uint32_t n_rows,
+                                uint32_t F, uint32_t ld) {
   const uint64_t total = (uint64_t)n_rows * ld;
   for (uint64_t i = (uint64_t)blockIdx.x * blockDim.x + threadIdx.x; i < total; i += (uint64_t)gridDim.x * blockDim.x) {
     const uint64_t r = i / ld;
     const uint32_t c = (uint32_t)(i - r * ld);
-    dst[i] = c < F ? __ldg(src + r * F + c) : 0.f;
+    dst[i] = c < F ? __ldg(src + r * lds + c) : 0.f;
   }
 }
 
@@ -668,7 +668,8 @@
     return launch_planned<T, K_, U_, 1, B_>(pl, sh, in, ldc, out, F, Q, st);                                         \
   }
 
-constexpr int kHubBM = 128, kHubBN = 128, kHubBK = 16, kHubThreads = 256;
+constexpr int kHubBN = 128, kHubBK = 16, kHubStages = 4;
+enum { kHubRmw = 0, kHubStore = 1, kHubRed = 2 };
 
 __device__ __forceinline__ void p_cp_async16(void *smem_dst, const void *gmem_src, bool full) {
   asm volatile("cp.async.cg.shared.global [%0], [%1], 16, %2;" ::"r"(p_smem_u32(smem_dst)), "l"(gmem_src),
@@ -676,19 +677,62 @@
                : "memory");
 }
 
-template <class TB, int OUTV, bool SPLIT>
-__global__ void __launch_bounds__(kHubThreads, 2)
+template <int OUTV>
+__device__ __forceinline__ void load_add_chunk(const float *__restrict__ orow, uint32_t col, uint32_t F, float4 &a) {
+  if constexpr (OUTV == 4) {
+    const float4 o = *reinterpret_cast<const float4 *>(orow + col);
+    a.x += o.x, a.y += o.y, a.z += o.z, a.w += o.w;
+  } else if constexpr (OUTV == 2) {
+    const float2 o = *reinterpret_cast<const float2 *>(orow + col);
+    a.x += o.x, a.y += o.y;
+    if (col + 2 < F) {
+      const float2 o1 = *reinterpret_cast<const float2 *>(orow + col + 2);
+      a.z += o1.x, a.w += o1.y;
+    }
+  } else {
+    a.x += orow[col];
+    if (col + 1 < F)
+      a.y += orow[col + 1];
+    if (col + 2 < F)
+      a.z += orow[col + 2];
+    if (col + 3 < F)
+      a.w += orow[col + 3];
+  }
+}
+
+template <int OUTV>
+__device__ __forceinline__ void store_chunk(float *__restrict__ orow, uint32_t col, uint32_t F, float4 a) {
+  if constexpr (OUTV == 4) {
+    *reinterpret_cast<float4 *>(orow + col) = a;
+  } else if constexpr (OUTV == 2) {
+    *reinterpret_cast<float2 *>(orow + col) = make_float2(a.x, a.y);
+    if (col + 2 < F)
+      *reinterpret_cast<float2 *>(orow + col + 2) = make_float2(a.z, a.w);
+  } else {
+    const float v[4] = {a.x, a.y, a.z, a.w};
+#pragma unroll
+    for (int i = 0; i < 4; i++)
+      if (col + i < F)
+        orow[col + i] = v[i];
+  }
+}
+
+template <class TB, int BM, int OUTV, int EPI>
+__global__ void __launch_bounds__(2 * BM, 256 / BM)
     hub_block_gemm_kernel(const float *__restrict__ At, uint32_t lda, uint32_t M, uint32_t K, uint32_t k_split,
                           const TB *__restrict__ B, uint32_t ldb, const uint32_t *__restrict__ colmap,
                           float *__restrict__ out, uint32_t F, const uint32_t *__restrict__ rowmap, uint32_t m_tiles,
                           uint32_t n_tiles) {
+  static_assert(BM == 64 || BM == 128, "M tile of 64 or 128 rows");
+  constexpr int kThreads = 2 * BM;
   constexpr bool kBf16 = std::is_same<TB, __nv_bfloat16>::value;
   constexpr uint32_t kBV = 16 / sizeof(TB);
-  __shared__ __align__(16) float As[2][kHubBK][kHubBM];
-  __shared__ __align__(16) TB Bs[2][kHubBK][kHubBN];
+  extern __shared__ __align__(16) unsigned char hub_smem[];
+  auto As = reinterpret_cast<float(*)[kHubBK][BM]>(hub_smem);
+  auto Bs = reinterpret_cast<TB(*)[kHubBK][kHubBN]>(hub_smem + sizeof(float) * kHubStages * kHubBK * BM);
   const uint32_t t = threadIdx.x;
   const uint32_t n_tile = blockIdx.x % n_tiles, rest = blockIdx.x / n_tiles;
-  const uint32_t m0 = (rest % m_tiles) * kHubBM, n0 = n_tile * kHubBN;
+  const uint32_t m0 = (rest % m_tiles) * BM, n0 = n_tile * kHubBN;
   const uint32_t k_begin = (rest / m_tiles) * k_split;
   const uint32_t k_end = min(K, k_begin + k_split);
   if (k_begin >= k_end)
@@ -697,23 +741,24 @@
 
   auto load = [&](uint32_t kt, int buf) {
 #pragma unroll
-    for (int i = 0; i < 2; i++) {
-      const uint32_t c = t + i * kHubThreads, kk = c >> 5, c4 = (c & 31) * 4;
+    for (int i = 0; i < (int)(kHubBK * BM / 4 / kThreads); i++) {
+      constexpr uint32_t kRowChunks = BM / 4;
+      const uint32_t c = t + i * kThreads, kk = c / kRowChunks, c4 = (c % kRowChunks) * 4;
       const uint32_t k = k_begin + kt * kHubBK + kk;
       const bool a_ok = k < k_end && m0 + c4 < lda;
       p_cp_async16(&As[buf][kk][c4], a_ok ? At + (size_t)k * lda + m0 + c4 : At, a_ok);
     }
 #pragma unroll
-    for (int i = 0; i < (int)(kHubBK * kHubBN / kBV / kHubThreads); i++) {
+    for (int i = 0; i < (int)(kHubBK * kHubBN / kBV / kThreads); i++) {
       constexpr uint32_t kRowChunks = kHubBN / kBV;
-      const uint32_t c = t + i * kHubThreads, kk = c / kRowChunks, cv = (c % kRowChunks) * kBV;
+      const uint32_t c = t + i * kThreads, kk = c / kRowChunks, cv = (c % kRowChunks) * kBV;
       const uint32_t k = k_begin + kt * kHubBK + kk;
       const bool b_ok = k < k_end && n0 + cv < ldb;
       const uint32_t brow = b_ok ? (colmap ? __ldg(colmap + k) : k) : 0;
       p_cp_async16(&Bs[buf][kk][cv], B + (size_t)brow * ldb + (b_ok ? n0 + cv : 0), b_ok);
     }
-    asm volatile("cp.async.commit_group;" ::: "memory");
   };
+  auto commit = [] { asm volatile("cp.async.commit_group;" ::: "memory"); };
   auto read_b4 = [&](int buf, int kk, uint32_t n) -> float4 {
     if constexpr (kBf16) {
       const uint2 u = *reinterpret_cast<const uint2 *>(&Bs[buf][kk][n]);
@@ -724,7 +769,9 @@
     }
   };
 
-  const uint32_t tx = t & 15, ty = t >> 4;
+  const uint32_t warp = t >> 5, lane = t & 31;
+  const uint32_t am = (warp >> 1) * 32 + (lane >> 3) * 4;
+  const uint32_t bn = (warp & 1) * 64 + (lane & 7) * 4;
   float acc[8][8];
 #pragma unroll
   for (int i = 0; i < 8; i++)
@@ -732,22 +779,25 @@
     for (int j = 0; j < 8; j++)
       acc[i][j] = 0.f;
 
-  load(0, 0);
+#pragma unroll
+  for (int s = 0; s < kHubStages - 1; s++) {
+    if ((uint32_t)s < n_kt)
+      load(s, s);
+    commit();
+  }
   for (uint32_t kt = 0; kt < n_kt; kt++) {
-    const int buf = kt & 1;
-    if (kt + 1 < n_kt) {
-      load(kt + 1, buf ^ 1);
-      asm volatile("cp.async.wait_group 1;" ::: "memory");
-    } else {
-      asm volatile("cp.async.wait_group 0;" ::: "memory");
-    }
+    asm volatile("cp.async.wait_group %0;" ::"n"(kHubStages - 2) : "memory");
     __syncthreads();
+    if (kt + kHubStages - 1 < n_kt)
+      load(kt + kHubStages - 1, (kt + kHubStages - 1) % kHubStages);
+    commit();
+    const int buf = kt % kHubStages;
 #pragma unroll
     for (int kk = 0; kk < kHubBK; kk++) {
-      const float4 a0 = *reinterpret_cast<const float4 *>(&As[buf][kk][ty * 4]);
-      const float4 a1 = *reinterpret_cast<const float4 *>(&As[buf][kk][64 + ty * 4]);
-      const float4 b0 = read_b4(buf, kk, tx * 4);
-      const float4 b1 = read_b4(buf, kk, 64 + tx * 4);
+      const float4 a0 = *reinterpret_cast<const float4 *>(&As[buf][kk][am]);
+      const float4 a1 = *reinterpret_cast<const float4 *>(&As[buf][kk][am + 16]);
+      const float4 b0 = read_b4(buf, kk, bn);
+      const float4 b1 = read_b4(buf, kk, bn + 32);
       const float a[8] = {a0.x, a0.y, a0.z, a0.w, a1.x, a1.y, a1.z, a1.w};
       const float b[8] = {b0.x, b0.y, b0.z, b0.w, b1.x, b1.y, b1.z, b1.w};
 #pragma unroll
@@ -756,56 +806,108 @@
         for (int j = 0; j < 8; j++)
           acc[i][j] = fmaf(a[i], b[j], acc[i][j]);
     }
-    __syncthreads();
-  }
-
-#pragma unroll
-  for (int i = 0; i < 8; i++) {
-    const uint32_t m = m0 + (i >> 2) * 64 + ty * 4 + (i & 3);
-    if (m >= M)
-      continue;
-    float *orow = out + (size_t)(rowmap ? __ldg(rowmap + m) : m) * F;
-#pragma unroll
-    for (int j = 0; j < 2; j++) {
-      const uint32_t col = n0 + j * 64 + tx * 4;
-      if (col < F)
-        flush_chunk<OUTV, SPLIT>(orow, col, F,
-                                 make_float4(acc[i][j * 4], acc[i][j * 4 + 1], acc[i][j * 4 + 2], acc[i][j * 4 + 3]));
-    }
-  }
+  }
+
+  auto out_row = [&](int i) -> float * {
+    const uint32_t m = m0 + am + (i >> 2) * 16 + (i & 3);
+    return m < M ? out + (size_t)(rowmap ? __ldg(rowmap + m) : m) * F : nullptr;
+  };
+  auto chunk = [&](int i, int j) { return make_float4(acc[i][j * 4], acc[i][j * 4 + 1], acc[i][j * 4 + 2], acc[i][j * 4 + 3]); };
+  if constexpr (EPI == kHubRmw) {
+    float4 v[8][2];
+#pragma unroll
+    for (int i = 0; i < 8; i++) {
+      const float *orow = out_row(i);
+#pragma unroll
+      for (int j = 0; j < 2; j++) {
+        v[i][j] = chunk(i, j);
+        const uint32_t col = n0 + bn + j * 32;
+        if (orow && col < F)
+          load_add_chunk<OUTV>(orow, col, F, v[i][j]);
+      }
+    }
+#pragma unroll
+    for (int i = 0; i < 8; i++) {
+      float *orow = out_row(i);
+#pragma unroll
+      for (int j = 0; j < 2; j++) {
+        const uint32_t col = n0 + bn + j * 32;
+        if (orow && col < F)
+          store_chunk<OUTV>(orow, col, F, v[i][j]);
+      }
+    }
+  } else {
+#pragma unroll
+    for (int i = 0; i < 8; i++) {
+      float *orow = out_row(i);
+#pragma unroll
+      for (int j = 0; j < 2; j++) {
+        const uint32_t col = n0 + bn + j * 32;
+        if (orow && col < F) {
+          if constexpr (EPI == kHubStore)
+            store_chunk<OUTV>(orow, col, F, chunk(i, j));
+          else
+            flush_chunk<OUTV, true>(orow, col, F, chunk(i, j));
+        }
+      }
+    }
+  }
+}
+
+template <class TB, int BM, int OUTV, int EPI>
+static int launch_hub_gemm(uint64_t blocks, const float *At, uint32_t lda, uint32_t M, uint32_t K, uint32_t k_split,
+                           const TB *B, uint32_t ldb, const uint32_t *colmap, float *out, uint32_t F,
+                           const uint32_t *rowmap, uint32_t m_tiles, uint32_t n_tiles, cudaStream_t st) {
+  auto kern = hub_block_gemm_kernel<TB, BM, OUTV, EPI>;
+  const size_t smem = (size_t)kHubStages * kHubBK * (BM * sizeof(float) + kHubBN * sizeof(TB));
+  NTS_ARG_CHECK(blocks <= 0x7fffffffull, "hub block grid too large");
+  NTS_CUDA_OK(cudaFuncSetAttribute(kern, cudaFuncAttributeMaxDynamicSharedMemorySize, (int)smem));
+  kern<<<(unsigned)blocks, 2 * BM, smem, st>>>(At, lda, M, K, k_split, B, ldb, colmap, out, F, rowmap, m_tiles,
+                                               n_tiles);
+  NTS_LAUNCH_CHECK();
+  return 0;
 }
 
 template <class TB, int OUTV>
-static int launch_hub_blocks(nts_gather_plan *pl, const TB *in, uint32_t ldb, float *out, uint32_t F,
+static int launch_hub_blocks(nts_gather_plan *pl, const TB *in, uint32_t ldb, float *out, uint32_t F, bool overwrite,
                              cudaStream_t st) {
   const uint32_t n_tiles = (F + kHubBN - 1) / kHubBN;
   if (pl->hub_cols) {
-    const uint32_t m_tiles = (pl->n_rows + kHubBM - 1) / kHubBM;
+    const uint32_t m_tiles = (pl->n_rows + 127) / 128;
     const uint64_t blocks = (uint64_t)m_tiles * n_tiles;
-    NTS_ARG_CHECK(blocks <= 0x7fffffffull, "hub column block grid too large");
-    hub_block_gemm_kernel<TB, OUTV, false><<<(unsigned)blocks, kHubThreads, 0, st>>>(
-        pl->dense, pl->lda_c, pl->n_rows, (uint32_t)pl->hub_cols, (uint32_t)pl->hub_cols, in, ldb, pl->hub_col_ids, out,
-        F, nullptr, m_tiles, n_tiles);
-    NTS_LAUNCH_CHECK();
+    const uint32_t hc = (uint32_t)pl->hub_cols;
+    const int rc = overwrite ? launch_hub_gemm<TB, 128, OUTV, kHubStore>(blocks, pl->dense, pl->lda_c, pl->n_rows, hc,
+                                                                          hc, in, ldb, pl->hub_col_ids, out, F, nullptr,
+                                                                          m_tiles, n_tiles, st)
+                             : launch_hub_gemm<TB, 128, OUTV, kHubRmw>(blocks, pl->dense, pl->lda_c, pl->n_rows, hc,
+                                                                        hc, in, ldb, pl->hub_col_ids, out, F, nullptr,
+                                                                        m_tiles, n_tiles, st);
+    if (rc)
+      return rc;
   }
   if (pl->hub_rows) {
-    const uint32_t m_tiles = (pl->hub_rows + kHubBM - 1) / kHubBM;
+    const uint32_t hr = (uint32_t)pl->hub_rows;
+    const uint32_t bm = (hr + 63) / 64 * 64 < (hr + 127) / 128 * 128 ? 64 : 128;
+    const uint32_t m_tiles = (hr + bm - 1) / bm;
     const uint32_t K = pl->gather_rows;
-    const uint64_t want = (uint64_t)sm_count() * 2 * 4;
+    const uint64_t want = (uint64_t)sm_count() * (256 / bm) * 4;
     uint64_t splits = (want + (uint64_t)m_tiles * n_tiles - 1) / ((uint64_t)m_tiles * n_tiles);
     uint32_t k_split = (uint32_t)((K + splits - 1) / splits);
     k_split = std::max<uint32_t>((k_split + kHubBK - 1) / kHubBK * kHubBK, 16 * kHubBK);
     splits = (K + k_split - 1) / k_split;
-    hub_block_gemm_kernel<TB, OUTV, true><<<(unsigned)(splits * m_tiles * n_tiles), kHubThreads, 0, st>>>(
-        pl->dense + (size_t)pl->hub_cols * pl->lda_c, pl->lda_r, (uint32_t)pl->hub_rows, K, k_split, in, ldb, nullptr,
-        out, F, pl->hub_row_ids, m_tiles, n_tiles);
-    NTS_LAUNCH_CHECK();
+    const float *Dr = pl->dense + (size_t)pl->hub_cols * pl->lda_c;
+    const uint64_t blocks = splits * m_tiles * n_tiles;
+    return bm == 64 ? launch_hub_gemm<TB, 64, OUTV, kHubRed>(blocks, Dr, pl->lda_r, hr, K, k_split, in, ldb, nullptr,
+                                                             out, F, pl->hub_row_ids, m_tiles, n_tiles, st)
+                    : launch_hub_gemm<TB, 128, OUTV, kHubRed>(blocks, Dr, pl->lda_r, hr, K, k_split, in, ldb, nullptr,
+                                                              out, F, pl->hub_row_ids, m_tiles, n_tiles, st);
   }
   return 0;
 }
 
 template <class T>
-static int run_gather(nts_gather_plan *pl, const T *in, uint32_t ld, float *output, uint32_t F, cudaStream_t st) {
+static int run_gather(nts_gather_plan *pl, const T *in, uint32_t ld, float *output, uint32_t F, bool overwrite,
+                      cudaStream_t st) {
   constexpr bool kBf16 = std::is_same<T, __nv_bfloat16>::value;
   PlanShape sh;
   const uint32_t ldc = ld / GatherT<T>::V;
@@ -817,9 +919,9 @@
   sh.tiles = (ldc + sh.tile_vecs - 1) / sh.tile_vecs;
   sh.outv = (F % 4 == 0 && aligned_to(output, 16)) ? 4 : ((F % 2 == 0 && aligned_to(output, 8)) ? 2 : 1);
   if (pl->hub_cols || pl->hub_rows) {
-    const int rc = sh.outv == 4   ? launch_hub_blocks<T, 4>(pl, in, ld, output, F, st)
-                   : sh.outv == 2 ? launch_hub_blocks<T, 2>(pl, in, ld, output, F, st)
-                                  : launch_hub_blocks<T, 1>(pl, in, ld, output, F, st);
+    const int rc = sh.outv == 4   ? launch_hub_blocks<T, 4>(pl, in, ld, output, F, overwrite, st)
+                   : sh.outv == 2 ? launch_hub_blocks<T, 2>(pl, in, ld, output, F, overwrite, st)
+                                  : launch_hub_blocks<T, 1>(pl, in, ld, output, F, overwrite, st);
     if (rc)
       return rc;
   }
@@ -932,22 +1034,37 @@
   return 0;
 }
 
-static int run_plan(nts_gather_plan *pl, const float *input, float *output, uint32_t F, cudaStream_t st) {
+static int begin_overwrite(nts_gather_plan *pl, float *output, uint32_t F, bool *overwrite, cudaStream_t st) {
+  if (!*overwrite || pl->n_rows == 0 || F == 0)
+    return 0;
+  NTS_ARG_CHECK(output, "null feature pointer");
+  if (pl->hub_cols && pl->n_edges)
+    return 0;
+  NTS_CUDA_OK(cudaMemsetAsync(output, 0, (size_t)pl->n_rows * F * sizeof(float), st));
+  *overwrite = false;
+  return 0;
+}
+
+static int run_plan(nts_gather_plan *pl, const float *input, uint32_t lds, float *output, uint32_t F, bool overwrite,
+                    cudaStream_t st) {
+  if (const int rc = begin_overwrite(pl, output, F, &overwrite, st))
+    return rc;
   if (pl->n_rows == 0 || pl->n_edges == 0 || F == 0)
     return 0;
   NTS_ARG_CHECK(input && output, "null feature pointer");
+  NTS_ARG_CHECK(lds >= F, "row stride below the feature width");
   const uint32_t ld = (F + 3u) & ~3u;
   const float *in = input;
-  if (ld != F || !aligned_to(input, 16)) {
+  if (lds != ld || !aligned_to(input, 16)) {
     if (const int rc = ensure_workspace(pl->workspace, pl->workspace_floats, (size_t)pl->gather_rows * ld))
       return rc;
     const uint64_t total = (uint64_t)pl->gather_rows * ld;
     const unsigned blocks = (unsigned)std::min<uint64_t>((total + 255) / 256, (uint64_t)sm_count() * 32);
-    pad_rows_kernel<<<blocks, 256, 0, st>>>(input, pl->workspace, pl->gather_rows, F, ld);
+    pad_rows_kernel<<<blocks, 256, 0, st>>>(input, lds, pl->workspace, pl->gather_rows, F, ld);
     NTS_LAUNCH_CHECK();
     in = pl->workspace;
   }
-  return run_gather<float>(pl, in, ld, output, F, st);
+  return run_gather<float>(pl, in, ld, output, F, overwrite, st);
 }
 
 int to_bf16_rows(const void *src, int dtype, uint32_t lds, void *dst, uint32_t n_rows, uint32_t F, uint32_t ld,
@@ -969,21 +1086,23 @@
 }
 
 int run_plan_bf16(nts_gather_plan *pl, const void *input, int dtype, uint32_t lds, float *output, uint32_t F,
-                  cudaStream_t st) {
+                  cudaStream_t st, bool overwrite) {
   NTS_ARG_CHECK(dtype == NTS_DTYPE_F32 || dtype == NTS_DTYPE_BF16, "input dtype must be NTS_DTYPE_F32 or NTS_DTYPE_BF16");
   NTS_ARG_CHECK(g_plan_variant == 0, "the TMA row-staging variant (nts_gather_plan_set_variant(1)) gathers FP32 rows only");
+  if (const int rc = begin_overwrite(pl, output, F, &overwrite, st))
+    return rc;
   if (pl->n_rows == 0 || pl->n_edges == 0 || F == 0)
     return 0;
   NTS_ARG_CHECK(input && output, "null feature pointer");
   NTS_ARG_CHECK(lds >= F, "row stride below the feature width");
   if (dtype == NTS_DTYPE_BF16 && lds % 8 == 0 && aligned_to(input, 16))
-    return run_gather<__nv_bfloat16>(pl, static_cast<const __nv_bfloat16 *>(input), lds, output, F, st);
+    return run_gather<__nv_bfloat16>(pl, static_cast<const __nv_bfloat16 *>(input), lds, output, F, overwrite, st);
   const uint32_t ld = (F + 7u) & ~7u;
   if (const int rc = ensure_workspace(pl->workspace_bf16, pl->workspace_bf16_elems, (size_t)pl->gather_rows * ld))
     return rc;
   if (const int rc = to_bf16_rows(input, dtype, lds, pl->workspace_bf16, pl->gather_rows, F, ld, st))
     return rc;
-  return run_gather<__nv_bfloat16>(pl, pl->workspace_bf16, ld, output, F, st);
+  return run_gather<__nv_bfloat16>(pl, pl->workspace_bf16, ld, output, F, overwrite, st);
 }
 
 }
@@ -1370,7 +1489,7 @@
       float t = 0.f;
       if (cudaEventRecord(e0, st) != cudaSuccess ||
           (bf16 ? run_plan_bf16(pl, x, NTS_DTYPE_BF16, feature_size, y, feature_size, st)
-                : run_plan(pl, x, y, feature_size, st)) != 0 ||
+                : run_plan(pl, x, feature_size, y, feature_size, false, st)) != 0 ||
           cudaEventRecord(e1, st) != cudaSuccess || cudaEventSynchronize(e1) != cudaSuccess ||
           cudaEventElapsedTime(&t, e0, e1) != cudaSuccess)
         return false;
@@ -1441,8 +1560,8 @@
             cudaMemsetAsync(x, 0, xb, st) == cudaSuccess && cudaMemsetAsync(y, 0, yb, st) == cudaSuccess &&
             cudaEventCreate(&e0) == cudaSuccess && cudaEventCreate(&e1) == cudaSuccess;
   auto run_one = [&](nts_gather_plan *pl) {
-    return bf16 ? run_plan_bf16(pl, x, NTS_DTYPE_BF16, feature_size, y, feature_size, st)
-                : run_plan(pl, x, y, feature_size, st);
+    return bf16 ? run_plan_bf16(pl, x, NTS_DTYPE_BF16, feature_size, y, feature_size, st, true)
+                : run_plan(pl, x, feature_size, y, feature_size, true, st);
   };
   auto time_plan = [&](nts_gather_plan *pl, float *ms) -> bool {
     *ms = 1e30f;
@@ -1581,13 +1700,25 @@
 
 int nts_gather_plan_run(nts_gather_plan *pl, const float *input, float *output, nts_vid_t feature_size, void *stream) {
   NTS_ARG_CHECK(pl != nullptr, "null plan");
-  return run_plan(pl, input, output, feature_size, as_stream(stream));
+  return run_plan(pl, input, feature_size, output, feature_size, false, as_stream(stream));
 }
 
 int nts_gather_plan_run_bf16(nts_gather_plan *pl, const void *input, int input_dtype, float *output,
                              nts_vid_t feature_size, void *stream) {
   NTS_ARG_CHECK(pl != nullptr, "null plan");
   return run_plan_bf16(pl, input, input_dtype, feature_size, output, feature_size, as_stream(stream));
+}
+
+int nts_gather_plan_run_ex(nts_gather_plan *pl, const void *input, int input_dtype, nts_vid_t input_ld, float *output,
+                           nts_vid_t feature_size, int flags, void *stream) {
+  NTS_ARG_CHECK(pl != nullptr, "null plan");
+  const uint32_t lds = input_ld ? input_ld : feature_size;
+  NTS_ARG_CHECK((flags & ~(NTS_PLAN_OVERWRITE | NTS_PLAN_GATHER_BF16)) == 0, "unknown nts_gather_plan_run_ex flag");
+  const bool overwrite = flags & NTS_PLAN_OVERWRITE;
+  if (flags & NTS_PLAN_GATHER_BF16)
+    return run_plan_bf16(pl, input, input_dtype, lds, output, feature_size, as_stream(stream), overwrite);
+  NTS_ARG_CHECK(input_dtype == NTS_DTYPE_F32, "a BF16 input needs NTS_PLAN_GATHER_BF16");
+  return run_plan(pl, static_cast<const float *>(input), lds, output, feature_size, overwrite, as_stream(stream));
 }
 
 int nts_rows_to_bf16(const void *src, int src_dtype, nts_vid_t lds, void *dst, nts_vid_t n_rows, nts_vid_t feature_size,
diff --git a/neutronstarlite_b200/exchange.py b/neutronstarlite_b200/exchange.py
--- a/neutronstarlite_b200/exchange.py
+++ b/neutronstarlite_b200/exchange.py
@@ -192,10 +192,11 @@
         pg, plan, P, p = self.pg, self.plan, self.P, self.p
         bf16 = ops._check_gather_dtype(gather_dtype) is not None
         F = x.shape[1]
+        if P == 1:
+            y = torch.empty((pg.owned_vertices, F), dtype=torch.float32, device=x.device)
+            return ops.gather_by_dst_from_src(pg.graph_chunks[0], y, x, gather_dtype=gather_dtype, overwrite=True)
         y = torch.zeros((pg.owned_vertices, F), dtype=torch.float32, device=x.device)
         cur = torch.cuda.current_stream()
-        if P == 1:
-            return ops.gather_by_dst_from_src(pg.graph_chunks[0], y, x, gather_dtype=gather_dtype)
         if self._p2p is not None:
             return self._forward_p2p(x, y, bf16)
         if bf16:
@@ -348,10 +349,11 @@
         pg, plan, P, p = self.pg, self.plan, self.P, self.p
         bf16 = ops._check_gather_dtype(gather_dtype) is not None
         F = g.shape[1]
+        if P == 1:
+            dx = torch.empty((pg.owned_vertices, F), dtype=torch.float32, device=g.device)
+            return ops.gather_by_src_from_dst(pg.graph_chunks[0], dx, g, gather_dtype=gather_dtype, overwrite=True)
         dx = torch.zeros((pg.owned_vertices, F), dtype=torch.float32, device=g.device)
         cur = torch.cuda.current_stream()
-        if P == 1:
-            return ops.gather_by_src_from_dst(pg.graph_chunks[0], dx, g, gather_dtype=gather_dtype)
         if self._p2p is not None:
             return self._backward_p2p(g, dx, bf16)
         if bf16:
diff --git a/neutronstarlite_b200/ops.py b/neutronstarlite_b200/ops.py
--- a/neutronstarlite_b200/ops.py
+++ b/neutronstarlite_b200/ops.py
@@ -28,7 +28,17 @@
     return gather_dtype
 
 
-def _check_gathered(t, name, gather_dtype):
+def row_padded(t):
+    return t.dim() == 2 and t.stride(1) == 1 and t.stride(0) >= t.shape[1]
+
+
+def padded_rows(n_rows, F, device):
+    return torch.zeros((n_rows, (F + 3) // 4 * 4), dtype=torch.float32, device=device)[:, :F]
+
+
+def _check_gathered(t, name, gather_dtype, rows_ok=False):
+    if rows_ok and t.is_cuda and t.dtype == torch.float32 and row_padded(t):
+        return t
     if gather_dtype is None or (t.is_cuda and t.dtype == torch.float32):
         return _check_input(t, name)
     if not t.is_cuda:
@@ -41,6 +51,7 @@
 
 
 _DTYPE_CODE = {torch.float32: 0, torch.bfloat16: 1}
+_PLAN_OVERWRITE, _PLAN_GATHER_BF16 = 1, 2
 
 
 def _ptr(t):
@@ -127,16 +138,17 @@
     def key(self):
         return (self.slabs,) + ((self.hub_cols, self.hub_rows) if self.hub_cols or self.hub_rows else ())
 
-    def run(self, x, out, gather_dtype=None):
-        if _check_gather_dtype(gather_dtype) is not None:
-            if x.dtype not in _DTYPE_CODE:
-                raise _lib.NtsError("BF16 gathers take a float32 or bfloat16 input, not %s" % x.dtype)
-            _lib.call("nts_gather_plan_run_bf16", self.handle, _ptr(x), _DTYPE_CODE[x.dtype], _ptr(out),
-                      int(x.shape[1]), _stream())
-            return out
-        if x.dtype == torch.bfloat16:
+    def run(self, x, out, gather_dtype=None, overwrite=False):
+        bf16 = _check_gather_dtype(gather_dtype) is not None
+        if bf16 and x.dtype not in _DTYPE_CODE:
+            raise _lib.NtsError("BF16 gathers take a float32 or bfloat16 input, not %s" % x.dtype)
+        if not bf16 and x.dtype == torch.bfloat16:
             raise _lib.NtsError("a bfloat16 input needs gather_dtype=torch.bfloat16")
-        _lib.call("nts_gather_plan_run", self.handle, _ptr(x), _ptr(out), int(x.shape[1]), _stream())
+        if not row_padded(x):
+            raise _lib.NtsError("the gathered rows must be contiguous (row padding allowed)")
+        flags = (_PLAN_OVERWRITE if overwrite else 0) | (_PLAN_GATHER_BF16 if bf16 else 0)
+        _lib.call("nts_gather_plan_run_ex", self.handle, _ptr(x), _DTYPE_CODE[x.dtype] if bf16 else 0,
+                  int(x.stride(0)), _ptr(out), int(x.shape[1]), flags, _stream())
         return out
 
     def bytes(self):
@@ -204,14 +216,17 @@
     return _chunk_plan(chunk, direction, F, gather_dtype)
 
 
-def gather_by_dst_from_src(chunk, out, x, with_weight=True, gather_dtype=None):
+def gather_by_dst_from_src(chunk, out, x, with_weight=True, gather_dtype=None, overwrite=False):
     plan = _bf16_plan(chunk, "fwd", x.shape[1], with_weight, gather_dtype)
     ev = _timer.bracket("fwd", x.shape[1], chunk.edge_size, chunk.batch_size_forward) if _timer else None
     if ev:
         ev[0].record()
     if plan is not None:
-        plan.run(x, out, gather_dtype)
+        plan.run(x, out, gather_dtype, overwrite)
     else:
+        x = x.contiguous()
+        if overwrite:
+            out.zero_()
         _lib.call("nts_gather_by_dst_from_src", _ptr(x), _ptr(out), _ptr(chunk.edge_weight_forward_gpu),
                   _ptr(chunk.row_indices_gpu), _ptr(chunk.column_offset_gpu), chunk.src_range[0], chunk.src_range[1],
                   chunk.dst_range[0], chunk.dst_range[1], chunk.edge_size, chunk.batch_size_forward,
@@ -221,14 +236,16 @@
     return out
 
 
-def gather_by_src_from_dst(chunk, out, grad, with_weight=True, gather_dtype=None):
+def gather_by_src_from_dst(chunk, out, grad, with_weight=True, gather_dtype=None, overwrite=False):
     plan = _bf16_plan(chunk, "bwd", grad.shape[1], with_weight, gather_dtype)
     ev = _timer.bracket("bwd", grad.shape[1], chunk.edge_size, chunk.batch_size_backward) if _timer else None
     if ev:
         ev[0].record()
     if plan is not None:
-        plan.run(grad, out, gather_dtype)
+        plan.run(grad, out, gather_dtype, overwrite)
     else:
+        if overwrite:
+            out.zero_()
         _lib.call("nts_gather_by_src_from_dst", _ptr(grad), _ptr(out), _ptr(chunk.edge_weight_backward_gpu),
                   _ptr(chunk.row_offset_gpu), _ptr(chunk.column_indices_gpu), chunk.src_range[0], chunk.src_range[1],
                   chunk.dst_range[0], chunk.dst_range[1], chunk.edge_size, chunk.batch_size_backward,
@@ -261,16 +278,16 @@
         self.gather_dtype = _check_gather_dtype(gather_dtype)
 
     def forward(self, f_input, f_input1=None):
-        x = _check_gathered(f_input, "input", self.gather_dtype)
+        x = _check_gathered(f_input, "input", self.gather_dtype, rows_ok=True)
         c = self.partitioned_graph_.graph_chunks[0]
-        y = torch.zeros((c.batch_size_forward, x.shape[1]), dtype=torch.float32, device=x.device)
-        return gather_by_dst_from_src(c, y, x, gather_dtype=self.gather_dtype)
+        y = torch.empty((c.batch_size_forward, x.shape[1]), dtype=torch.float32, device=x.device)
+        return gather_by_dst_from_src(c, y, x, gather_dtype=self.gather_dtype, overwrite=True)
 
     def backward(self, f_output_grad):
         g = _check_input(f_output_grad, "output_grad")
         c = self.partitioned_graph_.graph_chunks[0]
-        dx = torch.zeros((c.batch_size_backward, g.shape[1]), dtype=torch.float32, device=g.device)
-        return gather_by_src_from_dst(c, dx, g, gather_dtype=self.gather_dtype)
+        dx = torch.empty((c.batch_size_backward, g.shape[1]), dtype=torch.float32, device=g.device)
+        return gather_by_src_from_dst(c, dx, g, gather_dtype=self.gather_dtype, overwrite=True)
 
 
 class ForwardGPUfuseOp(ntsGraphOp):
diff --git a/neutronstarlite_b200/toolkits.py b/neutronstarlite_b200/toolkits.py
--- a/neutronstarlite_b200/toolkits.py
+++ b/neutronstarlite_b200/toolkits.py
@@ -95,12 +95,16 @@
         self.train_rows = (self.MASK == 0).nonzero().view(-1)
         self.X = [None] * len(self.layers)
         self.gather_dtype = ops._check_gather_dtype(gather_dtype)
-        if self.gather_dtype is not None and self._input_is_gathered:
-            features = features.detach().to(self.gather_dtype)
-        self.X[0] = features.requires_grad_(True)
         if op_class is None:
             op_class = ops.ForwardSingleGPUfuseOp if partitioned_graph.partitions == 1 else ops.ForwardGPUfuseOp
         self.op_class = op_class
+        if self.gather_dtype is not None and self._input_is_gathered:
+            features = features.detach().to(self.gather_dtype)
+        elif self._input_is_gathered and op_class is ops.ForwardSingleGPUfuseOp and features.shape[1] % 4:
+            padded = ops.padded_rows(features.shape[0], features.shape[1], features.device)
+            padded.copy_(features.detach())
+            features = padded
+        self.X[0] = features.requires_grad_(True)
         self.op_kwargs = dict(op_kwargs or {})
         if self.gather_dtype is not None:
             self.op_kwargs["gather_dtype"] = self.gather_dtype
@@ -119,7 +123,8 @@
                 dropped = torch.nn.functional.dropout(x_i, self.drop_rate, training=True)
                 self.ctx.appendNNOp(x_i, dropped)
                 x_i = dropped
-            x_i = x_i.contiguous()
+            if not (self.op_class is ops.ForwardSingleGPUfuseOp and ops.row_padded(x_i)):
+                x_i = x_i.contiguous()
             y_i = self.ctx.runGraphOp(self.op_class, self.pg, None, x_i, **self.op_kwargs)
             self.X[i + 1] = self.ctx.runVertexForward(lambda n, v, _l=i: self.vertexForward(n, v, _l), y_i, x_i)
 
```
